# thomasneff/AdaNeRF

Hardware: AMD Instinct MI355X
Metric: FPS at 800x800 (higher is better)
Workload: dtype bf16

## Files before the change

adanerf_amd/csrc/adanerf_hip.hip:

```cpp
#include "context.hpp"

#include <algorithm>
#include <cmath>
#include <cstdio>
#include <cstring>
#include <exception>
#include <limits>
#include <string>
#include <vector>

#include "guard_record.hpp"
#include "kernels.hip.hpp"
#include "launch_f32.hpp"
#include "k_generic_f32.hip.hpp"
#include "k_generic16.hip.hpp"

using namespace adanerf;

namespace adanerf {

int fail(adanerf_ctx* c, int code, const std::string& msg) {
  if (c) c->err = msg;
  else g_create_error = msg;
  return code;
}

int hip_rc(adanerf_ctx* c, hipError_t e, const char* what) {
  return e == hipSuccess ? ADANERF_OK : fail(c, ADANERF_EDEVICE, std::string(what) + ": " + hipGetErrorString(e));
}

int dev_alloc(adanerf_ctx* c, DevBuf* b, size_t bytes) {
  if (b->bytes >= bytes && b->p) return ADANERF_OK;
  void* grown = nullptr;
  if (bytes) HIP_TRY(c, hipMalloc(&grown, bytes));
  if (b->p) HIP_TRY(c, hipFree(b->p));
  b->p = grown;
  b->bytes = bytes;
  return ADANERF_OK;
}

}

namespace {

enum { kTotalSamples = 0, kTotalRefined = 4, kTotalGuardSeen = 8, kTotalSlots = 16 };
enum { kSeenMax = 0, kSeenViolations = 1, kSeenPair = 2, kSeenAuditMismatch = 3, kSeenAudited = 4, kGuardSeenSlots = 5 };

constexpr const char* kOccupancyQuery = "hipOccupancyMaxActiveBlocksPerMultiprocessor";

int upload_net(adanerf_ctx* c, const PackedNet& pn, PackedDev* d) {
  int rc;
  if ((rc = dev_alloc(c, &d->w, pn.weights.size()))) return rc;
  if ((rc = dev_alloc(c, &d->b, pn.bias.size() * sizeof(float)))) return rc;
  HIP_TRY(c, hipMemcpy(d->w.p, pn.weights.data(), pn.weights.size(), hipMemcpyHostToDevice));
  HIP_TRY(c, hipMemcpy(d->b.p, pn.bias.data(), pn.bias.size() * sizeof(float), hipMemcpyHostToDevice));
  d->params.w = reinterpret_cast<const u32x4*>(d->w.p);
  d->params.bias = reinterpret_cast<const float*>(d->b.p);
  for (size_t i = 0; i < pn.w_off.size() && i < kMaxLayers; ++i) {
    d->params.w_off[i] = pn.w_off[i];
    d->params.b_off[i] = pn.b_off[i];
  }
  d->params.n_bias = static_cast<uint32_t>(pn.bias.size());
  d->params.out_scale[0] = std::ldexp(1.0f, pn.out_exp[0]);
  d->params.out_scale[1] = std::ldexp(1.0f, pn.out_exp[1]);
  return ADANERF_OK;
}

int ensure_shading_net(adanerf_ctx* c, int prec, bool coarse) {
  if (prec < 0 || prec > 2) return fail(c, ADANERF_EINVAL, "precision must be ADANERF_PREC_{BF16,FP16,FP32}");
  PackedDev& dev = coarse ? c->netc[prec] : c->net1[prec];
  if (dev.w.p) return ADANERF_OK;
  PackedNet pn;
  std::string err;
  const NetShape sh = coarse ? shape_of(c->ms.fp0, c->ms.fd0, c->ms.fp0, c->ms.fd0, 0, false)
                             : shape_of(c->ms.fp0, c->ms.fd0, c->ms.fp1, c->ms.fd1, c->ms.ray_samples, !c->ms.coarse_fine);
  if (!pack_shading_net(coarse ? c->net0_host : c->net1_host, sh, elem_of(prec), &pn, &err))
    return fail(c, ADANERF_EIO, (coarse ? "model0.onnx: " : "model1.onnx: ") + err);
  return upload_net(c, pn, &dev);
}

int ensure_batch_buffers(adanerf_ctx* c, int n_rays, int n_max) {
  if (n_rays <= c->cap_rays && n_max <= c->cap_nmax) return ADANERF_OK;
  n_rays = std::max(n_rays, c->cap_rays);
  n_max = std::max(n_max, c->cap_nmax);
  if (c->cap_rays > 0) HIP_TRY(c, hipStreamSynchronize(c->stream));
  const size_t R = static_cast<size_t>(n_rays), S = R * static_cast<size_t>(n_max);
  const size_t nblk = (R + 31) / 32;
  int rc;
  if ((rc = dev_alloc(c, &c->rays, R * 8 * sizeof(float)))) return rc;
  if ((rc = dev_alloc(c, &c->ray_offsets, R * sizeof(int32_t)))) return rc;
  if ((rc = dev_alloc(c, &c->ray_counts, R * sizeof(int32_t)))) return rc;
  if (c->ms.coarse_fine) {
    const size_t Sc = R * static_cast<size_t>(c->ms.n_coarse);
    if ((rc = dev_alloc(c, &c->key_coarse, Sc * sizeof(uint32_t)))) return rc;
    if ((rc = dev_alloc(c, &c->raw_coarse, Sc * 4 * sizeof(float)))) return rc;
    if ((rc = dev_alloc(c, &c->sample_z, S * sizeof(float)))) return rc;
  } else {
    if ((rc = dev_alloc(c, &c->oracle, R * kBins * sizeof(float)))) return rc;
    if ((rc = dev_alloc(c, &c->selbin, S))) return rc;
    if ((rc = dev_alloc(c, &c->selw, S * sizeof(float)))) return rc;
    if (c->sampling_mode == ADANERF_SAMPLING_GUARDED) {
      if ((rc = dev_alloc(c, &c->guard_mask, nblk * sizeof(uint32_t)))) return rc;
      if ((rc = dev_alloc(c, &c->refine_list, R * sizeof(int32_t)))) return rc;
      if ((rc = dev_alloc(c, &c->guard_probe, R * 2 * sizeof(float)))) return rc;
    }
  }
  if ((rc = dev_alloc(c, &c->block_total, nblk * sizeof(int32_t)))) return rc;
  if ((rc = dev_alloc(c, &c->block_offset, nblk * sizeof(int32_t)))) return rc;
  if (!c->total.p) {
    if ((rc = dev_alloc(c, &c->total, kTotalSlots * sizeof(int32_t)))) return rc;
    HIP_TRY(c, hipMemset(c->total.p, 0, kTotalSlots * sizeof(int32_t)));
  }
  if ((rc = dev_alloc(c, &c->sample_key, S * sizeof(uint32_t)))) return rc;
  if ((rc = dev_alloc(c, &c->sample_w, S * sizeof(float)))) return rc;
  if ((rc = dev_alloc(c, &c->raw, S * 4 * sizeof(float)))) return rc;
  if (c->ms.info.sampler_mode == ADANERF_SAMPLER_PDF && (rc = dev_alloc(c, &c->sample_z, S * sizeof(float)))) return rc;
  c->cap_rays = n_rays;
  c->cap_nmax = n_max;
  return ADANERF_OK;
}

int ensure_compact_scratch(adanerf_ctx* c, int n_rays, int n_max) {
  const size_t R = static_cast<size_t>(std::max(n_rays, 1)), S = R * static_cast<size_t>(n_max);
  const size_t nblk = (R + 31) / 32;
  int rc;
  if (c->selbin.bytes < S || c->selw.bytes < S * sizeof(float) || c->block_total.bytes < nblk * sizeof(int32_t) ||
      c->block_offset.bytes < nblk * sizeof(int32_t)) {
    HIP_TRY(c, hipStreamSynchronize(c->stream));
    if ((rc = dev_alloc(c, &c->selbin, S))) return rc;
    if ((rc = dev_alloc(c, &c->selw, S * sizeof(float)))) return rc;
    if ((rc = dev_alloc(c, &c->block_total, nblk * sizeof(int32_t)))) return rc;
    if ((rc = dev_alloc(c, &c->block_offset, nblk * sizeof(int32_t)))) return rc;
  }
  return ADANERF_OK;
}


int ensure_guard_band(adanerf_ctx* c);

bool has_split_sampling(const adanerf_ctx* c) { return (!c->generic0 || c->ms.ray_samples == 0) && c->topo0.width != kWideWidth; }

bool generic_split_sampling(const adanerf_ctx* c) {
  return c->generic0 && c->sampling_mode != ADANERF_SAMPLING_FP32 && c->ms.ray_samples == 0 && c->net0_split.w.p != nullptr;
}

RayGenParams rg_in_force(const adanerf_ctx* c) { return with_pixel_offset(c->ms.rg, c->px_dx, c->px_dy); }

bool has_budget_map(const adanerf_ctx* c) { return c->budget_n != nullptr || c->budget_thr != nullptr; }

struct RayList {
  const int32_t* ids;
  const int32_t* count;
};

int launch_sample_mlp(adanerf_ctx* c, int first_ray, int n_rays, float* d_oracle, float* d_rays, const SelectOut* sel = nullptr,
                      const RayList* list = nullptr) {
  if (n_rays <= 0) return ADANERF_OK;
  if (list && (c->generic0 || !sel || (c->sampling_mode != ADANERF_SAMPLING_SPLIT_FP16 && c->sampling_mode != ADANERF_SAMPLING_GUARDED)))
    return fail(c, ADANERF_EUNSUPPORTED, "a ray list needs the 8 x 256 sampling network on the split-precision engine with the fused selection");
  SampleArgs a{};
  if (sel) {
    a.sel = *sel;
    a.fused_select = 1;
  }
  a.g = rg_in_force(c);
  a.net = c->net0.params;
  a.net16 = c->net0_split.params;
  a.overflow_flag = reinterpret_cast<int32_t*>(c->overflow.p);
  a.first_ray = first_ray;
  a.n_rays = n_rays;
  a.oracle_out = d_oracle;
  a.rays_out = d_rays;
  dim3 grid((n_rays + 127) / 128), block(256);
  if (c->generic0) {
    if (generic_split_sampling(c)) {
      const int W0 = c->topo0.width;
      if (a.net16.n_bias > dispatch<64, 128, 256>(W0, [](auto w) { return uint32_t(gen_bias_cap<w()>()); }, 0u))
        return fail(c, ADANERF_EUNSUPPORTED, "sampling network: bias table exceeds the kernel's LDS capacity");
      return hip_rc(c, dispatch<kEnc10_4, kEnc2_2, kEncMax>(c->enc0, [&](auto e) {
        return dispatch<64, 128, 256>(W0, [&](auto w) {
          hipLaunchKernelGGL((sample_mlp16x3_gen_kernel<enc_fp(e()), enc_fd(e()), w()>), grid, block, 0, c->stream, a, c->gen0);
          return hipGetLastError();
        }, hipErrorInvalidValue);
      }, hipErrorInvalidValue), "hipGetLastError()");
    }
    if (sel) return fail(c, ADANERF_EINVAL, "fused selection is not available on the fp32 run-time-shaped sampling kernel");
    HIP_RETURN(c, launch_sample_mlp_gen(a, c->gen0, c->enc0, c->topo0.width, grid.x, c->stream));
  }
  const bool guarded = c->sampling_mode == ADANERF_SAMPLING_GUARDED && sel != nullptr && !has_budget_map(c) && !(c->sample_cap > 0.f) && !list;
  if (list) {
    a.ray_list = list->ids;
    a.n_list = list->count;
  }
  if (guarded) {
    if (int rc = c->guard_eps > 0.f ? 0 : ensure_guard_band(c)) return rc;
    a.sel.guard_mask = reinterpret_cast<uint32_t*>(c->guard_mask.p);
    a.sel.guard_eps = guard_band_of(c->ms.transform, c->guard_eps);
    a.sel.guard_pair = guard_pair_of(c->ms.transform, c->guard_eps, c->guard_eps_pair);
    a.sel.audit_period = c->guard_audit_period;
    a.sel.audit_phase = c->guard_audit_period > 0 ? static_cast<int32_t>(c->guard_frame & static_cast<uint32_t>(c->guard_audit_period - 1)) : 0;
    a.sel.guard_probe = reinterpret_cast<float*>(c->guard_probe.p);
    a.sel.guard_rows = reinterpret_cast<float*>(c->oracle.p);
    if (c->debug_guard & 1) a.sel.guard_rows = nullptr;
    a.sel.guard_seen = reinterpret_cast<uint32_t*>(c->total.p) + kTotalGuardSeen;
  }
  if (c->sampling_mode == ADANERF_SAMPLING_FP32) HIP_RETURN(c, launch_sample_mlp_f32(a, c->enc0, grid.x, c->stream));
  auto for_enc = [&](auto&& f) {
    return dispatch<kEnc10_4, kEnc2_2>(c->enc0, [&](auto e) { return f(std::integral_constant<int, enc_fp(e())>{}, std::integral_constant<int, enc_fd(e())>{}); },
                                       hipErrorInvalidValue);
  };
  if (c->sampling_mode == ADANERF_SAMPLING_FP16 || guarded) {
    if (!c->net0_f16.w.p) {
      PackedNet pn;
      std::string err;
      const NetShape sh = shape_of(c->ms.fp0, c->ms.fd0, c->ms.fp1, c->ms.fd1, c->ms.ray_samples);
      if (!pack_sampling_net(c->net0_host, sh, Elem::F16, &pn, &err)) return fail(c, ADANERF_EIO, "model0.onnx: " + err);
      if (int rc = upload_net(c, pn, &c->net0_f16)) return rc;
    }
    a.net16 = c->net0_f16.params;
    const bool two_blocks = sel != nullptr && a.fused_select && !a.oracle_out && !(c->debug_guard & 2) && (n_rays >= kSample16x2MinRays || (c->debug_guard & 4));
    if (int rc = hip_rc(c, for_enc([&](auto fp, auto fd) {
      return two_blocks ? launch_persistent(c->grids, sample_mlp16x2_kernel<fp(), fd()>, (n_rays + 255) / 256, 256, c->stream, a)
                        : launch_persistent(c->grids, sample_mlp16_kernel<fp(), fd()>, (n_rays + 255) / 256, 512, c->stream, a);
    }), kOccupancyQuery)) return rc;
    if (guarded) {
      const int n_words = (n_rays + 31) / 32;
      int32_t* n_list = reinterpret_cast<int32_t*>(c->total.p) + kTotalRefined;
      int resident = 0;
      if (int rc = hip_rc(c, for_enc([&](auto fp, auto fd) { return persistent_grid(c->grids, sample_mlp16x3_kernel<fp(), fd()>, 256, &resident); }), kOccupancyQuery)) return rc;
      const int rgrid = std::min(static_cast<int>(grid.x), resident);
      const int cap_round = (c->opt.flags & ADANERF_FLAG_GUARD_AUDIT_FILL) ? rgrid * 128 : 0;
      const int cycle = a.sel.audit_period > 0 ? static_cast<int>((c->guard_frame / static_cast<uint32_t>(a.sel.audit_period)) & 0x7fffffffu) : 0;
      hipLaunchKernelGGL(refine_list_kernel, dim3((n_words + 255) / 256), dim3(256), 0, c->stream, reinterpret_cast<const uint32_t*>(c->guard_mask.p),
                         n_words, n_rays, a.sel.audit_period, a.sel.audit_phase, cap_round, cycle, reinterpret_cast<int32_t*>(c->refine_list.p), n_list);
      SampleArgs r = a;
      r.net16 = c->net0_split.params;
      r.rays_out = nullptr;
      r.sel.guard_mask = nullptr;
      r.sel.guard_band = c->guard_eps;
      r.sel.guard_band_pair = c->ms.transform == kOracleRaw ? a.sel.guard_pair : 0.f;
      r.sel.guard_eps = 0.f;
      r.sel.guard_pair = 0.f;
      r.sel.audit_period = 0;
      r.sel.refine_list = reinterpret_cast<const int32_t*>(c->refine_list.p);
      r.ray_list = r.sel.refine_list;
      r.n_list = n_list;
      if (int rc = hip_rc(c, for_enc([&](auto fp, auto fd) { return launch_persistent(c->grids, sample_mlp16x3_kernel<fp(), fd()>, rgrid, 256, c->stream, r); }), kOccupancyQuery)) return rc;
    }
  } else {
    if (int rc = hip_rc(c, for_enc([&](auto fp, auto fd) { return launch_persistent(c->grids, sample_mlp16x3_kernel<fp(), fd()>, static_cast<int>(grid.x), 256, c->stream, a); }), kOccupancyQuery)) return rc;
  }
  HIP_RETURN(c, hipGetLastError());
}

constexpr int kInlineScanMaxBlocks = 65536;

SelectOut select_out(adanerf_ctx* c, int n_max, float thr, int32_t* d_cnt) {
  SelectOut so{};
  so.counts = d_cnt;
  so.selbin = reinterpret_cast<uint8_t*>(c->selbin.p);
  so.selw = reinterpret_cast<float*>(c->selw.p);
  so.seg_total = reinterpret_cast<int32_t*>(c->block_total.p);
  so.n_max = n_max;
  so.thr = thr;
  so.transform = c->ms.transform;
  return so;
}

int launch_expand(adanerf_ctx* c, int n_rays, int n_max, int seg_shift, int32_t* d_off, const int32_t* d_cnt, uint32_t* d_key, float* d_w,
                  int32_t* d_total) {
  const int nblk = (n_rays + (1 << seg_shift) - 1) >> seg_shift;
  const int32_t* bt = reinterpret_cast<const int32_t*>(c->block_total.p);
  int32_t* bo = reinterpret_cast<int32_t*>(c->block_offset.p);
  const dim3 egrid((n_rays + 255) / 256);
  const bool inline_scan = nblk <= kInlineScanMaxBlocks;
  if (!inline_scan) hipLaunchKernelGGL(scan_blocks_kernel, dim3(1), dim3(1024), 0, c->stream, bt, nblk, bo, d_total);
  hipLaunchKernelGGL(inline_scan ? expand_kernel<true> : expand_kernel<false>, egrid, dim3(256), 0, c->stream, d_cnt, reinterpret_cast<const uint8_t*>(c->selbin.p),
                     reinterpret_cast<const float*>(c->selw.p), bo, bt, nblk, n_rays, n_max, seg_shift, d_off, d_key, d_w, d_total);
  HIP_RETURN(c, hipGetLastError());
}

struct BudgetMaps {
  const uint8_t* n;
  const float* thr;
  int first;
};

int launch_trim(adanerf_ctx* c, const BudgetMaps& bm, int n_rays, int n_max, float thr, int seg_shift, int32_t* d_cnt) {
  if (n_rays <= 0) return ADANERF_OK;
  const bool per_thread = n_max <= kTrimThreadMaxN;
  const dim3 grid(per_thread ? (n_rays + 255) / 256 : (n_rays + (1 << seg_shift) - 1) >> seg_shift);
  hipLaunchKernelGGL(per_thread ? trim_rows_kernel : trim_rows_wave_kernel, grid, dim3(256), 0, c->stream, d_cnt, reinterpret_cast<uint8_t*>(c->selbin.p),
                     reinterpret_cast<float*>(c->selw.p), bm.n, bm.thr, bm.first, n_rays, n_max, thr, seg_shift, reinterpret_cast<int32_t*>(c->block_total.p));
  HIP_RETURN(c, hipGetLastError());
}

struct DepthLimit {
  const float* zc;
  int first;
  const int32_t* list;
  const float* rays;
  const float* ztab;
  DepthPose pose;
};

DepthPose depth_pose(const float pos[3], const float rot[9]) { return DepthPose{{pos[0], pos[1], pos[2]}, rot[2], rot[5], rot[8]}; }

int launch_depth_limit(adanerf_ctx* c, const DepthLimit& dl, int n_rays, int n_max, int seg_shift, int32_t* d_cnt) {
  if (n_rays <= 0) return ADANERF_OK;
  hipLaunchKernelGGL(depth_limit_kernel, dim3((n_rays + 255) / 256), dim3(256), 0, c->stream, d_cnt, reinterpret_cast<uint8_t*>(c->selbin.p),
                     reinterpret_cast<float*>(c->selw.p), dl.rays, dl.zc, dl.list, dl.first, dl.pose, dl.ztab, n_rays, n_max, seg_shift,
                     reinterpret_cast<int32_t*>(c->block_total.p));
  HIP_RETURN(c, hipGetLastError());
}

bool has_sample_cap(const adanerf_ctx* c) { return c->sample_cap > 0.f; }

bool cap_trims(const adanerf_ctx* c) { return has_sample_cap(c) && c->sample_cap < static_cast<float>(c->ms.info.num_samples); }

int64_t cap_total_of(const adanerf_ctx* c, int n_rays) { return static_cast<int64_t>(std::floor(static_cast<double>(c->sample_cap) * n_rays)); }

constexpr size_t kCapStateBytes = sizeof(CapState) + static_cast<size_t>(kCapLevels) * 2 * kCapBins * sizeof(uint32_t);

int ensure_cap_buffers(adanerf_ctx* c, int n_rays) {
  const size_t map_bytes = static_cast<size_t>(std::max(n_rays, 1)) * sizeof(float);
  if (c->cap_state.p && c->cap_record.p && c->cap_map.bytes >= map_bytes) return ADANERF_OK;
  HIP_TRY(c, hipStreamSynchronize(c->stream));
  int rc;
  if ((rc = dev_alloc(c, &c->cap_state, kCapStateBytes))) return rc;
  if ((rc = dev_alloc(c, &c->cap_map, map_bytes))) return rc;
  if (!c->cap_record.p) {
    if ((rc = dev_alloc(c, &c->cap_record, sizeof(CapRecord)))) return rc;
    hipLaunchKernelGGL(cap_reset_kernel, dim3(1), dim3(1), 0, c->stream, reinterpret_cast<CapRecord*>(c->cap_record.p));
    HIP_TRY(c, hipGetLastError());
  }
  return ADANERF_OK;
}

int launch_cap(adanerf_ctx* c, int n_rays, int n_max, float thr, int seg_shift, int32_t* d_cnt, int64_t cap_total) {
  if (n_rays <= 0) return ADANERF_OK;
  CapState* st = reinterpret_cast<CapState*>(c->cap_state.p);
  uint32_t* hist = reinterpret_cast<uint32_t*>(st + 1);
  CapRecord* rec = reinterpret_cast<CapRecord*>(c->cap_record.p);
  float* map = reinterpret_cast<float*>(c->cap_map.p);
  const float* selw = reinterpret_cast<const float*>(c->selw.p);
  HIP_TRY(c, hipMemsetAsync(st, 0, kCapStateBytes, c->stream));
  const bool wave = n_max > kCapThreadMaxN;
  const int cus = std::max(c->ms.info.compute_units, 1);
  const dim3 grid(wave ? std::min((n_rays + 3) / 4, 4 * cus) : std::min((n_rays + 255) / 256, 2 * cus));
  for (int level = 0; level < kCapLevels; ++level) {
    uint32_t* h = hist + static_cast<size_t>(level) * 2 * kCapBins;
    hipLaunchKernelGGL(wave ? cap_hist_kernel<true> : cap_hist_kernel<false>, grid, dim3(256), 0, c->stream, d_cnt, selw, n_rays, n_max, level, st, h);
    hipLaunchKernelGGL(cap_search_kernel, dim3(1), dim3(1024), 0, c->stream, level, static_cast<long long>(cap_total), st, h, rec);
  }
  hipLaunchKernelGGL(cap_fill_kernel, dim3((n_rays + 255) / 256), dim3(256), 0, c->stream, rec, n_rays, map);
  HIP_TRY(c, hipGetLastError());
  return launch_trim(c, BudgetMaps{nullptr, map, 0}, n_rays, n_max, thr, seg_shift, d_cnt);
}

bool use_pair_select(const adanerf_ctx* c, int n_max) { return n_max <= kPairMaxN && !(c->opt.flags & ADANERF_FLAG_WAVE_SELECT); }

int launch_compact(adanerf_ctx* c, const float* d_oracle, int n_rays, int n_max, float thr, int32_t* d_off, int32_t* d_cnt,
                   uint32_t* d_key, float* d_w, int32_t* d_total, const BudgetMaps* bm = nullptr, const DepthLimit* dl = nullptr,
                   const int64_t* cap_total = nullptr) {
  if (n_rays <= 0) return ADANERF_OK;
  if (thr == 0.0f) {
    const size_t n = static_cast<size_t>(n_rays) * kBins;
    dim3 grid(static_cast<unsigned>((n + 255) / 256)), block(256);
    hipLaunchKernelGGL(dense_expand_kernel, grid, block, 0, c->stream, d_oracle, n_rays, d_off, d_cnt, d_key, d_w, d_total);
    HIP_RETURN(c, hipGetLastError());
  }
  if (use_pair_select(c, n_max)) {
    hipLaunchKernelGGL(select_rows_kernel, dim3((n_rays + 127) / 128), dim3(256), 0, c->stream, d_oracle, n_rays, select_out(c, n_max, thr, d_cnt),
                       static_cast<const int32_t*>(nullptr));
    if (bm)
      if (int rc = launch_trim(c, *bm, n_rays, n_max, thr, kPairSegShift, d_cnt)) return rc;
    if (dl)
      if (int rc = launch_depth_limit(c, *dl, n_rays, n_max, kPairSegShift, d_cnt)) return rc;
    if (cap_total)
      if (int rc = launch_cap(c, n_rays, n_max, thr, kPairSegShift, d_cnt, *cap_total)) return rc;
    return launch_expand(c, n_rays, n_max, kPairSegShift, d_off, d_cnt, d_key, d_w, d_total);
  }
  const int nblk = (n_rays + kSelRaysPerBlock - 1) / kSelRaysPerBlock;
  hipLaunchKernelGGL(select_kernel, dim3(nblk), dim3(256), 0, c->stream, d_oracle, n_rays, n_max, thr, c->ms.transform, d_cnt,
                     reinterpret_cast<uint8_t*>(c->selbin.p), reinterpret_cast<float*>(c->selw.p),
                     reinterpret_cast<int32_t*>(c->block_total.p));
  if (bm)
    if (int rc = launch_trim(c, *bm, n_rays, n_max, thr, kSelSegShift, d_cnt)) return rc;
  if (dl)
    if (int rc = launch_depth_limit(c, *dl, n_rays, n_max, kSelSegShift, d_cnt)) return rc;
  if (cap_total)
    if (int rc = launch_cap(c, n_rays, n_max, thr, kSelSegShift, d_cnt, *cap_total)) return rc;
  return launch_expand(c, n_rays, n_max, kSelSegShift, d_off, d_cnt, d_key, d_w, d_total);
}

GuardKey guard_key(adanerf_ctx* c) {
  if (!c->model0_hash) c->model0_hash = fnv1a64_file(join_path(c->model_dir, "model0.onnx"));
  return GuardKey{c->model0_hash, c->ms.fp0, c->ms.fd0, c->ms.transform, kGuardEngineRev, c->ms.info.num_samples, c->ms.info.threshold, c->model_dir, c->opt.flags};
}

void install_guard_band(adanerf_ctx* c, float max_diff, float max_pair, int poses, int source) {
  c->guard_eps = std::max(ADANERF_GUARD_CALIB_MARGIN * max_diff, ADANERF_GUARD_EPS_MIN);
  c->guard_eps_pair = (c->ms.transform == kOracleRaw && max_pair > 0.f)
                          ? std::min(std::max(ADANERF_GUARD_CALIB_MARGIN * max_pair, ADANERF_GUARD_EPS_MIN), 2.0f * c->guard_eps)
                          : 2.0f * c->guard_eps;
  c->ms.info.guard_eps = c->guard_eps;
  c->ms.info.guard_eps_pair = c->guard_eps_pair;
  c->ms.info.guard_calib_source = source;
  c->ms.info.guard_calib_poses = poses;
}

int calibrate_guard(adanerf_ctx* c, int n_poses, uint32_t seed, bool install, float* max_diff, float* max_pair) {
  if (c->ms.coarse_fine || c->generic0) return fail(c, ADANERF_EUNSUPPORTED, "guard calibration needs an 8 x 256 sampling network");
  if (n_poses < 1 || n_poses > 4096) return fail(c, ADANERF_EINVAL, "n_poses must be in 1..4096");
  constexpr int CW = 64, CH = 64, CR = CW * CH;
  const RayGenParams saved = c->ms.rg;
  const int saved_mode = c->sampling_mode;
  const float saved_dx = c->px_dx, saved_dy = c->px_dy;
  c->px_dx = c->px_dy = 0.f;
  RayGenParams g = saved;
  const double x_dist = -saved.start_x + saved.x_pp / 2, y_dist = -saved.start_y + saved.y_pp / 2;
  g.w = CW;
  g.h = CH;
  g.x_pp = x_dist / (CW / 2.0);
  g.y_pp = y_dist / (CH / 2.0);
  g.start_x = -(x_dist - g.x_pp / 2);
  g.start_y = -(y_dist - g.y_pp / 2);
  g.strip_rows = CH;
  g.world = 1;
  g.rank = 0;
  DevBuf a_buf, b_buf, acc;
  int rc = ADANERF_OK;
  auto done = [&](int code) {
    (void)hipStreamSynchronize(c->stream);
    c->ms.rg = saved;
    c->sampling_mode = saved_mode;
    c->px_dx = saved_dx;
    c->px_dy = saved_dy;
    return code;
  };
  if ((rc = dev_alloc(c, &a_buf, static_cast<size_t>(CR) * kBins * sizeof(float)))) return done(rc);
  if ((rc = dev_alloc(c, &b_buf, static_cast<size_t>(CR) * kBins * sizeof(float)))) return done(rc);
  if ((rc = dev_alloc(c, &acc, 64))) return done(rc);
  if (hipMemsetAsync(acc.p, 0, 64, c->stream) != hipSuccess) return done(fail(c, ADANERF_EDEVICE, "hipMemsetAsync failed"));
  const bool want_pairs = c->ms.transform == kOracleRaw && c->ms.info.threshold > 0.f && c->ms.info.num_samples <= kPairMaxN;
  float d = 0.f, dp = 0.f;
  bool nonfinite = false;
  for (int sweep = 0; sweep < (want_pairs ? 2 : 1) && !nonfinite; ++sweep) {
    const float two_eps = sweep == 0 ? 0.f : 2.0f * std::max(ADANERF_GUARD_CALIB_MARGIN * d, ADANERF_GUARD_EPS_MIN);
    uint64_t st = 0x9E3779B97F4A7C15ull ^ (static_cast<uint64_t>(seed) << 17);
    auto rnd = [&]() {
      st ^= st >> 12;
      st ^= st << 25;
      st ^= st >> 27;
      return static_cast<double>((st * 0x2545F4914F6CDD1Dull) >> 11) * (1.0 / 9007199254740992.0);
    };
    for (int k = 0; k < n_poses; ++k) {
      for (int i = 0; i < 3; ++i) g.pos[i] = g.center[i] + static_cast<float>((rnd() - 0.5) * 0.9 * c->ms.info.view_cell_size[i]);
      const double yaw = 2.0 * M_PI * rnd(), pitch = (rnd() - 0.5) * (c->ms.info.use_ndc ? 0.2 : 1.4);
      const double cy = std::cos(yaw), sy = std::sin(yaw), cp = std::cos(pitch), sp = std::sin(pitch);
      double fwd[3], right[3], up[3];
      if (c->ms.info.use_ndc) {
        fwd[0] = sp * cy; fwd[1] = sp * sy; fwd[2] = -cp;
        right[0] = 1; right[1] = 0; right[2] = 0;
      } else {
        fwd[0] = cp * cy; fwd[1] = cp * sy; fwd[2] = sp;
        right[0] = sy; right[1] = -cy; right[2] = 0;
      }
      const double rf = right[0] * fwd[0] + right[1] * fwd[1] + right[2] * fwd[2];
      double n = 0;
      for (int i = 0; i < 3; ++i) { right[i] -= rf * fwd[i]; n += right[i] * right[i]; }
      n = std::sqrt(n);
      for (int i = 0; i < 3; ++i) right[i] /= n;
      up[0] = right[1] * fwd[2] - right[2] * fwd[1];
      up[1] = right[2] * fwd[0] - right[0] * fwd[2];
      up[2] = right[0] * fwd[1] - right[1] * fwd[0];
      for (int i = 0; i < 3; ++i) {
        g.rot[3 * i + 0] = static_cast<float>(right[i]);
        g.rot[3 * i + 1] = static_cast<float>(up[i]);
        g.rot[3 * i + 2] = static_cast<float>(-fwd[i]);
      }
      c->ms.rg = g;
      c->sampling_mode = ADANERF_SAMPLING_SPLIT_FP16;
      if ((rc = launch_sample_mlp(c, 0, CR, reinterpret_cast<float*>(a_buf.p), nullptr))) return done(rc);
      c->sampling_mode = ADANERF_SAMPLING_FP16;
      if ((rc = launch_sample_mlp(c, 0, CR, reinterpret_cast<float*>(b_buf.p), nullptr))) return done(rc);
      hipLaunchKernelGGL(guard_stats_kernel, dim3((CR + 3) / 4), dim3(256), 0, c->stream, reinterpret_cast<const float*>(b_buf.p),
                         reinterpret_cast<const float*>(a_buf.p), CR, c->ms.info.num_samples, c->ms.info.threshold, two_eps, reinterpret_cast<uint32_t*>(acc.p));
    }
    uint32_t res[3] = {0, 0, 0};
    if (hipMemcpyAsync(res, acc.p, sizeof(res), hipMemcpyDeviceToHost, c->stream) != hipSuccess || hipStreamSynchronize(c->stream) != hipSuccess)
      return done(fail(c, ADANERF_EDEVICE, "guard calibration: read-back failed"));
    std::memcpy(&d, &res[0], sizeof(d));
    std::memcpy(&dp, &res[2], sizeof(dp));
    nonfinite = res[1] != 0;
  }
  if (max_diff) *max_diff = nonfinite ? INFINITY : d;
  if (max_pair) *max_pair = (nonfinite || !want_pairs) ? 0.f : dp;
  if (install) {
    if (nonfinite) {
      c->guard_eps = ADANERF_GUARD_EPS_DEFAULT;
      c->guard_eps_pair = 2.0f * c->guard_eps;
      c->ms.info.guard_eps = c->guard_eps;
      c->ms.info.guard_eps_pair = c->guard_eps_pair;
      c->ms.info.guard_calib_source = ADANERF_GUARD_FROM_CALIBRATION;
      c->ms.info.guard_calib_poses = n_poses;
    } else {
      install_guard_band(c, d, want_pairs ? dp : 0.f, n_poses, ADANERF_GUARD_FROM_CALIBRATION);
      const GuardKey key = guard_key(c);
      GuardRecord old;
      if (!(read_guard_record(key, &old) && old.poses > n_poses)) write_guard_record(key, GuardRecord{n_poses, seed, d, want_pairs ? dp : 0.f});
    }
  }
  return done(ADANERF_OK);
}

int ensure_guard_band(adanerf_ctx* c) {
  GuardRecord r;
  if (read_guard_record(guard_key(c), &r) && r.poses >= ADANERF_GUARD_CALIB_POSES) {
    install_guard_band(c, r.max_diff, r.max_pair, r.poses, ADANERF_GUARD_FROM_RECORD);
    return ADANERF_OK;
  }
  float d = 0.f, dp = 0.f;
  return calibrate_guard(c, ADANERF_GUARD_CALIB_POSES, 1u, true, &d, &dp);
}

int reset_guard_band(adanerf_ctx* c) {
  if (c->sampling_mode == ADANERF_SAMPLING_GUARDED)
    HIP_TRY(c, hipMemsetAsync(reinterpret_cast<int32_t*>(c->total.p) + kTotalRefined, 0, sizeof(int32_t), c->stream));
  const adanerf_options& opt = c->opt;
  c->guard_eps = opt.guard_eps > 0.f ? opt.guard_eps : 0.f;
  c->guard_eps_pair = (c->guard_eps > 0.f && opt.guard_eps_pair > 0.f) ? std::min(opt.guard_eps_pair, 2.0f * c->guard_eps) : 2.0f * c->guard_eps;
  c->ms.info.guard_eps = c->guard_eps;
  c->ms.info.guard_eps_pair = c->guard_eps_pair;
  c->ms.info.guard_calib_source = c->guard_eps > 0.f ? ADANERF_GUARD_FROM_OPTIONS : ADANERF_GUARD_FROM_NONE;
  c->ms.info.guard_calib_poses = 0;
  c->guard_frame = 0;
  c->guard_ev_stale = c->guard_ev_pending;
  return ADANERF_OK;
}

int apply_selection(adanerf_ctx* c) {
  if (int rc = ensure_batch_buffers(c, c->ms.info.batch_rays, c->ms.info.num_samples)) return rc;
  if (int rc = reset_guard_band(c)) return rc;
  c->ms.sp.ztab = reinterpret_cast<const float*>(c->ztab.p) + (c->ms.info.dense ? kBins : 0);
  return ADANERF_OK;
}

int apply_frame_size(adanerf_ctx* c, int was_rays) {
  const size_t B = static_cast<size_t>(c->ms.info.batch_rays);
  if (int rc = ensure_batch_buffers(c, c->ms.info.batch_rays, c->ms.info.num_samples)) return rc;
  if (c->disp_scratch.p && c->disp_scratch.bytes < B * 2 * sizeof(float)) {
    HIP_TRY(c, hipStreamSynchronize(c->stream));
    if (int rc = dev_alloc(c, &c->disp_scratch, B * 2 * sizeof(float))) return rc;
  }
  if (c->ms.info.rays_local != was_rays) {
    c->aux_depth = c->aux_acc = c->aux_disp = nullptr;
    c->budget_n = nullptr;
    c->budget_thr = nullptr;
    c->depth_limit = nullptr;
  }
  c->guard_frame = 0;
  return ADANERF_OK;
}

int launch_shade_mlp(adanerf_ctx* c, const float* d_rays, const uint32_t* d_key, const int32_t* d_total, int max_samples, int prec,
                     float* d_raw, const float* d_z = nullptr, bool coarse = false) {
  if (max_samples <= 0) return ADANERF_OK;
  const bool generic = coarse ? c->genericc : c->generic1;
  const NetTopology& topo = coarse ? c->topoc : c->topo1;
  const GenericTopo& gen = coarse ? c->genc : c->gen1;
  int rc = ensure_shading_net(c, prec, coarse);
  if (rc) return rc;
  ShadeArgs a{};
  a.sp = coarse ? c->spc : c->ms.sp;
  a.net = coarse ? c->netc[prec].params : c->net1[prec].params;
  a.rays = d_rays;
  a.sample_key = d_key;
  a.sample_z = d_z;
  a.total = d_total;
  a.max_samples = max_samples;
  a.raw_out = d_raw;
  a.pos_limit = prec == ADANERF_PREC_BF16 ? static_cast<float>(kPosIdentityBound) : std::numeric_limits<float>::max();
  const int enc = coarse ? enc_layout(c->ms.fp0, c->ms.fd0, false) : c->enc1;
  auto for_elem = [&](auto&& f) { return prec == ADANERF_PREC_BF16 ? f(Bf16{}) : f(Fp16{}); };
  if (generic && prec != ADANERF_PREC_FP32) {
    if (a.net.n_bias > dispatch<64, 128, 256, 512>(topo.width, [](auto w) { return uint32_t(gen_bias_cap<w()>()); }, 0u))
      return fail(c, ADANERF_EUNSUPPORTED, "shading network: bias table exceeds the kernel's LDS capacity");
    if ((rc = hip_rc(c, for_elem([&](auto et) {
      return dispatch<kEnc10_4, kEncMax>(enc, [&](auto e) {
        return dispatch<64, 128, 256, 512>(topo.width, [&](auto w) {
          using ET = decltype(et);
          constexpr int FP = enc_fp(e()), FD = enc_fd(e()), W = w(), NB = gen_blocks<W, FP>();
          const int tiles = (max_samples + 128 * NB - 1) / (128 * NB);
          return launch_persistent(c->grids, shade_mlp16_gen_staged_kernel<ET, FP, FD, W, NB, gen_occupancy<W, FP>()>, tiles, 256, c->stream, a, gen);
        }, hipErrorInvalidValue);
      }, hipErrorInvalidValue);
    }), kOccupancyQuery))) return rc;
  } else if (generic) {
    const int per_wg = topo.width == kWideWidth ? 64 : 128;
    HIP_TRY(c, launch_shade_mlp_gen(c->grids, a, gen, enc, topo.width, (max_samples + per_wg - 1) / per_wg, c->stream));
  } else if (prec == ADANERF_PREC_FP32) {
    HIP_TRY(c, launch_shade_mlp_f32(c->grids, a, (max_samples + 127) / 128, c->stream));
  } else {
    const int tiles = (max_samples + 255) / 256;
    if ((rc = hip_rc(c, for_elem([&](auto et) {
      using ET = decltype(et);
      hipLaunchKernelGGL((shade_mlp16x2_kernel<ET, 10, 4>), dim3(std::min(tiles, c->ms.info.compute_units)), dim3(256), 0, c->stream, a);
      return hipSuccess;
    }), kOccupancyQuery))) return rc;
  }
  HIP_RETURN(c, hipGetLastError());
}

int launch_sample_pdf(adanerf_ctx* c, const float* d_oracle, int n_rays, int n, int32_t* d_off, int32_t* d_cnt, uint32_t* d_key, float* d_w,
                      float* d_z, int32_t* d_total) {
  if (n_rays <= 0) return ADANERF_OK;
  const int grid = std::min((n_rays + 3) / 4, c->ms.info.compute_units * 8);
  hipLaunchKernelGGL(pdf_sample_kernel, dim3(grid), dim3(256), 0, c->stream, d_oracle, n_rays, n, c->ms.transform, c->ms.dm, d_off, d_cnt, d_key, d_w, d_z, d_total);
  HIP_RETURN(c, hipGetLastError());
}

int launch_camera_rays(adanerf_ctx* c, int first_ray, int n_rays, float* d_rays) {
  if (n_rays <= 0) return ADANERF_OK;
  hipLaunchKernelGGL(camera_rays_kernel, dim3((n_rays + 255) / 256), dim3(256), 0, c->stream, rg_in_force(c), first_ray, n_rays, d_rays);
  HIP_RETURN(c, hipGetLastError());
}

int launch_sample_uniform(adanerf_ctx* c, int n_rays, int n, int32_t* d_off, int32_t* d_cnt, uint32_t* d_key, int32_t* d_total) {
  if (n_rays <= 0) return ADANERF_OK;
  const int64_t s = static_cast<int64_t>(n_rays) * n;
  hipLaunchKernelGGL(uniform_sample_kernel, dim3(static_cast<unsigned>((s + 255) / 256)), dim3(256), 0, c->stream, n_rays, n, d_off, d_cnt, d_key, d_total);
  HIP_RETURN(c, hipGetLastError());
}

int launch_sample_fine(adanerf_ctx* c, const float* d_raw_coarse, const float* d_rays, int n_rays, int32_t* d_off, int32_t* d_cnt,
                       uint32_t* d_key, float* d_z, int32_t* d_total) {
  if (n_rays <= 0) return ADANERF_OK;
  hipLaunchKernelGGL(fine_sample_kernel, dim3((n_rays + kFineRaysPerBlock - 1) / kFineRaysPerBlock), dim3(kFineRaysPerBlock), 0, c->stream,
                     reinterpret_cast<const float4*>(d_raw_coarse), reinterpret_cast<const float*>(c->ztab_coarse.p), d_rays, n_rays, c->ms.n_coarse,
                     c->ms.info.num_samples - c->ms.n_coarse, d_off, d_cnt, d_key, d_z, d_total);
  HIP_RETURN(c, hipGetLastError());
}

int launch_composite_classic(adanerf_ctx* c, const float* d_raw, const float* d_z, const float* d_rays, int n_rays, int n, float* d_rgb,
                             void* d_rgba8, float* d_depth = nullptr, float* d_acc = nullptr) {
  if (n_rays <= 0) return ADANERF_OK;
  const bool wave = n > 32;
  hipLaunchKernelGGL(wave ? composite_classic_wave_kernel : composite_classic_kernel, dim3((n_rays + (wave ? 3 : 255)) / (wave ? 4 : 256)), dim3(256), 0, c->stream,
                     reinterpret_cast<const float4*>(d_raw), d_z, d_rays, n_rays, n, d_rgb, reinterpret_cast<uchar4*>(d_rgba8), d_depth, d_acc);
  HIP_RETURN(c, hipGetLastError());
}

int launch_composite(adanerf_ctx* c, const float* d_raw, const float* d_w, const int32_t* d_off, const int32_t* d_cnt, int n_rays,
                     float* d_rgb, void* d_rgba8, const uint32_t* d_key = nullptr, float* d_depth = nullptr, float* d_acc = nullptr) {
  if (n_rays <= 0) return ADANERF_OK;
  AuxOut aux{};
  if ((d_key || c->ms.info.dense) && (d_depth || d_acc)) {
    aux.depth = d_depth;
    aux.acc = d_acc;
    aux.sample_key = d_key;
    aux.ztab = c->ms.sp.ztab;
  }
  if (c->ms.info.num_samples > 32)
    hipLaunchKernelGGL(composite_wave_kernel, dim3((n_rays + 3) / 4), dim3(256), 0, c->stream, reinterpret_cast<const float4*>(d_raw), d_w,
                       d_off, d_cnt, n_rays, c->ms.mult_mode, d_rgb, reinterpret_cast<uchar4*>(d_rgba8), aux);
  else {
    const int N = c->ms.info.num_samples;
    auto run = [&](auto rb_tag) {
      constexpr int RB = decltype(rb_tag)::value;
      const int cap = RB * N;
      hipLaunchKernelGGL(composite_kernel<RB>, dim3((n_rays + RB - 1) / RB), dim3(RB), static_cast<size_t>(cap) * 20, c->stream,
                         reinterpret_cast<const float4*>(d_raw), d_w, d_off, d_cnt, n_rays, c->ms.mult_mode, cap, d_rgb,
                         reinterpret_cast<uchar4*>(d_rgba8), aux);
    };
    if (N <= 9) run(std::integral_constant<int, 256>{});
    else if (N <= 19) run(std::integral_constant<int, 128>{});
    else run(std::integral_constant<int, 64>{});
  }
  HIP_RETURN(c, hipGetLastError());
}

}


extern "C" {

const char* adanerf_last_error(const adanerf_ctx* ctx) { return ctx ? ctx->err.c_str() : g_create_error.c_str(); }

static int create_on(adanerf_ctx* c, const char* model_dir, const adanerf_options* opt, adanerf_ctx** out);

int adanerf_create(const char* model_dir, const adanerf_options* opt, adanerf_ctx** out) {
  if (!out) return fail(nullptr, ADANERF_EINVAL, "out == NULL");
  *out = nullptr;
  if (!model_dir || !opt) return fail(nullptr, ADANERF_EINVAL, "model_dir/opt == NULL");
  adanerf_ctx* c = nullptr;
  try {
    c = new adanerf_ctx();
    return create_on(c, model_dir, opt, out);
  } catch (const std::exception& e) {
    *out = nullptr;
    adanerf_destroy(c);
    return fail(nullptr, ADANERF_EIO, std::string("adanerf_create: ") + e.what());
  }
}

static int create_on(adanerf_ctx* c, const char* model_dir, const adanerf_options* opt, adanerf_ctx** out) {
  auto bail = [&](int code, const std::string& msg) {
    g_create_error = msg;
    adanerf_destroy(c);
    return code;
  };
  std::string err;
  ModelSetup& ms = c->ms;
  int rc = setup_model(model_dir, opt, &ms, &err);
  if (rc) return bail(rc, err);
  c->opt = *opt;

  TensorMap& n0 = c->net0_host;
  if (!read_onnx_initializers(join_path(model_dir, "model0.onnx"), &n0, &err)) return bail(ADANERF_EIO, err);
  if (!read_onnx_initializers(join_path(model_dir, "model1.onnx"), &c->net1_host, &err)) return bail(ADANERF_EIO, err);
  const NetShape sh = shape_of(c->ms.fp0, c->ms.fd0, c->ms.fp1, c->ms.fd1, c->ms.ray_samples, !c->ms.coarse_fine);
  c->enc0 = enc_layout(c->ms.fp0, c->ms.fd0, !c->ms.coarse_fine);
  c->enc1 = enc_layout(c->ms.fp1, c->ms.fd1, false);
  PackedNet p0, p0s, p1;
  if (c->ms.coarse_fine) {
    const NetShape shc = shape_of(c->ms.fp0, c->ms.fd0, c->ms.fp0, c->ms.fd0, 0, false);
    if (!pack_shading_net(n0, shc, Elem::F32, &p0, &err)) return bail(ADANERF_EIO, "model0.onnx: " + err);
    c->topoc = p0.topo;
    c->genericc = !p0.topo.is_default(true) || c->enc0 == kEncMax;
    if (opt->precision != ADANERF_PREC_FP32 && !pack_shading_net(n0, shc, elem_of(opt->precision), &p0, &err))
      return bail(ADANERF_EIO, "model0.onnx: " + err);
  } else {
    if (!pack_sampling_net(n0, sh, Elem::F32, &p0, &err)) return bail(ADANERF_EIO, "model0.onnx: " + err);
    if (p0.topo.bins != ms.bins)
      return bail(ADANERF_EIO, "model0.onnx has " + std::to_string(p0.topo.bins) + " outputs, config.ini says multiDepthFeatures = " + std::to_string(ms.bins));
    c->topo0 = p0.topo;
    c->generic0 = !p0.topo.is_default(false) || c->enc0 == kEncMax;
    if (has_split_sampling(c) && !pack_sampling_net(n0, sh, Elem::F16_SPLIT, &p0s, &err)) return bail(ADANERF_EIO, "model0.onnx: " + err);
  }
  c->sampling_mode = opt->sampling_mode;
  c->model_dir = model_dir;
  if (const char* dbg = std::getenv("ADANERF_DEBUG_GUARD")) c->debug_guard = std::atoi(dbg);
  c->guard_audit_period = opt->guard_audit_period == 0 ? ADANERF_GUARD_AUDIT_PERIOD : std::max(opt->guard_audit_period, 0);
  c->ms.info.guard_audit_period = c->sampling_mode == ADANERF_SAMPLING_GUARDED ? c->guard_audit_period : 0;
  if (c->sampling_mode == ADANERF_SAMPLING_GUARDED) c->model0_hash = fnv1a64_file(join_path(model_dir, "model0.onnx"));
  {
    PackedNet probe;
    if (!pack_shading_net(c->net1_host, sh, Elem::F32, &probe, &err)) return bail(ADANERF_EIO, "model1.onnx: " + err);
    c->topo1 = probe.topo;
    c->generic1 = !probe.topo.is_default(true) || c->enc1 == kEncMax;
    if (opt->precision == ADANERF_PREC_FP32) p1 = std::move(probe);
    else if (!pack_shading_net(c->net1_host, sh, elem_of(opt->precision), &p1, &err)) return bail(ADANERF_EIO, "model1.onnx: " + err);
  }
  auto width_ok = [](int w) { return w == 64 || w == 128 || w == 256 || w == kWideWidth; };
  if (c->genericc && !width_ok(c->topoc.width)) return bail(ADANERF_EUNSUPPORTED, "model0.onnx: layer width " + std::to_string(c->topoc.width) + " (64, 128, 256 or 512 supported)");
  if (c->generic0 && !width_ok(c->topo0.width)) return bail(ADANERF_EUNSUPPORTED, "model0.onnx: layer width " + std::to_string(c->topo0.width) + " (64, 128, 256 or 512 supported)");
  if (c->generic1 && !width_ok(c->topo1.width)) return bail(ADANERF_EUNSUPPORTED, "model1.onnx: layer width " + std::to_string(c->topo1.width) + " (64, 128, 256 or 512 supported)");

  int n_dev = 0;
  if (hipGetDeviceCount(&n_dev) != hipSuccess || n_dev <= 0)
    return bail(ADANERF_EDEVICE, "no HIP device available: libadanerf_hip has no CPU fallback");
  if (hipSetDevice(opt->device_id) != hipSuccess) return bail(ADANERF_EDEVICE, "hipSetDevice failed");
  hipDeviceProp_t prop;
  if (hipGetDeviceProperties(&prop, opt->device_id) != hipSuccess) return bail(ADANERF_EDEVICE, "hipGetDeviceProperties failed");
  if (std::string(prop.gcnArchName).find("gfx950") == std::string::npos)
    return bail(ADANERF_EDEVICE, std::string("device is ") + prop.gcnArchName + "; this library is built for gfx950 (MI355X) only");
  c->ms.info.compute_units = c->grids.compute_units = prop.multiProcessorCount;
  c->device = opt->device_id;
  if (hipStreamCreateWithFlags(&c->own_stream, hipStreamNonBlocking) != hipSuccess) return bail(ADANERF_EDEVICE, "hipStreamCreate failed");
  c->stream = c->own_stream;

  rc = dev_alloc(c, &c->ztab, 2 * kBins * sizeof(float));
  if (rc) return bail(rc, c->err);
  float ztabs[2 * kBins];
  depth_table(ms, false, ztabs);
  depth_table(ms, true, ztabs + kBins);
  if (hipMemcpy(c->ztab.p, ztabs, sizeof(ztabs), hipMemcpyHostToDevice) != hipSuccess)
    return bail(ADANERF_EDEVICE, "ztab upload failed");
  if (c->ms.coarse_fine) {
    if ((rc = upload_net(c, p0, &c->netc[opt->precision]))) return bail(rc, c->err);
    if ((rc = dev_alloc(c, &c->ztab_coarse, kMaxCoarse * sizeof(float)))) return bail(rc, c->err);
    if (hipMemcpy(c->ztab_coarse.p, ms.ztab_coarse.data(), ms.ztab_coarse.size() * sizeof(float), hipMemcpyHostToDevice) != hipSuccess)
      return bail(ADANERF_EDEVICE, "coarse depth table upload failed");
    c->spc = c->ms.sp;
    c->spc.normalize = ms.normalize0;
    c->ms.sp.unit_dir = 0;
    c->spc.ztab = reinterpret_cast<const float*>(c->ztab_coarse.p);
    c->genc = GenericTopo{c->topoc.depth, c->topoc.cat_mask, 0, 0, nullptr, 0.f};
  } else {
    if ((rc = upload_net(c, p0, &c->net0))) return bail(rc, c->err);
    if (has_split_sampling(c) && (rc = upload_net(c, p0s, &c->net0_split))) return bail(rc, c->err);
  }
  if (c->ms.ray_samples > 0) {
    if ((rc = dev_alloc(c, &c->rsi_z, ms.rsi_z.size() * sizeof(float)))) return bail(rc, c->err);
    if (hipMemcpy(c->rsi_z.p, ms.rsi_z.data(), ms.rsi_z.size() * sizeof(float), hipMemcpyHostToDevice) != hipSuccess)
      return bail(ADANERF_EDEVICE, "raySampleInput depth table upload failed");
  }
  c->gen0 = GenericTopo{c->topo0.depth, 0, c->ms.ray_samples, p0.rsi_w_off, reinterpret_cast<const float*>(c->rsi_z.p), c->ms.cfg.depthRange[1]};
  c->gen1 = GenericTopo{c->topo1.depth, c->topo1.cat_mask, 0, 0, nullptr, 0.f};
  if ((rc = dev_alloc(c, &c->overflow, 64))) return bail(rc, c->err);
  if (hipMemset(c->overflow.p, 0, 64) != hipSuccess) return bail(ADANERF_EDEVICE, "hipMemset failed");
  if ((rc = upload_net(c, p1, &c->net1[opt->precision]))) return bail(rc, c->err);
  if ((rc = apply_selection(c))) return bail(rc, c->err);
  *out = c;
  return ADANERF_OK;
}

int adanerf_destroy(adanerf_ctx* c) {
  if (!c) return ADANERF_OK;
  (void)hipSetDevice(c->device);
  if (c->peer_event) (void)hipEventDestroy(c->peer_event);
  if (c->stream) (void)hipStreamSynchronize(c->stream);
  for (hipEvent_t e : c->events) (void)hipEventDestroy(e);
  for (int32_t* p : c->pinned_totals) (void)hipHostFree(p);
  if (c->guard_host) (void)hipHostFree(c->guard_host);
  if (c->guard_ev) (void)hipEventDestroy(c->guard_ev);
  const hipStream_t own = c->own_stream;
  delete c;
  if (own) (void)hipStreamDestroy(own);
  return ADANERF_OK;
}

int adanerf_get_info(const adanerf_ctx* c, adanerf_info* info) {
  if (!c || !info) return ADANERF_EINVAL;
  *info = c->ms.info;
  return ADANERF_OK;
}

int adanerf_set_camera(adanerf_ctx* c, const float pos[3], const float rot[9]) {
  if (!c) return ADANERF_EINVAL;
  if (!pos || !rot) return fail(c, ADANERF_EINVAL, "pos/rot == NULL");
  if (c->ms.pos_bound.active) {
    double d2 = 0.0;
    for (int i = 0; i < 3; ++i) d2 += (pos[i] - c->ms.pos_bound.center[i]) * (pos[i] - c->ms.pos_bound.center[i]);
    const double bound = c->ms.pos_bound.at(std::sqrt(d2));
    if (!(bound <= kPosIdentityBound)) {
      char msg[256];
      std::snprintf(msg, sizeof(msg), "camera %.3g away from the view-cell centre: sample positions can reach %.3g, beyond the %.0f the bf16 shading path's "
                    "layer scaling assumes -- create the context with precision fp16 or fp32 for such poses", std::sqrt(d2), bound, kPosIdentityBound);
      return fail(c, ADANERF_EUNSUPPORTED, msg);
    }
  }
  std::memcpy(c->ms.rg.pos, pos, 3 * sizeof(float));
  std::memcpy(c->ms.rg.rot, rot, 9 * sizeof(float));
  return ADANERF_OK;
}

int adanerf_set_selection(adanerf_ctx* c, int32_t num_samples, float threshold) {
  BIND(c);
  if (std::isnan(threshold)) return fail(c, ADANERF_EINVAL, "threshold is not a number (a negative value keeps the one in force)");
  if (threshold >= 0.f && c->ms.info.sampler_mode != ADANERF_SAMPLER_ADAPTIVE)
    return fail(c, ADANERF_EUNSUPPORTED, "this model's sampler takes no threshold (adanerf_create ignores options.threshold for it): pass a negative one");
  if (threshold == 0.f && has_budget_map(c))
    return fail(c, ADANERF_EUNSUPPORTED, "threshold 0 (dense) keeps every bin: remove the budget map first (adanerf_set_budget_map with two NULLs)");
  if (threshold == 0.f && c->depth_limit)
    return fail(c, ADANERF_EUNSUPPORTED, "threshold 0 (dense) keeps every bin with implicit keys: remove the depth limit first (adanerf_set_depth_limit with NULL)");
  if (threshold == 0.f && has_sample_cap(c))
    return fail(c, ADANERF_EUNSUPPORTED, "threshold 0 (dense) keeps every bin: remove the sample cap first (adanerf_set_sample_cap with 0)");
  ModelSetup& ms = c->ms;
  const adanerf_info was = ms.info;
  const ModelSetup::PosBound was_bound = ms.pos_bound;
  const int was_n = ms.sel_n;
  const float was_thr = ms.sel_thr;
  std::vector<float> was_ztab = ms.ztab;
  std::string err;
  if (int rc = select_samples(&ms, num_samples, threshold, &err)) return fail(c, rc, err);
  if (ms.info.num_samples == was.num_samples && ms.info.threshold == was.threshold) return ADANERF_OK;
  if (int rc = apply_selection(c)) {
    ms.info = was;
    ms.pos_bound = was_bound;
    ms.sel_n = was_n;
    ms.sel_thr = was_thr;
    ms.ztab = std::move(was_ztab);
    return rc;
  }
  return ADANERF_OK;
}

int adanerf_set_frame_size(adanerf_ctx* c, int32_t width, int32_t height) {
  BIND(c);
  ModelSetup& ms = c->ms;
  const int w = width > 0 ? width : ms.info.width, h = height > 0 ? height : ms.info.height;
  if (w == ms.info.width && h == ms.info.height) return ADANERF_OK;
  const adanerf_info was = ms.info;
  const RayGenParams was_rg = ms.rg;
  std::string err;
  if (int rc = frame_geometry(&ms, &c->opt, w, h, &err)) return fail(c, rc, err);
  if (int rc = apply_frame_size(c, was.rays_local)) {
    ms.info = was;
    ms.rg = was_rg;
    return rc;
  }
  c->opt.width = w;
  c->opt.height = h;
  return ADANERF_OK;
}

int adanerf_set_pixel_offset(adanerf_ctx* c, float dx, float dy) {
  if (!c) return ADANERF_EINVAL;
  if (!(std::fabs(dx) <= 1.f) || !(std::fabs(dy) <= 1.f))
    return fail(c, ADANERF_EINVAL, "adanerf_set_pixel_offset: dx and dy must be finite and within -1..1 (pixels)");
  c->px_dx = dx;
  c->px_dy = dy;
  return ADANERF_OK;
}

int adanerf_get_pixel_offset(const adanerf_ctx* c, float out[2]) {
  if (!c || !out) return ADANERF_EINVAL;
  out[0] = c->px_dx;
  out[1] = c->px_dy;
  return ADANERF_OK;
}

int adanerf_sync(adanerf_ctx* c) {
  BIND(c);
  HIP_RETURN(c, hipStreamSynchronize(c->stream));
}

int adanerf_ray_features(adanerf_ctx* c, int32_t first_ray, int32_t n_rays, float* d_feat, float* d_rays) {
  BIND(c);
  if (c->ms.coarse_fine) return fail(c, ADANERF_EUNSUPPORTED, "coarse/fine models have no sampling network");
  if (first_ray < 0 || n_rays < 0 || first_ray + n_rays > c->ms.info.rays_local) return fail(c, ADANERF_EINVAL, "ray range outside this context's rays");
  if (n_rays == 0) return ADANERF_OK;
  dim3 grid((n_rays + 255) / 256), block(256);
  const float* rz = reinterpret_cast<const float*>(c->rsi_z.p);
  const float d1 = c->ms.cfg.depthRange[1];
  hipLaunchKernelGGL(ray_features_kernel, grid, block, 0, c->stream, rg_in_force(c), first_ray, n_rays, d_feat, d_rays, c->ms.ray_samples, rz, d1, c->ms.fp0, c->ms.fd0);
  HIP_RETURN(c, hipGetLastError());
}

int adanerf_sample_mlp(adanerf_ctx* c, int32_t first_ray, int32_t n_rays, float* d_oracle, float* d_rays) {
  BIND(c);
  if (c->ms.coarse_fine) return fail(c, ADANERF_EUNSUPPORTED, "coarse/fine models have no sampling network (adanerf_sample_uniform / adanerf_shade_mlp_coarse)");
  if (first_ray < 0 || n_rays < 0 || first_ray + n_rays > c->ms.info.rays_local) return fail(c, ADANERF_EINVAL, "ray range outside this context's rays");
  return launch_sample_mlp(c, first_ray, n_rays, d_oracle, d_rays);
}

int adanerf_compact(adanerf_ctx* c, const float* d_oracle, int32_t n_rays, int32_t n_max, float thr, int32_t* d_off, int32_t* d_cnt,
                    uint32_t* d_key, float* d_w, int32_t* d_total) {
  BIND(c);
  if (!d_oracle || !d_off || !d_cnt || !d_key || !d_w || !d_total) return fail(c, ADANERF_EINVAL, "NULL buffer");
  if (n_rays < 0 || n_max < 1 || n_max > kBins || thr < 0.f) return fail(c, ADANERF_EINVAL, "n_rays/n_max/thr out of range");
  if (thr == 0.f && n_max != kBins) return fail(c, ADANERF_EINVAL, "dense mode (thr == 0) requires n_max == 128");
  if (static_cast<int64_t>(n_rays) >= (1ll << 25)) return fail(c, ADANERF_EINVAL, "n_rays must be < 2^25 per batch");
  if (static_cast<int64_t>(n_rays) * n_max > 0x7fffffffll) return fail(c, ADANERF_EINVAL, "n_rays * n_max exceeds 2^31 - 1");
  if (int rc = ensure_compact_scratch(c, n_rays, n_max)) return rc;
  return launch_compact(c, d_oracle, n_rays, n_max, thr, d_off, d_cnt, d_key, d_w, d_total);
}

int adanerf_compact_guarded(adanerf_ctx* c, const float* d_approx, const float* d_exact, int32_t n_rays, int32_t n_max, float thr, float eps,
                            float eps_pair, int32_t audit_period, int32_t audit_phase, int32_t audit_fill_cap, int32_t audit_cycle, int32_t* d_off,
                            int32_t* d_cnt, uint32_t* d_key, float* d_w, int32_t* d_total, int32_t* d_refined, uint32_t* d_monitor) {
  BIND(c);
  if (!d_approx || !d_exact || !d_off || !d_cnt || !d_key || !d_w || !d_total || !d_refined) return fail(c, ADANERF_EINVAL, "NULL buffer");
  if (n_rays < 0 || n_max < 1 || n_max > kPairMaxN || !(thr > 0.f) || !(eps > 0.f)) return fail(c, ADANERF_EINVAL, "n_rays/n_max/thr/eps out of range");
  if (audit_period > 32 || (audit_period > 0 && (audit_period & (audit_period - 1)) != 0)) return fail(c, ADANERF_EINVAL, "audit_period must be a power of two <= 32");
  if (static_cast<int64_t>(n_rays) >= (1ll << 25)) return fail(c, ADANERF_EINVAL, "n_rays must be < 2^25 per batch");
  if (n_rays == 0) return ADANERF_OK;
  int rc = ensure_compact_scratch(c, n_rays, n_max);
  if (rc) return rc;
  const int n_words = (n_rays + 31) / 32;
  if (c->guard_mask.bytes < n_words * sizeof(uint32_t) || c->refine_list.bytes < static_cast<size_t>(n_rays) * sizeof(int32_t) ||
      c->guard_probe.bytes < static_cast<size_t>(n_rays) * 2 * sizeof(float)) {
    HIP_TRY(c, hipStreamSynchronize(c->stream));
    if ((rc = dev_alloc(c, &c->guard_mask, n_words * sizeof(uint32_t)))) return rc;
    if ((rc = dev_alloc(c, &c->refine_list, static_cast<size_t>(n_rays) * sizeof(int32_t)))) return rc;
    if ((rc = dev_alloc(c, &c->guard_probe, static_cast<size_t>(n_rays) * 2 * sizeof(float)))) return rc;
  }
  const int period = audit_period > 0 ? audit_period : 0, phase = period ? (audit_phase & (period - 1)) : 0;
  SelectOut so = select_out(c, n_max, thr, d_cnt);
  so.guard_mask = reinterpret_cast<uint32_t*>(c->guard_mask.p);
  so.guard_eps = guard_band_of(c->ms.transform, eps);
  so.guard_pair = guard_pair_of(c->ms.transform, eps, eps_pair);
  so.audit_period = period;
  so.audit_phase = phase;
  so.guard_probe = reinterpret_cast<float*>(c->guard_probe.p);
  const dim3 grid((n_rays + 127) / 128), block(256);
  hipLaunchKernelGGL(select_rows_kernel, grid, block, 0, c->stream, d_approx, n_rays, so, static_cast<const int32_t*>(nullptr));
  hipLaunchKernelGGL(refine_list_kernel, dim3((n_words + 255) / 256), dim3(256), 0, c->stream, reinterpret_cast<const uint32_t*>(c->guard_mask.p), n_words,
                     n_rays, period, phase, audit_fill_cap > 0 ? audit_fill_cap : 0, audit_cycle, reinterpret_cast<int32_t*>(c->refine_list.p), d_refined);
  so.guard_mask = nullptr;
  so.guard_band = eps;
  so.guard_band_pair = c->ms.transform == kOracleRaw ? so.guard_pair : 0.f;
  so.guard_eps = 0.f;
  so.guard_pair = 0.f;
  so.audit_period = 0;
  so.refine_list = reinterpret_cast<const int32_t*>(c->refine_list.p);
  so.guard_rows = d_monitor ? const_cast<float*>(d_approx) : nullptr;
  so.guard_seen = d_monitor;
  hipLaunchKernelGGL(select_rows_kernel, grid, block, 0, c->stream, d_exact, n_rays, so, static_cast<const int32_t*>(d_refined));
  return launch_expand(c, n_rays, n_max, kPairSegShift, d_off, d_cnt, d_key, d_w, d_total);
}

int adanerf_calibrate_guard(adanerf_ctx* c, int32_t n_poses, uint32_t seed, int32_t set, float* max_diff, float* max_pair_diff) {
  BIND(c);
  return calibrate_guard(c, n_poses, seed, set != 0, max_diff, max_pair_diff);
}

int adanerf_guard_calibration_file(const adanerf_ctx* c, char* buf, size_t buf_bytes) {
  if (!c) return ADANERF_EINVAL;
  const std::string p = guard_record_path(guard_key(const_cast<adanerf_ctx*>(c)));
  if (buf && buf_bytes > 0) {
    const size_t n = std::min(p.size(), buf_bytes - 1);
    std::memcpy(buf, p.data(), n);
    buf[n] = 0;
  }
  return static_cast<int>(p.size() + 1);
}

int adanerf_abi_version(void) { return ADANERF_ABI_VERSION; }

int adanerf_struct_sizes(int32_t sizes_out[3]) {
  if (!sizes_out) return ADANERF_EINVAL;
  sizes_out[0] = static_cast<int32_t>(sizeof(adanerf_options));
  sizes_out[1] = static_cast<int32_t>(sizeof(adanerf_info));
  sizes_out[2] = static_cast<int32_t>(sizeof(adanerf_stats));
  return ADANERF_OK;
}

int adanerf_shade_features(adanerf_ctx* c, const float* d_rays, const uint32_t* d_key, int32_t n_samples, float* d_feat) {
  BIND(c);
  if (!d_rays || !d_key || !d_feat || n_samples < 0) return fail(c, ADANERF_EINVAL, "bad argument");
  if (n_samples == 0) return ADANERF_OK;
  ShadeArgs a{};
  a.sp = c->ms.sp;
  a.rays = d_rays;
  a.sample_key = d_key;
  a.max_samples = n_samples;
  hipLaunchKernelGGL(shade_features_kernel, dim3((n_samples + 255) / 256), dim3(256), 0, c->stream, a, d_feat, c->ms.fp1, c->ms.fd1);
  HIP_RETURN(c, hipGetLastError());
}

int adanerf_shade_mlp(adanerf_ctx* c, const float* d_rays, const uint32_t* d_key, const int32_t* d_total, int32_t max_samples,
                      int32_t precision, float* d_raw) {
  return adanerf_shade_mlp_z(c, d_rays, d_key, nullptr, d_total, max_samples, precision, d_raw);
}

int adanerf_shade_mlp_z(adanerf_ctx* c, const float* d_rays, const uint32_t* d_key, const float* d_z, const int32_t* d_total,
                        int32_t max_samples, int32_t precision, float* d_raw) {
  BIND(c);
  if (!d_rays || !d_key || !d_raw || max_samples < 0) return fail(c, ADANERF_EINVAL, "bad argument");
  return launch_shade_mlp(c, d_rays, d_key, d_total, max_samples, precision < 0 ? c->ms.info.precision : precision, d_raw, d_z);
}

int adanerf_sample_uniform(adanerf_ctx* c, int32_t first_ray, int32_t n_rays, float* d_rays, int32_t* d_off, int32_t* d_cnt, uint32_t* d_key,
                           int32_t* d_total) {
  BIND(c);
  if (!c->ms.coarse_fine) return fail(c, ADANERF_EUNSUPPORTED, "adanerf_sample_uniform: not a coarse/fine model");
  if (!d_rays || !d_off || !d_cnt || !d_key || !d_total) return fail(c, ADANERF_EINVAL, "NULL buffer");
  if (first_ray < 0 || n_rays < 0 || first_ray + n_rays > c->ms.info.rays_local) return fail(c, ADANERF_EINVAL, "ray range outside this context's rays");
  int rc = launch_camera_rays(c, first_ray, n_rays, d_rays);
  return rc ? rc : launch_sample_uniform(c, n_rays, c->ms.n_coarse, d_off, d_cnt, d_key, d_total);
}

int adanerf_shade_mlp_coarse(adanerf_ctx* c, const float* d_rays, const uint32_t* d_key, const int32_t* d_total, int32_t max_samples,
                             int32_t precision, float* d_raw) {
  BIND(c);
  if (!c->ms.coarse_fine) return fail(c, ADANERF_EUNSUPPORTED, "adanerf_shade_mlp_coarse: not a coarse/fine model");
  if (!d_rays || !d_key || !d_raw || max_samples < 0) return fail(c, ADANERF_EINVAL, "bad argument");
  return launch_shade_mlp(c, d_rays, d_key, d_total, max_samples, precision < 0 ? c->ms.info.precision : precision, d_raw, nullptr, true);
}

int adanerf_sample_from_coarse(adanerf_ctx* c, const float* d_raw_coarse, const float* d_rays, int32_t n_rays, int32_t* d_off, int32_t* d_cnt,
                               uint32_t* d_key, float* d_z, int32_t* d_total) {
  BIND(c);
  if (!c->ms.coarse_fine) return fail(c, ADANERF_EUNSUPPORTED, "adanerf_sample_from_coarse: not a coarse/fine model");
  if (!d_raw_coarse || !d_rays || !d_off || !d_cnt || !d_key || !d_z || !d_total) return fail(c, ADANERF_EINVAL, "NULL buffer");
  if (n_rays < 0 || static_cast<int64_t>(n_rays) * c->ms.info.num_samples > 0x7fffffffll || n_rays >= (1 << 25))
    return fail(c, ADANERF_EINVAL, "n_rays out of range");
  return launch_sample_fine(c, d_raw_coarse, d_rays, n_rays, d_off, d_cnt, d_key, d_z, d_total);
}

int adanerf_sample_pdf(adanerf_ctx* c, const float* d_oracle, int32_t n_rays, int32_t n, int32_t* d_off, int32_t* d_cnt, uint32_t* d_key,
                       float* d_w, float* d_z, int32_t* d_total) {
  BIND(c);
  if (!d_oracle || !d_off || !d_cnt || !d_key || !d_w || !d_z || !d_total) return fail(c, ADANERF_EINVAL, "NULL buffer");
  if (n_rays < 0 || n < 1 || n > 4096) return fail(c, ADANERF_EINVAL, "n_rays/n out of range");
  if (static_cast<int64_t>(n_rays) * n > 0x7fffffffll || n_rays >= (1 << 25)) return fail(c, ADANERF_EINVAL, "n_rays * n too large");
  return launch_sample_pdf(c, d_oracle, n_rays, n, d_off, d_cnt, d_key, d_w, d_z, d_total);
}

int adanerf_composite_classic(adanerf_ctx* c, const float* d_raw, const float* d_z, const float* d_rays, int32_t n_rays, int32_t n,
                              float* d_rgb, void* d_rgba8) {
  BIND(c);
  if (!d_raw || !d_z || !d_rays || n_rays < 0 || n < 1) return fail(c, ADANERF_EINVAL, "bad argument");
  return launch_composite_classic(c, d_raw, d_z, d_rays, n_rays, n, d_rgb, d_rgba8);
}

int adanerf_composite(adanerf_ctx* c, const float* d_raw, const float* d_w, const int32_t* d_off, const int32_t* d_cnt, int32_t n_rays,
                      float* d_rgb, void* d_rgba8) {
  BIND(c);
  if (!d_raw || !d_w || !d_off || !d_cnt || n_rays < 0) return fail(c, ADANERF_EINVAL, "bad argument");
  return launch_composite(c, d_raw, d_w, d_off, d_cnt, n_rays, d_rgb, d_rgba8);
}

int adanerf_composite_aux(adanerf_ctx* c, const float* d_raw, const float* d_w, const int32_t* d_off, const int32_t* d_cnt, const uint32_t* d_key,
                          int32_t n_rays, float* d_rgb, void* d_rgba8, float* d_depth, float* d_acc) {
  BIND(c);
  if (!d_raw || !d_w || !d_off || !d_cnt || n_rays < 0) return fail(c, ADANERF_EINVAL, "bad argument");
  if (!d_key && !c->ms.info.dense && (d_depth || d_acc))
    return fail(c, ADANERF_EINVAL, "adanerf_composite_aux: a depth or acc map needs d_sample_key unless the context is dense (threshold 0)");
  return launch_composite(c, d_raw, d_w, d_off, d_cnt, n_rays, d_rgb, d_rgba8, d_key, d_depth, d_acc);
}

int adanerf_composite_classic_aux(adanerf_ctx* c, const float* d_raw, const float* d_z, const float* d_rays, int32_t n_rays, int32_t n,
                                  float* d_rgb, void* d_rgba8, float* d_depth, float* d_acc) {
  BIND(c);
  if (!d_raw || !d_z || !d_rays || n_rays < 0 || n < 1) return fail(c, ADANERF_EINVAL, "bad argument");
  return launch_composite_classic(c, d_raw, d_z, d_rays, n_rays, n, d_rgb, d_rgba8, d_depth, d_acc);
}

int adanerf_disp_map(adanerf_ctx* c, const float* d_depth, const float* d_acc, int32_t n, float* d_disp) {
  BIND(c);
  if (!d_depth || !d_acc || !d_disp || n < 0) return fail(c, ADANERF_EINVAL, "adanerf_disp_map: NULL buffer or n < 0");
  if (n == 0) return ADANERF_OK;
  hipLaunchKernelGGL(disp_map_kernel, dim3((n + 255) / 256), dim3(256), 0, c->stream, d_depth, d_acc, n, d_disp);
  HIP_RETURN(c, hipGetLastError());
}

namespace {

constexpr size_t kMaxProfiledBatches = 1 << 16;

void reset_record(adanerf_ctx* c) {
  c->events_used = 0;
  c->prof_frames = 0;
  c->folded = adanerf_stats{};
}

int sum_stats(adanerf_ctx* c, adanerf_stats* stats) {
  std::memset(stats, 0, sizeof(*stats));
  const size_t nb = c->events_used / 5;
  for (size_t b = 0; b < nb; ++b) {
    hipEvent_t* ev = &c->events[b * 5];
    float t;
    HIP_TRY(c, hipEventElapsedTime(&t, ev[0], ev[1]));
    stats->ms_sample_mlp += t;
    HIP_TRY(c, hipEventElapsedTime(&t, ev[1], ev[2]));
    stats->ms_compact += t;
    HIP_TRY(c, hipEventElapsedTime(&t, ev[2], ev[3]));
    stats->ms_shade_mlp += t;
    HIP_TRY(c, hipEventElapsedTime(&t, ev[3], ev[4]));
    stats->ms_composite += t;
    HIP_TRY(c, hipEventElapsedTime(&t, ev[0], ev[4]));
    stats->ms_total += t;
    const int32_t* tot = c->pinned_totals[b];
    stats->total_samples += tot[kTotalSamples];
    if (c->sampling_mode == ADANERF_SAMPLING_GUARDED) {
      stats->rays_refined += tot[kTotalRefined];
      const int32_t* gs = tot + kTotalGuardSeen;
      float seen, pair;
      std::memcpy(&seen, &gs[kSeenMax], sizeof(seen));
      std::memcpy(&pair, &gs[kSeenPair], sizeof(pair));
      stats->guard_max_seen = std::max(stats->guard_max_seen, seen);
      stats->guard_pair_seen = std::max(stats->guard_pair_seen, pair);
      stats->guard_violations = std::max(stats->guard_violations, gs[kSeenViolations]);
      stats->guard_audit_mismatch = std::max(stats->guard_audit_mismatch, gs[kSeenAuditMismatch]);
      stats->guard_audited = std::max(stats->guard_audited, gs[kSeenAudited]);
    }
  }
  int32_t ovf = 0;
  HIP_TRY(c, hipMemcpy(&ovf, c->overflow.p, sizeof(int32_t), hipMemcpyDeviceToHost));
  stats->sampling_overflow = ovf;
  stats->batches = static_cast<int32_t>(nb);
  stats->shade_launches = static_cast<int32_t>(nb);
  stats->sample_launches = static_cast<int32_t>(nb);
  const adanerf_stats& f = c->folded;
  stats->total_samples += f.total_samples;
  stats->rays_refined += f.rays_refined;
  stats->guard_max_seen = std::max(stats->guard_max_seen, f.guard_max_seen);
  stats->guard_violations = std::max(stats->guard_violations, f.guard_violations);
  stats->guard_pair_seen = std::max(stats->guard_pair_seen, f.guard_pair_seen);
  stats->guard_audit_mismatch = std::max(stats->guard_audit_mismatch, f.guard_audit_mismatch);
  stats->guard_audited = std::max(stats->guard_audited, f.guard_audited);
  stats->guard_widened = c->guard_widened;
  stats->ms_total += f.ms_total;
  stats->ms_sample_mlp += f.ms_sample_mlp;
  stats->ms_compact += f.ms_compact;
  stats->ms_shade_mlp += f.ms_shade_mlp;
  stats->ms_composite += f.ms_composite;
  stats->batches += f.batches;
  stats->shade_launches += f.shade_launches;
  stats->sample_launches += f.sample_launches;
  return ADANERF_OK;
}

}

int adanerf_copy_result_sampling_network(adanerf_ctx* c, const float* d_oracle, int32_t n_rays, void* d_rgba8) {
  BIND(c);
  if (!d_oracle || !d_rgba8) return fail(c, ADANERF_EINVAL, "NULL buffer");
  if (n_rays < 0) return fail(c, ADANERF_EINVAL, "n_rays out of range");
  if (n_rays == 0) return ADANERF_OK;
  hipLaunchKernelGGL(oracle_view_kernel, dim3((n_rays + 3) / 4), dim3(256), 0, c->stream, d_oracle, n_rays, static_cast<uchar4*>(d_rgba8));
  HIP_RETURN(c, hipGetLastError());
}

int adanerf_render_oracle(adanerf_ctx* c, void* d_rgba8) {
  BIND(c);
  if (!d_rgba8) return fail(c, ADANERF_EINVAL, "NULL buffer");
  if (c->ms.coarse_fine) return fail(c, ADANERF_EUNSUPPORTED, "coarse/fine models have no sampling network to view");
  const int R = c->ms.info.rays_local, B = c->ms.info.batch_rays;
  int rc = ensure_batch_buffers(c, std::min(B, std::max(R, 1)), c->ms.info.num_samples);
  if (rc) return rc;
  float* rays = reinterpret_cast<float*>(c->rays.p);
  float* oracle = reinterpret_cast<float*>(c->oracle.p);
  for (int first = 0; first < R; first += B) {
    const int n = std::min(B, R - first);
    if ((rc = launch_sample_mlp(c, first, n, oracle, rays))) return rc;
    if ((rc = adanerf_copy_result_sampling_network(c, oracle, n, static_cast<char*>(d_rgba8) + static_cast<size_t>(first) * 4))) return rc;
  }
  return ADANERF_OK;
}

namespace {

void poll_guard(adanerf_ctx* c) {
  if (!c->guard_ev_pending) return;
  const hipError_t q = hipEventQuery(c->guard_ev);
  (void)hipGetLastError();
  if (q != hipSuccess) return;
  c->guard_ev_pending = false;
  float seen, pair;
  std::memcpy(&seen, &c->guard_host[kSeenMax], sizeof(seen));
  std::memcpy(&pair, &c->guard_host[kSeenPair], sizeof(pair));
  const int viol = c->guard_host[kSeenViolations], mism = c->guard_host[kSeenAuditMismatch];
  if (c->guard_ev_stale) {
    c->guard_ev_stale = false;
    c->guard_viol_seen = std::max(c->guard_viol_seen, viol);
    c->guard_mism_seen = std::max(c->guard_mism_seen, mism);
    return;
  }
  bool widened = false;
  if (viol > c->guard_viol_seen) {
    c->guard_viol_seen = viol;
    if (seen > c->guard_eps) {
      c->guard_eps = ADANERF_GUARD_CALIB_MARGIN * seen;
      c->guard_eps_pair = 2.0f * c->guard_eps;
      widened = true;
    } else if (pair > c->guard_eps_pair) {
      c->guard_eps_pair = ADANERF_GUARD_CALIB_MARGIN * pair;
      widened = true;
    }
  }
  if (mism > c->guard_mism_seen) {
    c->guard_mism_seen = mism;
    if (!widened) {
      c->guard_eps *= 2.0f;
      c->guard_eps_pair = 2.0f * c->guard_eps;
      widened = true;
    }
  }
  if (widened) {
    c->guard_eps_pair = std::min(std::max(c->guard_eps_pair, ADANERF_GUARD_EPS_MIN), 2.0f * c->guard_eps);
    c->ms.info.guard_eps = c->guard_eps;
    c->ms.info.guard_eps_pair = c->guard_eps_pair;
    c->ms.info.guard_calib_source = ADANERF_GUARD_FROM_MONITOR;
    ++c->guard_widened;
  }
}


int begin_record(adanerf_ctx* c, adanerf_stats* stats, int n_batches, bool* record_out) {
  int rc;
  if (stats && c->profiling && c->events_used) {
    HIP_TRY(c, hipStreamSynchronize(c->stream));
    reset_record(c);
  }
  const bool record = (stats || c->profiling) && static_cast<size_t>(n_batches) <= kMaxProfiledBatches;
  if (record && c->events_used && c->events_used / 5 + n_batches > kMaxProfiledBatches) {
    HIP_TRY(c, hipStreamSynchronize(c->stream));
    adanerf_stats part;
    if ((rc = sum_stats(c, &part))) return rc;
    c->folded = part;
    c->events_used = 0;
  }
  if (record) {
    const size_t need = c->events_used + static_cast<size_t>(n_batches) * 5;
    while (c->events.size() < need) {
      hipEvent_t e;
      HIP_TRY(c, hipEventCreate(&e));
      c->events.push_back(e);
    }
    while (c->pinned_totals.size() < need / 5) {
      int32_t* p = nullptr;
      HIP_TRY(c, hipHostMalloc(reinterpret_cast<void**>(&p), kTotalSlots * sizeof(int32_t), hipHostMallocDefault));
      std::memset(p, 0, kTotalSlots * sizeof(int32_t));
      c->pinned_totals.push_back(p);
    }
  }
  *record_out = record;
  return ADANERF_OK;
}

struct BatchOut {
  float* rgb;
  void* rgba8;
  float* depth;
  float* acc;
  float* disp;
};

int render_batch(adanerf_ctx* c, int first, int n, const RayList* list, const BatchOut& out, bool record) {
  const int B = c->ms.info.batch_rays, N = c->ms.info.num_samples;
  const float thr = c->ms.info.threshold;
  const bool budget = has_budget_map(c);
  int rc;
  float* rays = reinterpret_cast<float*>(c->rays.p);
  float* oracle = reinterpret_cast<float*>(c->oracle.p);
  int32_t* off = reinterpret_cast<int32_t*>(c->ray_offsets.p);
  const bool cfm = c->ms.coarse_fine;
  int32_t* cnt = reinterpret_cast<int32_t*>(c->ray_counts.p);
  uint32_t* key = reinterpret_cast<uint32_t*>(c->sample_key.p);
  float* sw = reinterpret_cast<float*>(c->sample_w.p);
  float* raw = reinterpret_cast<float*>(c->raw.p);
  int32_t* total = reinterpret_cast<int32_t*>(c->total.p);
  hipEvent_t* ev = record ? &c->events[c->events_used] : nullptr;
  if (ev) HIP_TRY(c, hipEventRecord(ev[0], c->stream));
  const bool pdf = c->ms.info.sampler_mode == ADANERF_SAMPLER_PDF || cfm;
  if (cfm) {
    uint32_t* keyc = reinterpret_cast<uint32_t*>(c->key_coarse.p);
    float* rawc = reinterpret_cast<float*>(c->raw_coarse.p);
    if ((rc = launch_camera_rays(c, first, n, rays))) return rc;
    if ((rc = launch_sample_uniform(c, n, c->ms.n_coarse, off, cnt, keyc, total))) return rc;
    if ((rc = launch_shade_mlp(c, rays, keyc, total, n * c->ms.n_coarse, c->ms.info.precision, rawc, nullptr, true))) return rc;
    if (ev) HIP_TRY(c, hipEventRecord(ev[1], c->stream));
    if ((rc = launch_sample_fine(c, rawc, rays, n, off, cnt, key, reinterpret_cast<float*>(c->sample_z.p), total))) return rc;
  }
  const bool fused = !pdf && thr > 0.f && use_pair_select(c, N) && c->sampling_mode != ADANERF_SAMPLING_FP32 && (!c->generic0 || generic_split_sampling(c)) &&
                     !(c->opt.flags & ADANERF_FLAG_KEEP_ORACLE);
  const SelectOut so = select_out(c, N, thr, cnt);
  const BudgetMaps bm{c->budget_n, c->budget_thr, first};
  const bool limited = c->depth_limit != nullptr;
  const bool capped = cap_trims(c) && !pdf && thr > 0.f;
  const int64_t cap_total = capped ? cap_total_of(c, n) : 0;
  const DepthLimit dl{c->depth_limit, first, list ? list->ids : nullptr, rays, c->ms.sp.ztab, depth_pose(c->ms.rg.pos, c->ms.rg.rot)};
  if (!cfm && (rc = launch_sample_mlp(c, first, n, fused ? nullptr : oracle, rays, fused ? &so : nullptr, list))) return rc;
  if (ev && !cfm) HIP_TRY(c, hipEventRecord(ev[1], c->stream));
  float* sz = reinterpret_cast<float*>(c->sample_z.p);
  if (cfm) rc = ADANERF_OK;
  else if (pdf) rc = launch_sample_pdf(c, oracle, n, N, off, cnt, key, sw, sz, total);
  else if (fused) {
    rc = budget ? launch_trim(c, bm, n, N, thr, kPairSegShift, cnt) : ADANERF_OK;
    if (!rc && limited) rc = launch_depth_limit(c, dl, n, N, kPairSegShift, cnt);
    if (!rc && capped) rc = launch_cap(c, n, N, thr, kPairSegShift, cnt, cap_total);
    if (!rc) rc = launch_expand(c, n, N, kPairSegShift, off, cnt, key, sw, total);
  }
  else if (thr == 0.f) {
    hipLaunchKernelGGL(dense_offsets_kernel, dim3((n + 255) / 256), dim3(256), 0, c->stream, n, off, cnt, total);
    HIP_TRY(c, hipGetLastError());
  } else rc = launch_compact(c, oracle, n, N, thr, off, cnt, key, sw, total, budget ? &bm : nullptr, limited ? &dl : nullptr, capped ? &cap_total : nullptr);
  if (rc) return rc;
  const bool dense_implicit = !cfm && !pdf && !fused && thr == 0.f;
  const uint32_t* key_s = dense_implicit ? nullptr : key;
  const float* sw_s = dense_implicit ? oracle : sw;
  if (ev) HIP_TRY(c, hipEventRecord(ev[2], c->stream));
  const int64_t max_s = static_cast<int64_t>(n) * N;
  if ((rc = launch_shade_mlp(c, rays, key_s, total, static_cast<int>(max_s), c->ms.info.precision, raw, pdf ? sz : nullptr))) return rc;
  if (ev) HIP_TRY(c, hipEventRecord(ev[3], c->stream));
  float* depth_b = out.depth;
  float* acc_b = out.acc;
  if (out.disp && (!depth_b || !acc_b)) {
    if ((rc = dev_alloc(c, &c->disp_scratch, static_cast<size_t>(B) * 2 * sizeof(float)))) return rc;
    if (!depth_b) depth_b = reinterpret_cast<float*>(c->disp_scratch.p);
    if (!acc_b) acc_b = reinterpret_cast<float*>(c->disp_scratch.p) + B;
  }
  if (pdf) rc = launch_composite_classic(c, raw, sz, rays, n, N, out.rgb, out.rgba8, depth_b, acc_b);
  else rc = launch_composite(c, raw, sw_s, off, cnt, n, out.rgb, out.rgba8, key_s, depth_b, acc_b);
  if (rc) return rc;
  if (out.disp && n > 0) {
    hipLaunchKernelGGL(disp_map_kernel, dim3((n + 255) / 256), dim3(256), 0, c->stream, depth_b, acc_b, n, out.disp);
    HIP_TRY(c, hipGetLastError());
  }
  if (ev) {
    HIP_TRY(c, hipEventRecord(ev[4], c->stream));
    HIP_TRY(c, hipMemcpyAsync(c->pinned_totals[c->events_used / 5], total, kTotalSlots * sizeof(int32_t), hipMemcpyDeviceToHost, c->stream));
    c->events_used += 5;
  }
  return ADANERF_OK;
}

int end_record(adanerf_ctx* c, adanerf_stats* stats, int n_batches, bool record, int rays) {
  if (record) c->prof_frames++;
  if (stats) {
    HIP_TRY(c, hipStreamSynchronize(c->stream));
    poll_guard(c);
    if (int rc = sum_stats(c, stats)) return rc;
    stats->rays = rays;
    if (n_batches > 0 && record) {
      const size_t e0 = c->events_used - static_cast<size_t>(n_batches) * 5;
      HIP_TRY(c, hipEventElapsedTime(&stats->ms_total, c->events[e0], c->events[c->events_used - 1]));
    }
    reset_record(c);
  }
  return ADANERF_OK;
}

}

int adanerf_render(adanerf_ctx* c, void* d_rgba8, float* d_rgb, adanerf_stats* stats) {
  BIND(c);
  poll_guard(c);
  const int R = c->ms.info.rays_local, B = c->ms.info.batch_rays, N = c->ms.info.num_samples;
  const int n_batches = R > 0 ? (R + B - 1) / B : 0;
  const bool budget = has_budget_map(c) || has_sample_cap(c);
  int rc = ensure_batch_buffers(c, std::min(B, std::max(R, 1)), N);
  if (rc) return rc;
  if (has_sample_cap(c)) c->cap_record_live = cap_trims(c);
  if (cap_trims(c)) {
    if ((rc = ensure_cap_buffers(c, std::min(B, std::max(R, 1))))) return rc;
    hipLaunchKernelGGL(cap_reset_kernel, dim3(1), dim3(1), 0, c->stream, reinterpret_cast<CapRecord*>(c->cap_record.p));
    HIP_TRY(c, hipGetLastError());
  }
  bool record = false;
  if ((rc = begin_record(c, stats, n_batches, &record))) return rc;
  int32_t* total = reinterpret_cast<int32_t*>(c->total.p);
  for (int b = 0; b < n_batches; ++b) {
    const int first = b * B, n = std::min(B, R - first);
    const BatchOut out{d_rgb ? d_rgb + static_cast<size_t>(first) * 3 : nullptr, d_rgba8 ? static_cast<char*>(d_rgba8) + static_cast<size_t>(first) * 4 : nullptr,
                       c->aux_depth ? c->aux_depth + first : nullptr, c->aux_acc ? c->aux_acc + first : nullptr, c->aux_disp ? c->aux_disp + first : nullptr};
    if ((rc = render_batch(c, first, n, nullptr, out, record))) return rc;
  }
  if (c->sampling_mode == ADANERF_SAMPLING_GUARDED && c->guard_mask.p && n_batches > 0 && !budget) ++c->guard_frame;
  if (c->sampling_mode == ADANERF_SAMPLING_GUARDED && c->guard_mask.p && n_batches > 0 && !budget && !c->guard_ev_pending) {
    if (!c->guard_host) {
      HIP_TRY(c, hipHostMalloc(reinterpret_cast<void**>(&c->guard_host), 8 * sizeof(int32_t)));
      std::memset(c->guard_host, 0, 8 * sizeof(int32_t));
      HIP_TRY(c, hipEventCreateWithFlags(&c->guard_ev, hipEventDisableTiming));
    }
    HIP_TRY(c, hipMemcpyAsync(c->guard_host, total + kTotalGuardSeen, kGuardSeenSlots * sizeof(int32_t), hipMemcpyDeviceToHost, c->stream));
    HIP_TRY(c, hipEventRecord(c->guard_ev, c->stream));
    c->guard_ev_pending = true;
  }
  return end_record(c, stats, n_batches, record, R);
}

namespace {

int ensure_mask_buffers(adanerf_ctx* c, int R, int n) {
  const size_t words = (static_cast<size_t>(R) + 31) / 32;
  if (c->mask_bits.bytes < words * sizeof(uint32_t) || c->ray_list.bytes < static_cast<size_t>(R) * sizeof(int32_t) || !c->ray_list_count.p || n > c->stage_cap) {
    HIP_TRY(c, hipStreamSynchronize(c->stream));
    n = std::max(n, c->stage_cap);
    const size_t S = static_cast<size_t>(n);
    int rc;
    if ((rc = dev_alloc(c, &c->mask_bits, std::max(words, size_t(4)) * sizeof(uint32_t)))) return rc;
    if ((rc = dev_alloc(c, &c->ray_list, static_cast<size_t>(std::max(R, 1)) * sizeof(int32_t)))) return rc;
    if ((rc = dev_alloc(c, &c->ray_list_count, 64))) return rc;
    if ((rc = dev_alloc(c, &c->stage_rgba8, std::max(S, size_t(1)) * 4))) return rc;
    if ((rc = dev_alloc(c, &c->stage_rgb, std::max(S, size_t(1)) * 3 * sizeof(float)))) return rc;
    if ((rc = dev_alloc(c, &c->stage_aux, std::max(S, size_t(1)) * 3 * sizeof(float)))) return rc;
    c->stage_cap = n;
  }
  return ADANERF_OK;
}

}

int adanerf_render_masked(adanerf_ctx* c, const uint8_t* d_mask, uint32_t values, void* d_rgba8, float* d_rgb, adanerf_stats* stats, int32_t* n_rendered) {
  if (!c) return ADANERF_EINVAL;
  if (!d_mask) return fail(c, ADANERF_EINVAL, "adanerf_render_masked: NULL mask");
  if (!d_rgba8 && !d_rgb) return fail(c, ADANERF_EINVAL, "adanerf_render_masked: both colour outputs NULL");
  if (values == 0) return fail(c, ADANERF_EINVAL, "adanerf_render_masked: values == 0 selects no mask byte");
  const int R = c->ms.info.rays_local, B = c->ms.info.batch_rays, N = c->ms.info.num_samples;
  const auto refuse = [&](const char* why) { return fail(c, ADANERF_EUNSUPPORTED, std::string("adanerf_render_masked: ") + why); };
  if (c->ms.coarse_fine) return refuse("the coarse / fine sampler has no ray list");
  if (c->ms.info.sampler_mode == ADANERF_SAMPLER_PDF) return refuse("the PDF sampler has no ray list");
  if (c->generic0) return refuse("run-time-shaped sampling networks have no ray list (the 8 x 256 network only)");
  if (c->sampling_mode != ADANERF_SAMPLING_SPLIT_FP16 && c->sampling_mode != ADANERF_SAMPLING_GUARDED)
    return refuse("sampling modes fp16 and fp32 have no ray list (split_fp16 or guarded only)");
  if (!(c->ms.info.threshold > 0.f)) return refuse("a dense context (threshold 0) has no fused selection");
  if (!use_pair_select(c, N) || (c->opt.flags & ADANERF_FLAG_KEEP_ORACLE))
    return refuse("the ray list needs the fused selection (N <= 16, neither ADANERF_FLAG_KEEP_ORACLE nor ADANERF_FLAG_WAVE_SELECT)");
  if (has_budget_map(c)) return refuse("a budget map is installed: its maps are indexed by frame position (remove it first)");
  if (has_sample_cap(c)) return refuse("a sample cap is installed: its threshold depends on which rays share a batch (adanerf_set_sample_cap(ctx, 0) removes it)");
  if (c->ms.rg.world != 1) return refuse("whole frames only (shard_world must be 1)");
  BIND(c);
  if (n_rendered) *n_rendered = 0;
  if (R <= 0) return ADANERF_OK;
  int rc = ensure_mask_buffers(c, R, 0);
  if (rc) return rc;
  const int n_words = (R + 31) / 32, n_halves = 2 * n_words;
  int32_t* ids = reinterpret_cast<int32_t*>(c->ray_list.p);
  int32_t* count = reinterpret_cast<int32_t*>(c->ray_list_count.p);
  hipLaunchKernelGGL(mask_bits_kernel, dim3((n_halves + 255) / 256), dim3(256), 0, c->stream, d_mask, R, values,
                     (reinterpret_cast<uintptr_t>(d_mask) & 15) == 0 ? 1 : 0, n_halves, reinterpret_cast<uint16_t*>(c->mask_bits.p));
  HIP_TRY(c, hipGetLastError());
  hipLaunchKernelGGL(refine_list_kernel, dim3((n_words + 255) / 256), dim3(256), 0, c->stream, reinterpret_cast<const uint32_t*>(c->mask_bits.p), n_words, R, 0, 0, 0,
                     0, ids, count);
  HIP_TRY(c, hipGetLastError());
  int32_t M = 0;
  HIP_TRY(c, hipMemcpyAsync(&M, count, sizeof(int32_t), hipMemcpyDeviceToHost, c->stream));
  HIP_TRY(c, hipStreamSynchronize(c->stream));
  if (M < 0 || M > R) return fail(c, ADANERF_EDEVICE, "adanerf_render_masked: the list count is outside 0..rays_local");
  if (n_rendered) *n_rendered = M;
  const int chunk = std::min(M, B), n_batches = M > 0 ? (M + B - 1) / B : 0;
  if (M > 0) {
    if ((rc = ensure_batch_buffers(c, chunk, N))) return rc;
    if ((rc = ensure_mask_buffers(c, R, chunk))) return rc;
    if (c->sampling_mode == ADANERF_SAMPLING_GUARDED)
      HIP_TRY(c, hipMemsetAsync(reinterpret_cast<int32_t*>(c->total.p) + kTotalRefined, 0, sizeof(int32_t), c->stream));
  }
  bool record = false;
  if ((rc = begin_record(c, stats, n_batches, &record))) return rc;
  const bool want_depth = c->aux_depth || c->aux_disp, want_acc = c->aux_acc || c->aux_disp;
  float* aux = reinterpret_cast<float*>(c->stage_aux.p);
  for (int b = 0; b < n_batches; ++b) {
    const int at = b * B, n = std::min(B, M - at);
    const RayList list{ids + at, count};
    const BatchOut out{d_rgb ? reinterpret_cast<float*>(c->stage_rgb.p) : nullptr, d_rgba8 ? c->stage_rgba8.p : nullptr, want_depth ? aux : nullptr,
                       want_acc ? aux + c->stage_cap : nullptr, c->aux_disp ? aux + 2 * static_cast<size_t>(c->stage_cap) : nullptr};
    if ((rc = render_batch(c, 0, n, &list, out, record))) return rc;
    MaskScatter s{};
    s.list = list.ids;
    s.rgba8 = static_cast<const uint32_t*>(out.rgba8);
    s.rgb = out.rgb;
    s.depth = out.depth;
    s.acc = out.acc;
    s.disp = out.disp;
    s.o_rgba8 = static_cast<uint32_t*>(d_rgba8);
    s.o_rgb = d_rgb;
    s.o_depth = c->aux_depth;
    s.o_acc = c->aux_acc;
    s.o_disp = c->aux_disp;
    hipLaunchKernelGGL(mask_scatter_kernel, dim3((n + 255) / 256), dim3(256), 0, c->stream, s, n);
    HIP_TRY(c, hipGetLastError());
  }
  return end_record(c, stats, n_batches, record, M);
}

int adanerf_set_aux_outputs(adanerf_ctx* c, float* d_depth_map, float* d_acc_map) {
  BIND(c);
  c->aux_depth = d_depth_map;
  c->aux_acc = d_acc_map;
  return ADANERF_OK;
}

int adanerf_set_disp_output(adanerf_ctx* c, float* d_disp_map) {
  BIND(c);
  c->aux_disp = d_disp_map;
  return ADANERF_OK;
}

int adanerf_set_budget_map(adanerf_ctx* c, const uint8_t* d_n_map, const float* d_thr_map) {
  BIND(c);
  if (d_n_map || d_thr_map) {
    if (c->ms.coarse_fine || c->ms.info.sampler_mode != ADANERF_SAMPLER_ADAPTIVE)
      return fail(c, ADANERF_EUNSUPPORTED, "per-ray budgets trim the adaptive selection: this model's sampler has none");
    if (c->ms.info.dense) return fail(c, ADANERF_EUNSUPPORTED, "threshold 0 (dense) keeps every bin: there is no selection to trim");
  }
  if (c->sampling_mode == ADANERF_SAMPLING_GUARDED && (d_n_map || d_thr_map) && !has_budget_map(c) && c->total.p)
    HIP_TRY(c, hipMemsetAsync(reinterpret_cast<int32_t*>(c->total.p) + kTotalRefined, 0, sizeof(int32_t), c->stream));
  c->budget_n = d_n_map;
  c->budget_thr = d_thr_map;
  return ADANERF_OK;
}

int adanerf_foveate(adanerf_ctx* c, float gaze_x, float gaze_y, int32_t n_rings, const int32_t* radius_px, const int32_t* n, const float* thr,
                    uint8_t* d_n_map, float* d_thr_map) {
  if (!c) return ADANERF_EINVAL;
  if (!std::isfinite(gaze_x) || !std::isfinite(gaze_y)) return fail(c, ADANERF_EINVAL, "adanerf_foveate: the gaze must be finite");
  if (n_rings < 0 || n_rings > kFoveaMaxRings) return fail(c, ADANERF_EINVAL, "adanerf_foveate: n_rings must be in 0.." + std::to_string(kFoveaMaxRings));
  if ((n_rings > 0 && !radius_px) || !n || !thr) return fail(c, ADANERF_EINVAL, "adanerf_foveate: NULL array");
  FoveaParams f{};
  for (int k = 0; k < n_rings; ++k) {
    if (radius_px[k] < 0 || (k > 0 && radius_px[k] <= radius_px[k - 1]))
      return fail(c, ADANERF_EINVAL, "adanerf_foveate: radii must be >= 0 and strictly ascending");
    const uint64_t d = 2ull * static_cast<uint64_t>(radius_px[k]);
    f.r2x4[k] = d * d;
  }
  for (int k = 0; k <= n_rings; ++k) {
    if (n[k] < 0 || n[k] > 255) return fail(c, ADANERF_EINVAL, "adanerf_foveate: every n must be in 0..255");
    if (std::isnan(thr[k])) return fail(c, ADANERF_EINVAL, "adanerf_foveate: a threshold is not a number");
    f.n[k] = static_cast<uint8_t>(n[k]);
    f.thr[k] = thr[k];
  }
  for (int k = n_rings; k < kFoveaMaxRings; ++k) {
    f.r2x4[k] = ~0ull;
    f.n[k + 1] = f.n[n_rings];
    f.thr[k + 1] = f.thr[n_rings];
  }
  auto half_px = [](float g) { return static_cast<int64_t>(std::lrintf(std::min(std::max(2.0f * g, -2147483648.0f), 2147483648.0f))); };
  f.gx2 = half_px(gaze_x);
  f.gy2 = half_px(gaze_y);
  BIND(c);
  const int R = c->ms.info.rays_local;
  if (R <= 0 || (!d_n_map && !d_thr_map)) return ADANERF_OK;
  hipLaunchKernelGGL(foveate_kernel, dim3((R + 255) / 256), dim3(256), 0, c->stream, c->ms.rg, f, R, d_n_map, d_thr_map);
  HIP_RETURN(c, hipGetLastError());
}

int adanerf_compact_budget(adanerf_ctx* c, const float* d_oracle, int32_t n_rays, int32_t n_max, float thr, const uint8_t* d_n_map,
                           const float* d_thr_map, int32_t* d_off, int32_t* d_cnt, uint32_t* d_key, float* d_w, int32_t* d_total) {
  BIND(c);
  if (!d_oracle || !d_off || !d_cnt || !d_key || !d_w || !d_total) return fail(c, ADANERF_EINVAL, "NULL buffer");
  if (n_rays < 0 || n_max < 1 || n_max > kBins || !(thr > 0.f)) return fail(c, ADANERF_EINVAL, "n_rays/n_max/thr out of range (thr must be > 0: the dense mode selects nothing)");
  if (static_cast<int64_t>(n_rays) >= (1ll << 25)) return fail(c, ADANERF_EINVAL, "n_rays must be < 2^25 per batch");
  if (static_cast<int64_t>(n_rays) * n_max > 0x7fffffffll) return fail(c, ADANERF_EINVAL, "n_rays * n_max exceeds 2^31 - 1");
  if (int rc = ensure_compact_scratch(c, n_rays, n_max)) return rc;
  const BudgetMaps bm{d_n_map, d_thr_map, 0};
  return launch_compact(c, d_oracle, n_rays, n_max, thr, d_off, d_cnt, d_key, d_w, d_total, &bm);
}

int adanerf_set_depth_limit(adanerf_ctx* c, const float* d_limit_zc) {
  if (!c) return ADANERF_EINVAL;
  if (d_limit_zc) {
    if (c->ms.coarse_fine || c->ms.info.sampler_mode != ADANERF_SAMPLER_ADAPTIVE)
      return fail(c, ADANERF_EUNSUPPORTED, "adanerf_set_depth_limit: a depth limit trims the adaptive selection: this model's sampler has none");
    if (c->ms.info.use_ndc) return fail(c, ADANERF_EUNSUPPORTED, "adanerf_set_depth_limit: the samples of a useNDC model live in NDC space, not along the camera's viewing axis");
    if (c->ms.info.dense) return fail(c, ADANERF_EUNSUPPORTED, "adanerf_set_depth_limit: threshold 0 (dense) keeps every bin with implicit keys: there is no selection to trim");
    if (reinterpret_cast<uintptr_t>(d_limit_zc) & 3) return fail(c, ADANERF_EINVAL, "adanerf_set_depth_limit: the map must be 4-byte aligned");
  }
  c->depth_limit = d_limit_zc;
  return ADANERF_OK;
}

int adanerf_compact_depth_limit(adanerf_ctx* c, const float* d_oracle, int32_t n_rays, int32_t n_max, float thr, const float* d_rays,
                                const float* d_limit_zc, const float pos[3], const float rot[9], int32_t* d_off, int32_t* d_cnt, uint32_t* d_key,
                                float* d_w, int32_t* d_total) {
  BIND(c);
  if (!d_oracle || !d_rays || !d_limit_zc || !pos || !rot || !d_off || !d_cnt || !d_key || !d_w || !d_total) return fail(c, ADANERF_EINVAL, "NULL buffer");
  if (n_rays < 0 || n_max < 1 || n_max > kBins || !(thr > 0.f)) return fail(c, ADANERF_EINVAL, "n_rays/n_max/thr out of range (thr must be > 0: the dense mode selects nothing)");
  if (static_cast<int64_t>(n_rays) >= (1ll << 25)) return fail(c, ADANERF_EINVAL, "n_rays must be < 2^25 per batch");
  if (static_cast<int64_t>(n_rays) * n_max > 0x7fffffffll) return fail(c, ADANERF_EINVAL, "n_rays * n_max exceeds 2^31 - 1");
  if ((reinterpret_cast<uintptr_t>(d_rays) & 15) || (reinterpret_cast<uintptr_t>(d_limit_zc) & 3))
    return fail(c, ADANERF_EINVAL, "d_rays must be 16-byte aligned, d_limit_zc 4-byte aligned");
  if (!c->ms.sp.ztab) return fail(c, ADANERF_EUNSUPPORTED, "adanerf_compact_depth_limit: this context has no depth table");
  if (int rc = ensure_compact_scratch(c, n_rays, n_max)) return rc;
  const DepthLimit dl{d_limit_zc, 0, nullptr, d_rays, c->ms.sp.ztab, depth_pose(pos, rot)};
  return launch_compact(c, d_oracle, n_rays, n_max, thr, d_off, d_cnt, d_key, d_w, d_total, nullptr, &dl);
}

int adanerf_set_sample_cap(adanerf_ctx* c, float mean_samples_per_ray) {
  BIND(c);
  const float cap = mean_samples_per_ray;
  if (cap != 0.f && !(std::isfinite(cap) && cap >= 1.f))
    return fail(c, ADANERF_EINVAL, "adanerf_set_sample_cap: the cap must be 0 (off) or a finite mean of at least 1 sample per ray");
  if (cap != 0.f) {
    if (c->ms.coarse_fine || c->ms.info.sampler_mode != ADANERF_SAMPLER_ADAPTIVE)
      return fail(c, ADANERF_EUNSUPPORTED, "adanerf_set_sample_cap: a cap trims the adaptive selection: this model's sampler has none");
    if (c->ms.info.dense) return fail(c, ADANERF_EUNSUPPORTED, "adanerf_set_sample_cap: threshold 0 (dense) keeps every bin: there is no selection to trim");
  }
  if (c->sampling_mode == ADANERF_SAMPLING_GUARDED && cap != 0.f && !has_sample_cap(c) && c->total.p)
    HIP_TRY(c, hipMemsetAsync(reinterpret_cast<int32_t*>(c->total.p) + kTotalRefined, 0, sizeof(int32_t), c->stream));
  c->sample_cap = cap == 0.f ? 0.f : cap;
  return ADANERF_OK;
}

int adanerf_sample_cap_report(adanerf_ctx* c, adanerf_cap_report* out) {
  BIND(c);
  if (!out) return fail(c, ADANERF_EINVAL, "adanerf_sample_cap_report: out == NULL");
  CapRecord r{};
  r.thr_max = -INFINITY;
  if (c->cap_record.p && c->cap_record_live) {
    HIP_TRY(c, hipMemcpyAsync(&r, c->cap_record.p, sizeof(r), hipMemcpyDeviceToHost, c->stream));
    HIP_TRY(c, hipStreamSynchronize(c->stream));
  }
  out->threshold_max = r.thr_max;
  out->batches_trimmed = r.batches_trimmed;
  out->samples_selected = r.selected;
  out->samples_kept = r.kept;
  return ADANERF_OK;
}

int adanerf_compact_cap(adanerf_ctx* c, const float* d_oracle, int32_t n_rays, int32_t n_max, float thr, const uint8_t* d_n_map, const float* d_thr_map,
                        const float* d_rays, const float* d_limit_zc, const float pos[3], const float rot[9], int64_t cap_total, int32_t* d_off,
                        int32_t* d_cnt, uint32_t* d_key, float* d_w, int32_t* d_total, float* d_tstar) {
  BIND(c);
  if (!d_oracle || !d_off || !d_cnt || !d_key || !d_w || !d_total || !d_tstar) return fail(c, ADANERF_EINVAL, "NULL buffer");
  if (n_rays < 0 || n_max < 1 || n_max > kBins || !(thr > 0.f)) return fail(c, ADANERF_EINVAL, "n_rays/n_max/thr out of range (thr must be > 0: the dense mode selects nothing)");
  if (static_cast<int64_t>(n_rays) >= (1ll << 25)) return fail(c, ADANERF_EINVAL, "n_rays must be < 2^25 per batch");
  if (static_cast<int64_t>(n_rays) * n_max > 0x7fffffffll) return fail(c, ADANERF_EINVAL, "n_rays * n_max exceeds 2^31 - 1");
  if (cap_total < n_rays) return fail(c, ADANERF_EINVAL, "adanerf_compact_cap: cap_total must be at least n_rays (every non-empty row keeps one entry)");
  if (d_limit_zc) {
    if (!d_rays || !pos || !rot) return fail(c, ADANERF_EINVAL, "adanerf_compact_cap: a depth limit needs d_rays, pos and rot");
    if ((reinterpret_cast<uintptr_t>(d_rays) & 15) || (reinterpret_cast<uintptr_t>(d_limit_zc) & 3))
      return fail(c, ADANERF_EINVAL, "d_rays must be 16-byte aligned, d_limit_zc 4-byte aligned");
    if (!c->ms.sp.ztab) return fail(c, ADANERF_EUNSUPPORTED, "adanerf_compact_cap: this context has no depth table");
  }
  if (int rc = ensure_compact_scratch(c, n_rays, n_max)) return rc;
  if (int rc = ensure_cap_buffers(c, n_rays)) return rc;
  c->cap_record_live = true;
  const BudgetMaps bm{d_n_map, d_thr_map, 0};
  const DepthLimit dl = d_limit_zc ? DepthLimit{d_limit_zc, 0, nullptr, d_rays, c->ms.sp.ztab, depth_pose(pos, rot)} : DepthLimit{};
  hipLaunchKernelGGL(cap_reset_kernel, dim3(1), dim3(1), 0, c->stream, reinterpret_cast<CapRecord*>(c->cap_record.p));
  HIP_TRY(c, hipGetLastError());
  if (int rc = launch_compact(c, d_oracle, n_rays, n_max, thr, d_off, d_cnt, d_key, d_w, d_total, (d_n_map || d_thr_map) ? &bm : nullptr,
                              d_limit_zc ? &dl : nullptr, &cap_total))
    return rc;
  HIP_RETURN(c, hipMemcpyAsync(d_tstar, c->cap_record.p, sizeof(float), hipMemcpyDeviceToDevice, c->stream));
}

int adanerf_set_stream(adanerf_ctx* c, void* hip_stream) {
  BIND(c);
  HIP_TRY(c, hipStreamSynchronize(c->stream));
  c->stream = hip_stream ? reinterpret_cast<hipStream_t>(hip_stream) : c->own_stream;
  return ADANERF_OK;
}

int adanerf_set_profiling(adanerf_ctx* c, int32_t enabled) {
  BIND(c);
  HIP_TRY(c, hipStreamSynchronize(c->stream));
  c->profiling = enabled != 0;
  reset_record(c);
  return ADANERF_OK;
}

int adanerf_collect_stats(adanerf_ctx* c, adanerf_stats* stats, int32_t* frames) {
  if (!c || !stats) return ADANERF_EINVAL;
  BIND(c);
  HIP_TRY(c, hipStreamSynchronize(c->stream));
  if (int rc = sum_stats(c, stats)) return rc;
  stats->rays = c->ms.info.rays_local;
  if (frames) *frames = c->prof_frames;
  reset_record(c);
  return ADANERF_OK;
}

int adanerf_assemble_strips(adanerf_ctx* c, const void* d_gathered, void* d_image) {
  BIND(c);
  if (!d_gathered || !d_image) return fail(c, ADANERF_EINVAL, "NULL buffer");
  const int n = c->ms.info.width * c->ms.info.height;
  hipLaunchKernelGGL(assemble_strips_kernel, dim3((n + 255) / 256), dim3(256), 0, c->stream, reinterpret_cast<const uchar4*>(d_gathered),
                     reinterpret_cast<uchar4*>(d_image), c->ms.info.width, c->ms.info.height, c->ms.rg.strip_rows, c->ms.rg.world, c->ms.info.rays_local_max);
  HIP_RETURN(c, hipGetLastError());
}

int adanerf_gather_to(adanerf_ctx* dst, void* d_dst, adanerf_ctx* src, const void* d_src, size_t bytes) {
  if (!dst || !src) return ADANERF_EINVAL;
  if (!d_dst || !d_src) return fail(dst, ADANERF_EINVAL, "NULL buffer");
  if (bytes == 0) return ADANERF_OK;
  adanerf_ctx* c = src;
  BIND(src);
  if (src->device != dst->device) {
    if (dst->device < 64 && !((src->peer_tried >> dst->device) & 1)) {
      src->peer_tried |= 1ull << dst->device;
      int can = 0;
      if (hipDeviceCanAccessPeer(&can, src->device, dst->device) == hipSuccess && can)
        (void)hipDeviceEnablePeerAccess(dst->device, 0);
      (void)hipGetLastError();
    }
    HIP_TRY(c, hipMemcpyPeerAsync(d_dst, dst->device, d_src, src->device, bytes, src->stream));
  } else {
    HIP_TRY(c, hipMemcpyAsync(d_dst, d_src, bytes, hipMemcpyDeviceToDevice, src->stream));
  }
  if (src == dst || src->stream == dst->stream) return ADANERF_OK;
  if (!src->peer_event) HIP_TRY(c, hipEventCreateWithFlags(&src->peer_event, hipEventDisableTiming));
  HIP_TRY(c, hipEventRecord(src->peer_event, src->stream));
  c = dst;
  BIND(dst);
  HIP_RETURN(c, hipStreamWaitEvent(dst->stream, src->peer_event, 0));
}

int adanerf_probe_mfma(adanerf_ctx* c, int32_t operands, int32_t f16, float target_ms, float* tflops, float* clock_mhz) {
  BIND(c);
  if (operands < 0 || operands > 3 || !(target_ms > 0.f) || target_ms > 5000.f || !tflops || !clock_mhz)
    return fail(c, ADANERF_EINVAL, "operands must be 0..3, target_ms in (0, 5000], outputs non-NULL");
  HIP_TRY(c, hipStreamSynchronize(c->stream));
  double tf = 0, mhz = 0;
  HIP_TRY(c, probe_mfma_rate(operands, f16 != 0, target_ms, c->ms.info.compute_units, c->stream, &tf, &mhz));
  *tflops = static_cast<float>(tf);
  *clock_mhz = static_cast<float>(mhz);
  return ADANERF_OK;
}

int adanerf_malloc(adanerf_ctx* c, size_t bytes, void** d_out) {
  if (!c || !d_out) return ADANERF_EINVAL;
  BIND(c);
  HIP_RETURN(c, hipMalloc(d_out, bytes ? bytes : 1));
}
int adanerf_free(adanerf_ctx* c, void* d_ptr) {
  BIND(c);
  HIP_TRY(c, hipStreamSynchronize(c->stream));
  HIP_RETURN(c, hipFree(d_ptr));
}
int adanerf_memcpy_h2d(adanerf_ctx* c, void* d_dst, const void* src, size_t bytes) {
  BIND(c);
  HIP_TRY(c, hipMemcpyAsync(d_dst, src, bytes, hipMemcpyHostToDevice, c->stream));
  HIP_RETURN(c, hipStreamSynchronize(c->stream));
}
int adanerf_memcpy_d2h(adanerf_ctx* c, void* dst, const void* d_src, size_t bytes) {
  BIND(c);
  HIP_TRY(c, hipMemcpyAsync(dst, d_src, bytes, hipMemcpyDeviceToHost, c->stream));
  HIP_RETURN(c, hipStreamSynchronize(c->stream));
}

int adanerf_get_buffer(adanerf_ctx* c, int32_t which, void** d_out, size_t* bytes_out) {
  if (!c || !d_out) return ADANERF_EINVAL;
  DevBuf* b = nullptr;
  switch (which) {
    case ADANERF_BUF_RAYS: b = &c->rays; break;
    case ADANERF_BUF_ORACLE: b = &c->oracle; break;
    case ADANERF_BUF_RAY_OFFSETS: b = &c->ray_offsets; break;
    case ADANERF_BUF_RAY_COUNTS: b = &c->ray_counts; break;
    case ADANERF_BUF_SAMPLE_KEY: b = &c->sample_key; break;
    case ADANERF_BUF_SAMPLE_W: b = &c->sample_w; break;
    case ADANERF_BUF_RAW: b = &c->raw; break;
    case ADANERF_BUF_TOTAL: b = &c->total; break;
    case ADANERF_BUF_SAMPLE_Z: b = &c->sample_z; break;
    case ADANERF_BUF_RAW_COARSE: b = &c->raw_coarse; break;
    case ADANERF_BUF_RAY_LIST: b = &c->ray_list; break;
    case ADANERF_BUF_RAY_LIST_COUNT: b = &c->ray_list_count; break;
    default: return fail(c, ADANERF_EINVAL, "unknown buffer id");
  }
  *d_out = b->p;
  if (bytes_out) *bytes_out = b->bytes;
  return ADANERF_OK;
}

}
```

adanerf_amd/csrc/context.hpp:

```cpp
#pragma once
#include "../../include/adanerf_hip.h"

#include <hip/hip_runtime.h>

#include <string>
#include <utility>
#include <vector>

#include "k_common.hip.hpp"
#include "launch.hpp"
#include "model_setup.hpp"

namespace adanerf {

struct DevBuf {
  void* p = nullptr;
  size_t bytes = 0;
  DevBuf() = default;
  DevBuf(DevBuf&& o) noexcept { *this = std::move(o); }
  DevBuf& operator=(DevBuf&& o) noexcept { return std::swap(p, o.p), std::swap(bytes, o.bytes), *this; }
  ~DevBuf() {
    if (p) (void)hipFree(p);
  }
};

struct PackedDev {
  DevBuf w, b;
  NetParams params{};
};

int fail(adanerf_ctx* c, int code, const std::string& msg);
int hip_rc(adanerf_ctx* c, hipError_t e, const char* what);
int dev_alloc(adanerf_ctx* c, DevBuf* b, size_t bytes);

struct StageScratch {
  DevBuf flip_tab, flip_partial, flip_mean;
  double flip_ppd = 0.0;
  FlipParams flip_params{};
  bool flip_lds_raised = false;
  DevBuf zbuf;
  DevBuf gather_surface;
  DevBuf count;
  DevBuf upsample_zp;
};

}

struct adanerf_ctx {
  adanerf_options opt{};
  adanerf::ModelSetup ms;
  std::string err;
  hipStream_t stream = nullptr;
  hipStream_t own_stream = nullptr;
  adanerf::GridCache grids;
  std::vector<hipEvent_t> events;
  size_t events_used = 0;
  bool profiling = false;
  int prof_frames = 0;
  std::vector<int32_t*> pinned_totals;
  int32_t* guard_host = nullptr;
  hipEvent_t guard_ev = nullptr;
  bool guard_ev_pending = false;
  int guard_viol_seen = 0;
  int guard_mism_seen = 0;
  bool guard_ev_stale = false;
  int guard_widened = 0;
  uint32_t guard_frame = 0;
  int debug_guard = 0;
  std::string model_dir;
  uint64_t model0_hash = 0;
  adanerf_stats folded{};

  adanerf::NetTopology topo0, topo1;
  bool generic0 = false, generic1 = false;
  int enc0 = adanerf::kEnc10_4, enc1 = adanerf::kEnc10_4;
  adanerf::GenericTopo gen0{}, gen1{};
  adanerf::DevBuf rsi_z;

  adanerf::PackedDev net0;
  adanerf::PackedDev net0_split;
  adanerf::PackedDev net0_f16;
  adanerf::TensorMap net0_host;
  int sampling_mode = 0;
  adanerf::DevBuf overflow;
  adanerf::PackedDev net1[3];
  adanerf::TensorMap net1_host;
  adanerf::DevBuf ztab;
  adanerf::PackedDev netc[3];
  adanerf::NetTopology topoc;
  bool genericc = false;
  adanerf::GenericTopo genc{};
  adanerf::ShadeParams spc{};
  adanerf::DevBuf ztab_coarse, raw_coarse, key_coarse;

  int cap_rays = 0, cap_nmax = 0;
  adanerf::DevBuf rays, oracle, ray_offsets, ray_counts, selbin, selw, block_total, block_offset, total;
  adanerf::DevBuf sample_key, sample_w, raw, sample_z;
  adanerf::DevBuf guard_mask, refine_list, guard_probe;
  float guard_eps = 0.f;
  float guard_eps_pair = 0.f;
  int guard_audit_period = 0;
  int device = 0;
  float* aux_depth = nullptr;
  float* aux_acc = nullptr;
  float* aux_disp = nullptr;
  const uint8_t* budget_n = nullptr;
  const float* budget_thr = nullptr;
  const float* depth_limit = nullptr;
  float sample_cap = 0.f;
  adanerf::DevBuf cap_state;
  adanerf::DevBuf cap_record;
  bool cap_record_live = false;
  adanerf::DevBuf cap_map;
  adanerf::DevBuf disp_scratch;
  adanerf::StageScratch stages;
  adanerf::DevBuf mask_bits, ray_list, ray_list_count, stage_rgba8, stage_rgb, stage_aux;
  int stage_cap = 0;
  float px_dx = 0.f, px_dy = 0.f;
  hipEvent_t peer_event = nullptr;
  uint64_t peer_tried = 0;
};

#define HIP_TRY(ctx, call) do { if (int rc_ = adanerf::hip_rc(ctx, (call), #call)) return rc_; } while (0)
#define HIP_RETURN(ctx, call) return adanerf::hip_rc(ctx, (call), #call)
#define BIND(ctx) do { if (!(ctx)) return ADANERF_EINVAL; HIP_TRY(ctx, hipSetDevice((ctx)->device)); } while (0)
```

adanerf_amd/csrc/k_compact.hip.hpp:

```cpp
#pragma once
#include "k_common.hip.hpp"
#include "tuning.hpp"
#include "k_select_pair.hip.hpp"

namespace adanerf {


using tune::kSelRaysPerBlock;
static_assert(kSelRaysPerBlock == 32 || kSelRaysPerBlock == 64, "segment must fit one wave");
constexpr int kSelSegShift = kSelRaysPerBlock == 64 ? 6 : 5;
constexpr float kFltMax = __FLT_MAX__;

__device__ __forceinline__ void select_ray(float v0, float v1, int lane, int n_max, float thr, uint64_t* s0, uint64_t* s1) {
  const uint64_t b0 = __ballot(v0 >= thr), b1 = __ballot(v1 >= thr);
  const int c = __popcll(b0) + __popcll(b1);
  uint64_t sel0, sel1;
  if (c <= n_max && c > 0) {
    sel0 = b0;
    sel1 = b1;
  } else {
    const float m = wave_max_f32(fmaxf(v0, v1));
    const uint64_t e0 = __ballot(v0 == m), e1 = __ballot(v1 == m);
    if (c == 0) {
      sel0 = e0 & (~e0 + 1);
      sel1 = e0 ? 0 : (e1 & (~e1 + 1));
      if ((sel0 | sel1) == 0) sel0 = 1;
    } else {
      float lo = thr, hi = m;
      uint64_t g0 = e0, g1 = e1;
      int ch = __popcll(e0) + __popcll(e1);
      uint64_t t0 = b0, t1 = b1;
      if (m == INFINITY && ch < n_max) {
        const uint64_t f0 = __ballot(v0 >= kFltMax), f1 = __ballot(v1 >= kFltMax);
        const int cf = __popcll(f0) + __popcll(f1);
        if (cf <= n_max) {
          hi = kFltMax;
          g0 = f0;
          g1 = f1;
          ch = cf;
        } else {
          lo = kFltMax;
          t0 = f0;
          t1 = f1;
        }
      }
      while (ch < n_max) {
        const float mid = lo + (hi - lo) * 0.5f;
        if (!(mid > lo) || !(mid < hi)) break;
        const uint64_t m0 = __ballot(v0 >= mid), m1 = __ballot(v1 >= mid);
        const int cm = __popcll(m0) + __popcll(m1);
        if (cm > n_max) {
          lo = mid;
          t0 = m0;
          t1 = m1;
        } else {
          hi = mid;
          g0 = m0;
          g1 = m1;
          ch = cm;
        }
      }
      if (ch >= n_max) {
        if (ch == n_max) {
          sel0 = g0;
          sel1 = g1;
        } else {
          g0 = 0;
          g1 = 0;
          ch = 0;
          t0 = e0;
          t1 = e1;
          goto tie;
        }
      } else {
      tie:
        const uint64_t q0 = t0 & ~g0, q1 = t1 & ~g1;
        const int need = n_max - ch;
        const int r0 = mbcnt64(q0), r1 = __popcll(q0) + mbcnt64(q1);
        const uint64_t k0 = __ballot(((q0 >> lane) & 1) && r0 < need), k1 = __ballot(((q1 >> lane) & 1) && r1 < need);
        sel0 = g0 | k0;
        sel1 = g1 | k1;
      }
    }
  }
  *s0 = sel0;
  *s1 = sel1;
}

__device__ __forceinline__ float wave_sum_all_f32(float v) { return wave_sum_dpp_f32(v); }

__device__ __forceinline__ void oracle_transform_wave(int transform, float* v0, float* v1) {
  if (transform == kOracleSigmoid) {
    *v0 = 1.0f / (1.0f + expf(-*v0));
    *v1 = 1.0f / (1.0f + expf(-*v1));
  } else if (transform == kOracleSoftmax) {
    const float m = wave_max_f32(fmaxf(*v0, *v1));
    const float e0 = expf(*v0 - m), e1 = expf(*v1 - m);
    const float s = wave_sum_all_f32(e0 + e1);
    *v0 = e0 / s;
    *v1 = e1 / s;
  }
}

__global__ __launch_bounds__(256) void select_kernel(const float* __restrict__ oracle, int n_rays, int n_max, float thr, int transform,
                                                     int32_t* __restrict__ counts, uint8_t* __restrict__ selbin,
                                                     float* __restrict__ selw, int32_t* __restrict__ block_total) {
  __shared__ int wave_tot[4];
  constexpr int RPW = kSelRaysPerBlock / 4;
  const int lane = lane_id();
  const int wave = static_cast<int>(threadIdx.x) >> 6;
  const int base = blockIdx.x * kSelRaysPerBlock + wave * RPW;
  int total = 0;
  float n0[4], n1[4];
  auto fetch = [&](int i) {
#pragma unroll
    for (int u = 0; u < 4; ++u) {
      const int r = base + i + u;
      const float* row = oracle + static_cast<size_t>(r < n_rays ? r : 0) * kBins;
      n0[u] = row[lane];
      n1[u] = row[64 + lane];
    }
  };
  fetch(0);
#pragma unroll
  for (int i = 0; i < RPW; i += 4) {
    float v0[4], v1[4];
#pragma unroll
    for (int u = 0; u < 4; ++u) {
      v0[u] = n0[u];
      v1[u] = n1[u];
    }
    if (i + 4 < RPW) fetch(i + 4);
#pragma unroll
    for (int u = 0; u < 4; ++u) {
      const int r = base + i + u;
      if (r >= n_rays) break;
      uint64_t s0, s1;
      oracle_transform_wave(transform, &v0[u], &v1[u]);
      select_ray(v0[u], v1[u], lane, n_max, thr, &s0, &s1);
      const int c0 = __popcll(s0);
      const int cnt = c0 + __popcll(s1);
      const size_t o = static_cast<size_t>(r) * n_max;
      if ((s0 >> lane) & 1) {
        const int rank = mbcnt64(s0);
        selbin[o + rank] = static_cast<uint8_t>(lane);
        selw[o + rank] = v0[u];
      }
      if ((s1 >> lane) & 1) {
        const int rank = c0 + mbcnt64(s1);
        selbin[o + rank] = static_cast<uint8_t>(64 + lane);
        selw[o + rank] = v1[u];
      }
      if (lane == 0) counts[r] = cnt;
      total += cnt;
    }
  }
  if (lane == 0) wave_tot[wave] = total;
  __syncthreads();
  if (threadIdx.x == 0) block_total[blockIdx.x] = wave_tot[0] + wave_tot[1] + wave_tot[2] + wave_tot[3];
}

__global__ __launch_bounds__(256) void select_rows_kernel(const float* __restrict__ oracle, int n_rays, SelectOut so,
                                                          const int32_t* __restrict__ n_list = nullptr) {
  __shared__ __attribute__((aligned(16))) char lds[4 * kPairLdsBytesPerWave];
  const int lane = lane_id();
  const int wave = static_cast<int>(threadIdx.x) >> 6;
  const int j = lane & 31, h = lane >> 5;
  const int first = (blockIdx.x * 4 + wave) * 32;
  if (n_list) n_rays = min(n_rays, *n_list);
  if (first >= n_rays) return;
  const int local = first + j;
  const bool valid = local < n_rays;
  const int lidx = valid ? local : n_rays - 1;
  const int entry = n_list ? so.refine_list[lidx] : 0;
  const float* row = oracle + static_cast<size_t>(n_list ? (entry & kRefineRayMask) : lidx) * kBins;
  float x[64];
#pragma unroll
  for (int m = 0; m < 4; ++m)
#pragma unroll
    for (int g = 0; g < 4; ++g) {
      const float4 v = *reinterpret_cast<const float4*>(row + 32 * m + 8 * g + 4 * h);
      x[16 * m + 4 * g + 0] = v.x;
      x[16 * m + 4 * g + 1] = v.y;
      x[16 * m + 4 * g + 2] = v.z;
      x[16 * m + 4 * g + 3] = v.w;
    }
  const uint32_t stage = static_cast<uint32_t>(reinterpret_cast<uintptr_t>(lds)) + wave * kPairLdsBytesPerWave + lane * 16;
  bool bad = false;
  if (so.guard_mask) {
    float z = 0.f;
#pragma unroll
    for (int i = 0; i < 64; ++i) z = __builtin_fmaf(x[i], 0.f, z);
    bad = (z != z) | (pair_xchg(static_cast<uint32_t>(z != z)) != 0u);
  }
  GuardAcc gacc;
  pair_epilogue(x, lane, local, valid, stage, so, bad, entry, &gacc);
  if (n_list) guard_flush(so, gacc, lane);
}

__global__ __launch_bounds__(256) void max_abs_diff_kernel(const float* __restrict__ a, const float* __restrict__ b, size_t n, uint32_t* __restrict__ out) {
  float m = 0.f;
  bool bad = false;
  for (size_t i = static_cast<size_t>(blockIdx.x) * blockDim.x + threadIdx.x; i < n; i += static_cast<size_t>(gridDim.x) * blockDim.x) {
    const float d = fabsf(a[i] - b[i]);
    if (d == d && d < INFINITY) m = fmaxf(m, d);
    else bad = true;
  }
  m = wave_max_nonneg(m);
  const uint64_t anybad = __ballot(bad);
  if ((threadIdx.x & 63) == 0) {
    if (m > 0.f) atomicMax(&out[0], __builtin_bit_cast(uint32_t, m));
    if (anybad) atomicAdd(&out[1], 1u);
  }
}

__global__ __launch_bounds__(256) void guard_stats_kernel(const float* __restrict__ y, const float* __restrict__ x, int n_rays, int n_max, float thr,
                                                          float two_eps, uint32_t* __restrict__ out) {
  const int lane = lane_id();
  const int r = blockIdx.x * 4 + (static_cast<int>(threadIdx.x) >> 6);
  if (r >= n_rays) return;
  const float* yr = y + static_cast<size_t>(r) * kBins;
  const float* xr = x + static_cast<size_t>(r) * kBins;
  const float y0 = yr[lane], y1 = yr[64 + lane];
  const float d0 = y0 - xr[lane], d1 = y1 - xr[64 + lane];
  const bool f0 = fabsf(d0) < INFINITY, f1 = fabsf(d1) < INFINITY;
  const float ma = wave_max_f32(fmaxf(f0 ? fabsf(d0) : 0.f, f1 ? fabsf(d1) : 0.f));
  const uint64_t bad = __ballot(!f0 || !f1);
  float mp = 0.f;
  if (two_eps > 0.f && !bad) {
    float a0 = y0, a1 = y1, c0 = 0.f, tn = 0.f;
    for (int k = 0; k < n_max; ++k) {
      const float m = wave_max_f32(fmaxf(a0, a1));
      if (k == 0) c0 = m;
      tn = m;
      const uint64_t e0 = __ballot(a0 == m), e1 = __ballot(a1 == m);
      if (e0) {
        if (lane == __builtin_ctzll(e0)) a0 = -INFINITY;
      } else if (lane == __builtin_ctzll(e1)) a1 = -INFINITY;
    }
    const bool none = c0 < thr;
    const float t = none ? c0 : fmaxf(tn, thr);
    const float cut = none ? c0 - two_eps : fmaxf(tn - two_eps, thr - 0.5f * two_eps);
    const float dk = wave_max_f32(fmaxf(y0 >= t ? d0 : -INFINITY, y1 >= t ? d1 : -INFINITY));
    const float dn = -wave_max_f32(fmaxf((y0 >= cut && y0 < t) ? -d0 : -INFINITY, (y1 >= cut && y1 < t) ? -d1 : -INFINITY));
    const float pr = dk - dn;
    mp = (pr > 0.f && pr < INFINITY) ? pr : 0.f;
  }
  if (lane == 0) {
    if (ma > 0.f) atomicMax(&out[0], __builtin_bit_cast(uint32_t, ma));
    if (bad) atomicAdd(&out[1], 1u);
    if (mp > 0.f) atomicMax(&out[2], __builtin_bit_cast(uint32_t, mp));
  }
}

__global__ __launch_bounds__(1024) void scan_blocks_kernel(const int32_t* __restrict__ block_total, int n_blocks,
                                                           int32_t* __restrict__ block_offset, int32_t* __restrict__ total) {
  __shared__ int part[1024];
  const int t = threadIdx.x;
  const int per = (n_blocks + 1023) / 1024;
  const int lo = t * per;
  int s = 0;
  for (int i = 0; i < per; ++i) {
    const int k = lo + i;
    if (k < n_blocks) s += block_total[k];
  }
  part[t] = s;
  __syncthreads();
  for (int off = 1; off < 1024; off <<= 1) {
    int v = (t >= off) ? part[t - off] : 0;
    __syncthreads();
    part[t] += v;
    __syncthreads();
  }
  int run = part[t] - s;
  for (int i = 0; i < per; ++i) {
    const int k = lo + i;
    if (k < n_blocks) {
      block_offset[k] = run;
      run += block_total[k];
    }
  }
  if (t == 1023) *total = part[1023];
}

template <bool INLINE_SCAN>
__global__ __launch_bounds__(256) void expand_kernel(const int32_t* __restrict__ counts, const uint8_t* __restrict__ selbin,
                                                     const float* __restrict__ selw, const int32_t* __restrict__ block_offset,
                                                     const int32_t* __restrict__ block_total, int n_blocks, int n_rays, int n_max,
                                                     int seg_shift, int32_t* __restrict__ ray_offsets, uint32_t* __restrict__ sample_key,
                                                     float* __restrict__ sample_w, int32_t* __restrict__ total) {
  const int segs = 256 >> seg_shift;
  const int t = static_cast<int>(threadIdx.x);
  const int r = blockIdx.x * 256 + t;
  const int c = (r < n_rays) ? counts[r] : 0;
  const int x = seg_shift == 5 ? wave_incl_sum_dpp_i32<32>(c) : wave_incl_sum_dpp_i32<64>(c);
  const int seg = r >> seg_shift;
  int seg_base;
  if (INLINE_SCAN) {
    __shared__ int part[4];
    const int b0 = blockIdx.x * segs;
    int s = 0;
    for (int i = t; i < b0; i += 256) s += block_total[i];
    s = wave_sum_dpp_i32(s);
    if ((t & 63) == 0) part[t >> 6] = s;
    __syncthreads();
    seg_base = part[0] + part[1] + part[2] + part[3];
    for (int i = b0; i < seg && i < n_blocks; ++i) seg_base += block_total[i];
    if (blockIdx.x == gridDim.x - 1 && t == 0) {
      int tot = part[0] + part[1] + part[2] + part[3];
      for (int i = b0; i < n_blocks; ++i) tot += block_total[i];
      *total = tot;
    }
  } else {
    seg_base = (seg < n_blocks) ? block_offset[seg] : 0;
  }
  if (r >= n_rays) return;
  const int o = seg_base + x - c;
  ray_offsets[r] = o;
  const size_t src = static_cast<size_t>(r) * n_max;
  for (int k = 0; k < c; ++k) {
    sample_key[o + k] = (static_cast<uint32_t>(r) << 7) | selbin[src + k];
    sample_w[o + k] = selw[src + k];
  }
}

struct RefinePlan {
  int tot_und, tot_aud, budget, offset;
};
__device__ __forceinline__ int refine_accepted_before(const RefinePlan& p, int pa) {
  if (p.budget >= p.tot_aud) return pa;
  const int wrap = p.offset + p.budget - p.tot_aud;
  if (wrap <= 0) return min(max(pa - p.offset, 0), p.budget);
  return min(pa, wrap) + max(pa - p.offset, 0);
}
__device__ __forceinline__ bool refine_accepts(const RefinePlan& p, int pa) {
  if (p.budget >= p.tot_aud) return true;
  int d = pa - p.offset;
  if (d < 0) d += p.tot_aud;
  return d < p.budget;
}
__global__ __launch_bounds__(256) void refine_list_kernel(const uint32_t* __restrict__ mask, int n_words, int n_rays, int period, int phase,
                                                          int cap_round, int cycle, int32_t* __restrict__ list, int32_t* __restrict__ count) {
  __shared__ int red[4][4], wtot[2][4];
  const int t = static_cast<int>(threadIdx.x);
  const int b0 = blockIdx.x * 256;
  auto word = [&](int i, uint32_t m, uint32_t* und, uint32_t* aud) {
    const int left = n_rays - i * 32;
    const uint32_t in_range = left >= 32 ? 0xFFFFFFFFu : (left > 0 ? low_bits32(left) : 0u);
    const uint32_t u = m & in_range;
    *und = u;
    *aud = audit_bits(period, phase, i) & ~u & in_range;
  };
  int s[4] = {0, 0, 0, 0};
  auto tally = [&](int i, uint32_t m) {
    uint32_t u, a;
    word(i, m, &u, &a);
    const int cu = __popc(u), ca = __popc(a);
    if (i < b0) {
      s[0] += cu;
      s[1] += ca;
    }
    s[2] += cu;
    s[3] += ca;
  };
  const int n_quads = n_words >> 2;
  const uint4* __restrict__ mask4 = reinterpret_cast<const uint4*>(mask);
#pragma unroll 2
  for (int q = t; q < n_quads; q += 256) {
    const uint4 v = mask4[q];
    tally(4 * q, v.x);
    tally(4 * q + 1, v.y);
    tally(4 * q + 2, v.z);
    tally(4 * q + 3, v.w);
  }
  for (int i = 4 * n_quads + t; i < n_words; i += 256) tally(i, mask[i]);
#pragma unroll
  for (int k = 0; k < 4; ++k) s[k] = wave_sum_dpp_i32(s[k]);
  const int wi = b0 + t;
  uint32_t und = 0u, aud = 0u;
  if (wi < n_words) word(wi, mask[wi], &und, &aud);
  const int cu = __popc(und), ca = __popc(aud);
  const int xu = wave_incl_sum_dpp_i32<64>(cu), xa = wave_incl_sum_dpp_i32<64>(ca);
  if ((t & 63) == 63) {
    wtot[0][t >> 6] = xu;
    wtot[1][t >> 6] = xa;
  }
  if ((t & 63) == 0) {
#pragma unroll
    for (int k = 0; k < 4; ++k) red[k][t >> 6] = s[k];
  }
  __syncthreads();
  int tot[4];
#pragma unroll
  for (int k = 0; k < 4; ++k) tot[k] = red[k][0] + red[k][1] + red[k][2] + red[k][3];
  RefinePlan p;
  p.tot_und = tot[2];
  p.tot_aud = tot[3];
  p.budget = p.tot_aud;
  p.offset = 0;
  if (cap_round > 0) {
    const int rounds = max(1, (p.tot_und + cap_round - 1) / cap_round);
    int room = max(0, rounds * cap_round - p.tot_und);
    if (room < (p.tot_aud + 3) / 4) room += cap_round;
    p.budget = min(p.tot_aud, room);
    if (p.budget > 0 && p.budget < p.tot_aud) p.offset = static_cast<int>((static_cast<long long>(cycle) * p.budget) % p.tot_aud);
  }
  int pu = tot[0] + xu - cu, pa = tot[1] + xa - ca;
  for (int w = 0; w < (t >> 6); ++w) {
    pu += wtot[0][w];
    pa += wtot[1][w];
  }
  for (uint32_t r = und | aud; r; r &= r - 1u) {
    const int bit = __builtin_ctz(r);
    const int ray = wi * 32 + bit;
    if ((und >> bit) & 1u) {
      list[pu + refine_accepted_before(p, pa)] = ray;
      ++pu;
    } else {
      if (refine_accepts(p, pa)) list[pu + refine_accepted_before(p, pa)] = ray | kRefineAuditBit;
      ++pa;
    }
  }
  if (blockIdx.x == 0 && t == 0) *count = p.tot_und + p.budget;
}

__global__ __launch_bounds__(256) void oracle_view_kernel(const float* __restrict__ oracle, int n_rays, uchar4* __restrict__ rgba8) {
  const int lane = lane_id();
  const int r = blockIdx.x * 4 + (static_cast<int>(threadIdx.x) >> 6);
  if (r >= n_rays) return;
  const float* row = oracle + static_cast<size_t>(r) * kBins;
  float v0 = row[lane], v1 = row[64 + lane];
  int bin[3];
#pragma unroll
  for (int k = 0; k < 3; ++k) {
    const float m = wave_max_f32(fmaxf(v0, v1));
    const uint64_t e0 = __ballot(v0 == m), e1 = __ballot(v1 == m);
    int b = k;
    if (e0) b = __builtin_ctzll(e0);
    else if (e1) b = 64 + __builtin_ctzll(e1);
    bin[k] = b;
    if (b == lane) v0 = -INFINITY;
    if (b == 64 + lane) v1 = -INFINITY;
  }
  if (lane == 0) {
    uchar4 px;
    px.x = static_cast<unsigned char>((0.5f + static_cast<float>(bin[0])) / 128.0f * 255.0f);
    px.y = static_cast<unsigned char>((0.5f + static_cast<float>(bin[1])) / 128.0f * 255.0f);
    px.z = static_cast<unsigned char>((0.5f + static_cast<float>(bin[2])) / 128.0f * 255.0f);
    px.w = 255;
    rgba8[r] = px;
  }
}

__global__ __launch_bounds__(256) void dense_offsets_kernel(int n_rays, int32_t* __restrict__ ray_offsets, int32_t* __restrict__ counts,
                                                            int32_t* __restrict__ total) {
  const int r = blockIdx.x * blockDim.x + threadIdx.x;
  if (r == 0) *total = n_rays * kBins;
  if (r >= n_rays) return;
  ray_offsets[r] = r * kBins;
  counts[r] = kBins;
}

__global__ __launch_bounds__(256) void dense_expand_kernel(const float* __restrict__ oracle, int n_rays, int32_t* __restrict__ ray_offsets,
                                                           int32_t* __restrict__ counts, uint32_t* __restrict__ sample_key,
                                                           float* __restrict__ sample_w, int32_t* __restrict__ total) {
  const size_t i = static_cast<size_t>(blockIdx.x) * blockDim.x + threadIdx.x;
  const size_t n = static_cast<size_t>(n_rays) * kBins;
  if (i == 0) *total = static_cast<int32_t>(n);
  if (i >= n) return;
  sample_key[i] = static_cast<uint32_t>(i);
  sample_w[i] = oracle[i];
  if ((i & (kBins - 1)) == 0) {
    const int r = static_cast<int>(i >> 7);
    ray_offsets[r] = static_cast<int32_t>(i);
    counts[r] = kBins;
  }
}

}
```

adanerf_amd/csrc/k_mlp16.hip.hpp:

```cpp
#pragma once
#include "k_common.hip.hpp"
#include "k_mlp_f32.hip.hpp"
#include "tuning.hpp"
#include <utility>

namespace adanerf {


struct ShadeArgs {
  ShadeParams sp;
  NetParams net;
  const float* rays;
  const uint32_t* sample_key;
  const float* sample_z;
  const int32_t* total;
  int32_t max_samples;
  float* raw_out;
  float pos_limit;
};

__device__ __forceinline__ uint64_t position_outside(const ShadeArgs& a, const float x[3]) {
  const float m = __builtin_elementwise_maximum(__builtin_elementwise_maximum(fabsf(x[0]), fabsf(x[1])), fabsf(x[2]));
  uint64_t mask = __builtin_amdgcn_ballot_w64(!(m <= a.pos_limit));
  asm volatile("" : "+s"(mask));
  return mask;
}
__device__ __forceinline__ bool outside_lane(uint64_t mask) { return __builtin_amdgcn_inverse_ballot_w64(mask); }

__device__ __forceinline__ void store_raw(const ShadeArgs& a, int s, float r, float g, float b, float alpha, bool outside) {
  const float ks = a.net.out_scale[1], q = __builtin_nanf("");
  *reinterpret_cast<float4*>(a.raw_out + static_cast<size_t>(s) * 4) =
      make_float4(outside ? q : r * ks, outside ? q : g * ks, outside ? q : b * ks, outside ? q : alpha * a.net.out_scale[0]);
}
__device__ __forceinline__ void store_raw_f32(const ShadeArgs& a, int s, float r, float g, float b, float alpha, bool outside) {
  const float q = __builtin_nanf("");
  *reinterpret_cast<float4*>(a.raw_out + static_cast<size_t>(s) * 4) = make_float4(outside ? q : r, outside ? q : g, outside ? q : b, outside ? q : alpha);
}

struct Bf16 {
  static constexpr bool kClampRelu = true;
  typedef bf16x8 vec8;
  static __device__ __forceinline__ uint32_t pack(float lo, float hi) {
    f32x2 v = {lo, hi};
    return __builtin_bit_cast(uint32_t, __builtin_convertvector(v, bf16x2));
  }
  static __device__ __forceinline__ f32x16 mfma(u32x4 a, u32x4 b, f32x16 c) {
    return __builtin_amdgcn_mfma_f32_32x32x16_bf16(__builtin_bit_cast(bf16x8, a), __builtin_bit_cast(bf16x8, b), c, 0, 0, 0);
  }
};
struct Fp16 {
  static constexpr bool kClampRelu = false;
  typedef f16x8 vec8;
  static __device__ __forceinline__ uint32_t pack(float lo, float hi) {
    f32x2 v = {lo, hi};
    return __builtin_bit_cast(uint32_t, __builtin_convertvector(v, f16x2));
  }
  static __device__ __forceinline__ f32x16 mfma(u32x4 a, u32x4 b, f32x16 c) {
    return __builtin_amdgcn_mfma_f32_32x32x16_f16(__builtin_bit_cast(f16x8, a), __builtin_bit_cast(f16x8, b), c, 0, 0, 0);
  }
};

using tune::kRegFrags;
constexpr int kShadeFrags16 = 32 + 4 * 128 + 160 + 2 * 128 + 144 + 72 + 8;
constexpr int kShadeBiasFloats = 8 * 256 + 288 + 128 + 32;

template <int CF, int RS, int LPW, int NR = kRegFrags>
struct WStream {
  static constexpr int kRegs = NR;
  static constexpr int kChunk = CF;
  static constexpr int kChunkBytes = CF * 1024;
#if defined(__HIP_DEVICE_COMPILE__)
  __amdgpu_buffer_rsrc_t rsrc;
#endif
  const char* gbase;
  uint32_t gbytes;
  uint32_t goff;
  uint32_t lane_off;
  uint32_t wave_off;
  uint32_t slot_cur;
  uint32_t rd_cur;
  uint32_t rd_next;
  uint32_t lds_base;
  uint32_t grp;
  uint32_t issuer;
  uint32_t dma_lds;
  uint32_t dma_goff;
  bool stag;
  u32x4 R[NR];
};

__device__ __forceinline__ u32x4 lds_read128(uint32_t byte_addr) {
  typedef const __attribute__((address_space(3))) u32x4* lds_u32x4_ptr;
  return *((lds_u32x4_ptr)(uintptr_t)byte_addr);
}

template <int CF, int RS, int LPW, int NR>
__device__ __forceinline__ void ws_piece(WStream<CF, RS, LPW, NR>& st, int i) {
  static_assert(LPW >= 1 && LPW <= 8, "a piece is addressed by the 12-bit immediate offset of buffer_load ... lds (pieces 4 .. 7: a second base)");
#if defined(__HIP_DEVICE_COMPILE__)
  typedef __attribute__((address_space(3))) void* lds_ptr;
  const uint32_t far = i >= 4 ? 4096u : 0u;
  lds_ptr dst = (lds_ptr) static_cast<uintptr_t>(st.dma_lds + far);
  const int voff = static_cast<int>(st.lane_off), soff = static_cast<int>(st.dma_goff + far);
  if (tune::kAblateDmaBytes) {
    if ((i & 3) == 0) __builtin_amdgcn_raw_ptr_buffer_load_lds(st.rsrc, dst, 4, voff, soff, 0, 0);
    else if ((i & 3) == 1) __builtin_amdgcn_raw_ptr_buffer_load_lds(st.rsrc, dst, 4, voff, soff, 1024, 0);
    else if ((i & 3) == 2) __builtin_amdgcn_raw_ptr_buffer_load_lds(st.rsrc, dst, 4, voff, soff, 2048, 0);
    else __builtin_amdgcn_raw_ptr_buffer_load_lds(st.rsrc, dst, 4, voff, soff, 3072, 0);
    return;
  }
  if ((i & 3) == 0) __builtin_amdgcn_raw_ptr_buffer_load_lds(st.rsrc, dst, 16, voff, soff, 0, 0);
  else if ((i & 3) == 1) __builtin_amdgcn_raw_ptr_buffer_load_lds(st.rsrc, dst, 16, voff, soff, 1024, 0);
  else if ((i & 3) == 2) __builtin_amdgcn_raw_ptr_buffer_load_lds(st.rsrc, dst, 16, voff, soff, 2048, 0);
  else __builtin_amdgcn_raw_ptr_buffer_load_lds(st.rsrc, dst, 16, voff, soff, 3072, 0);
#endif
}

template <int CF, int RS, int LPW, int NR>
__device__ __forceinline__ void ws_chunk_begin(WStream<CF, RS, LPW, NR>& st, uint32_t slot) {
  st.dma_lds = st.lds_base + slot * (CF * 1024) + st.wave_off;
  st.dma_goff = st.goff + st.wave_off;
  st.goff += CF * 1024;
  if (st.goff >= st.gbytes) st.goff = 0;
}

template <int CF, int RS, int LPW, int NR>
__device__ __forceinline__ void ws_issue(WStream<CF, RS, LPW, NR>& st, uint32_t slot) {
  ws_chunk_begin(st, slot);
#pragma unroll
  for (int i = 0; i < LPW; ++i) ws_piece(st, i);
}

__device__ __forceinline__ void ws_skip_pad() {
  asm volatile("s_nop %0" ::"n"(tune::kSkipPad) : "memory");
}

template <int ABL, int CF, int RS, int LPW, int NR>
__device__ __forceinline__ void ws_sync(WStream<CF, RS, LPW, NR>& st, bool pad, int piece) {
  static_assert(RS >= 3 && (RS - 2) * LPW < 64, "vmcnt is a 6-bit counter");
  if (ABL & 1) return;
  if (!(ABL & 32)) asm volatile("s_waitcnt vmcnt(%0)\n\ts_barrier" ::"n"((RS - 3) * LPW) : "memory");
  const uint32_t slot = (st.grp == 0) ? st.slot_cur : (st.slot_cur == 0 ? RS - 1 : st.slot_cur - 1);
  if (!(ABL & 16)) {
    if (st.issuer) {
      ws_chunk_begin(st, slot);
      ws_piece(st, piece);
    } else if (pad) ws_skip_pad();
  }
}

template <int CF, int RS, int LPW, int NR>
__device__ __forceinline__ void ws_advance(WStream<CF, RS, LPW, NR>& st) {
  st.slot_cur = (st.slot_cur + 1 == RS) ? 0 : st.slot_cur + 1;
  const uint32_t nxt = (st.slot_cur + 1 == RS) ? 0 : st.slot_cur + 1;
  st.rd_cur = st.rd_next;
  st.rd_next = st.lds_base + nxt * (CF * 1024) + st.lane_off;
}


template <int ABL, int CF, int RS, int LPW, int NR>
__device__ __forceinline__ void ws_position(WStream<CF, RS, LPW, NR>& st, int f, bool tile_start) {
  constexpr int STEP = RS == 3 ? CF / LPW / 2 : CF / LPW;
  static_assert(CF % LPW == 0 && STEP >= 1 && (RS == 3 || (CF / 2) % STEP == 0), "piece positions: both groups' synchronisation points are piece positions");
  const bool pad = tile_start;
  const bool piece_pos = f % STEP == 0 && f / STEP < LPW && !(ABL & (1 | 16));
  if (f == 0) {
    if (ABL & 1) return;
    if (st.grp == 0) ws_sync<ABL>(st, pad, 0);
    else {
      if (pad) ws_skip_pad();
      if (piece_pos && st.issuer) ws_piece(st, 0);
    }
    ws_advance(st);
  } else if (f == CF / 2 && st.stag) {
    if (st.grp != 0) ws_sync<ABL>(st, pad, (CF / 2) / STEP);
    else {
      if (pad) ws_skip_pad();
      if (piece_pos && st.issuer) ws_piece(st, (CF / 2) / STEP);
    }
  } else if (piece_pos) {
    if (st.issuer) ws_piece(st, f / STEP);
  }
}

template <int ABL, int CF, int RS, int LPW, int NR>
__device__ __forceinline__ void ws_refill(WStream<CF, RS, LPW, NR>& st, int p) {
  if (ABL & 2) {
    asm volatile("" : "+v"(st.R[p % NR]));
    return;
  }
  const int q = p + NR;
  st.R[p % NR] = (q < CF) ? lds_read128(st.rd_cur + q * 1024) : lds_read128(st.rd_next + (q - CF) * 1024);
}

template <int CF, int RS, int LPW, int NR>
__device__ __forceinline__ void ws_start(WStream<CF, RS, LPW, NR>& st, const void* gbase, uint32_t gbytes, char* lds, int wave, int lane,
                                         int grp = -1, bool issuer = true) {
  st.stag = grp >= 0;
  st.grp = grp > 0 ? 1u : 0u;
  st.issuer = issuer;
  st.gbase = reinterpret_cast<const char*>(gbase);
  st.gbytes = gbytes;
#if defined(__HIP_DEVICE_COMPILE__)
  st.rsrc = __builtin_amdgcn_make_buffer_rsrc(const_cast<void*>(gbase), 0, static_cast<int>(gbytes), 0x00020000);
#endif
  st.goff = 0;
  st.lane_off = lane * 16;
  st.wave_off = wave * LPW * 1024;
  st.lds_base = static_cast<uint32_t>(reinterpret_cast<uintptr_t>(lds));
  if (issuer) {
#pragma unroll
    for (int k = 0; k < RS - 1; ++k) ws_issue(st, k);
  }
  asm volatile("s_waitcnt vmcnt(%0)\n\ts_barrier" ::"n"((RS - 2) * LPW) : "memory");
  st.slot_cur = RS - 1;
  st.rd_cur = st.lds_base + st.lane_off;
  st.rd_next = st.lds_base + st.lane_off;
#pragma unroll
  for (int i = 0; i < NR; ++i) st.R[i] = lds_read128(st.rd_next + i * 1024);
}

__device__ __forceinline__ float relu_keep_nan(float x) { return __builtin_elementwise_maximum(x, 0.0f); }

template <class ET, int F>
__device__ __forceinline__ void pe_pack(const float x[3], int h, uint32_t* out) {
  float t[pe_slots(F)];
  pe_eval<F, false>(x, h, t);
#pragma unroll
  for (int q = 0; q < pe_slots(F) / 2; ++q) out[q] = ET::pack(t[2 * q], t[2 * q + 1]);
}

struct BiasRegs {
  f32x4 b0, b1, b2, b3;
};
__device__ __forceinline__ void lds_bias_issue(uint32_t byte_addr, BiasRegs& r, uint32_t& rd0, uint32_t& rd1) {
  asm volatile("ds_read_b128 %0, %6\n\tds_read_b128 %1, %6 offset:16\n\tds_read_b128 %2, %6 offset:32\n\tds_read_b128 %3, %6 offset:48"
               : "=&v"(r.b0), "=&v"(r.b1), "=&v"(r.b2), "=&v"(r.b3), "+v"(rd0), "+v"(rd1)
               : "v"(byte_addr));
}
template <int YOUNGER = 0>
__device__ __forceinline__ void lds_bias_take(BiasRegs& r, f32x16* acc) {
  asm volatile("s_waitcnt lgkmcnt(%4)" : "+v"(r.b0), "+v"(r.b1), "+v"(r.b2), "+v"(r.b3) : "n"(YOUNGER > 15 ? 15 : YOUNGER));
  f32x16 a;
#pragma unroll
  for (int e = 0; e < 4; ++e) {
    a[e] = r.b0[e];
    a[4 + e] = r.b1[e];
    a[8 + e] = r.b2[e];
    a[12 + e] = r.b3[e];
  }
  *acc = a;
}

__device__ __forceinline__ void lds_bias16(uint32_t byte_addr, f32x16* acc) {
  f32x4 b0, b1, b2, b3;
  asm volatile("ds_read_b128 %0, %4\n\tds_read_b128 %1, %4 offset:16\n\tds_read_b128 %2, %4 offset:32\n\tds_read_b128 %3, %4 offset:48"
               : "=&v"(b0), "=&v"(b1), "=&v"(b2), "=&v"(b3)
               : "v"(byte_addr));
  asm volatile("s_waitcnt lgkmcnt(0)" : "+v"(b0), "+v"(b1), "+v"(b2), "+v"(b3));
  f32x16 a;
#pragma unroll
  for (int e = 0; e < 4; ++e) {
    a[e] = b0[e];
    a[4 + e] = b1[e];
    a[8 + e] = b2[e];
    a[12 + e] = b3[e];
  }
  *acc = a;
}

template <class ET, bool RELU>
__device__ __forceinline__ int mfma_guard(const f32x16& acc) {
  if constexpr (RELU && ET::kClampRelu) return __builtin_amdgcn_readfirstlane(__builtin_bit_cast(int, acc[15]));
  else return 0;
}

template <class ET, bool RELU>
__device__ __forceinline__ void epilogue_quad_16(const f32x16& acc, int m, int g, uint32_t* out, int guard = 0) {
  if constexpr (RELU && ET::kClampRelu) {
    uint32_t q0, q1;
    asm("v_cvt_pk_bf16_f32 %0, %1, %2 clamp\n\t; after the accumulator's guard %3" : "=v"(q0) : "v"(acc[4 * g + 0]), "v"(acc[4 * g + 1]), "s"(guard));
    asm("v_cvt_pk_bf16_f32 %0, %1, %2 clamp\n\t; after the accumulator's guard %3" : "=v"(q1) : "v"(acc[4 * g + 2]), "v"(acc[4 * g + 3]), "s"(guard));
    out[8 * m + 2 * g + 0] = q0;
    out[8 * m + 2 * g + 1] = q1;
    return;
  }
  uint32_t p0 = ET::pack(acc[4 * g + 0], acc[4 * g + 1]), p1 = ET::pack(acc[4 * g + 2], acc[4 * g + 3]);
  if (RELU) {
    if constexpr (std::is_same_v<ET, Fp16>) {
      const f16x2 z = {static_cast<_Float16>(0.f), static_cast<_Float16>(0.f)};
      p0 = __builtin_bit_cast(uint32_t, __builtin_elementwise_maximum(__builtin_bit_cast(f16x2, p0), z));
      p1 = __builtin_bit_cast(uint32_t, __builtin_elementwise_maximum(__builtin_bit_cast(f16x2, p1), z));
    } else {
      const s16x2 z = {0, 0};
      p0 = __builtin_bit_cast(uint32_t, __builtin_elementwise_max(__builtin_bit_cast(s16x2, p0), z));
      p1 = __builtin_bit_cast(uint32_t, __builtin_elementwise_max(__builtin_bit_cast(s16x2, p1), z));
    }
  }
  out[8 * m + 2 * g + 0] = p0;
  out[8 * m + 2 * g + 1] = p1;
}

constexpr int kKeepAllF32 = -2;


template <class ET, class WS, int S1, int S2, int MT, bool RELU, int FPOS, int KEEP_F32_TILE = -1>
__device__ __forceinline__ void layer_16(WS& st, uint32_t bias_addr, int lane, const uint32_t* in1, const uint32_t* in2,
                                         uint32_t* out, f32x16* keep = nullptr) {
  constexpr int CF = WS::kChunk;
  constexpr int KS = S1 + S2;
#pragma unroll
  for (int m = 0; m < MT; ++m) {
    f32x16 acc;
    if (tune::kAblateShade & 4) {
#pragma unroll
      for (int r = 0; r < 16; ++r) acc[r] = 0.f;
    } else {
      lds_bias16(bias_addr + m * 128, &acc);
    }
#pragma unroll
    for (int s = 0; s < KS; ++s) {
      const int f = (FPOS + m * KS + s) % CF;
      ws_position<tune::kAblateShade>(st, f, s == 0);
      const uint32_t* src = (s < S1) ? (in1 + 4 * s) : (in2 + 4 * (s - S1));
      u32x4 b = {src[0], src[1], src[2], src[3]};
      acc = ET::mfma(st.R[f % WS::kRegs], b, acc);
      ws_refill<tune::kAblateShade>(st, f);
    }
    if (KEEP_F32_TILE == kKeepAllF32) {
      keep[m] = acc;
    } else if (KEEP_F32_TILE == m) {
      *keep = acc;
    } else if (tune::kAblateShade & 8) {
      asm volatile("" ::"v"(acc));
#pragma unroll
      for (int g = 0; g < 8; ++g) asm volatile("" : "=v"(out[8 * m + g]));
    } else {
      const int gd = mfma_guard<ET, RELU>(acc);
#pragma unroll
      for (int g = 0; g < 4; ++g) epilogue_quad_16<ET, RELU>(acc, m, g, out, gd);
    }
  }
}

__device__ __forceinline__ uint64_t load_sample(const ShadeArgs& a, int s, int total, float x[3], float dpe[3]) {
  const int si = (s < total) ? s : (total > 0 ? total - 1 : 0);
  const uint32_t key = a.sample_key ? a.sample_key[si] : static_cast<uint32_t>(si);
  const uint32_t ray = key >> 7;
  const int bin = static_cast<int>(key & 127u);
  const float4* rr = reinterpret_cast<const float4*>(a.rays + static_cast<size_t>(ray) * 8);
  const float4 o4 = rr[0], d4 = rr[1];
  const float o[3] = {o4.x, o4.y, o4.z}, d[3] = {d4.x, d4.y, d4.z};
  sample_position(a.sp, o, d, a.sample_z ? a.sample_z[si] : a.sp.ztab[bin], x);
  if (a.sp.unit_dir) unit3(d, dpe);
  else {
    dpe[0] = d[0];
    dpe[1] = d[1];
    dpe[2] = d[2];
  }
  return position_outside(a, x);
}

template <int NQ>
__device__ __forceinline__ void lds_stash_write(uint32_t byte_addr, const uint32_t* v) {
#pragma unroll
  for (int g = 0; g < NQ; ++g) {
    const u32x4 t = {v[4 * g], v[4 * g + 1], v[4 * g + 2], v[4 * g + 3]};
    asm volatile("ds_write_b128 %0, %1" ::"v"(byte_addr + g * 1024), "v"(t) : "memory");
  }
}
template <int NQ>
__device__ __forceinline__ void lds_stash_read(uint32_t byte_addr, uint32_t* v) {
  u32x4 t[NQ];
#pragma unroll
  for (int g = 0; g < NQ; ++g) asm volatile("ds_read_b128 %0, %1" : "=&v"(t[g]) : "v"(byte_addr + g * 1024));
  if (NQ == 4) asm volatile("s_waitcnt lgkmcnt(0)" : "+v"(t[0]), "+v"(t[1]), "+v"(t[2]), "+v"(t[NQ > 3 ? 3 : 0]));
  else asm volatile("s_waitcnt lgkmcnt(0)" : "+v"(t[0]), "+v"(t[NQ > 1 ? 1 : 0]));
#pragma unroll
  for (int g = 0; g < NQ; ++g) {
    v[4 * g] = t[g][0];
    v[4 * g + 1] = t[g][1];
    v[4 * g + 2] = t[g][2];
    v[4 * g + 3] = t[g][3];
  }
}

struct PendingTile2 {
  f32x16 a, b;
};
template <class ET, class WS, int S1, int S2, int MT, bool RELU, int FPOS, int KEEP_F32_TILE = -1, int PEND_M = -1, bool PEND_RELU = true,
          bool CARRY_OUT = false>
__device__ __forceinline__ void layer_16x2(WS& st, uint32_t bias_addr, const uint32_t* in1A, const uint32_t* in2A, const uint32_t* in1B,
                                           const uint32_t* in2B, uint32_t* outA, uint32_t* outB, PendingTile2& pend, uint32_t* pendA = nullptr,
                                           uint32_t* pendB = nullptr, f32x16* keepA = nullptr, f32x16* keepB = nullptr) {
  constexpr int CF = WS::kChunk;
  constexpr int KS = S1 + S2;
  constexpr int ABL = tune::kAblateShade;
  constexpr int PER = (KS >= 8) ? 1 : (8 + KS - 1) / KS;
  constexpr bool kKeepAll = KEEP_F32_TILE == kKeepAllF32;
  auto kept = [](int m) { return kKeepAll || KEEP_F32_TILE == m; };
  constexpr bool kCarry = !(ABL & 8);
  constexpr bool kHasPend = kCarry && PEND_M >= 0;
  constexpr int PERP = 1;
  static_assert(!kHasPend || KS >= 16, "a carried tile is consumed by the last two k-steps of a 16-k-step input segment, 6 k-steps behind its last conversion");
  static_assert(!CARRY_OUT || (KEEP_F32_TILE != MT - 1 && KEEP_F32_TILE != kKeepAllF32), "the kept tile is not converted");
  constexpr bool kCounted = !(ABL & (2 | 4));
  constexpr int kYounger = kCounted ? KS : 0;
  BiasRegs br;
  f32x16 pA, pB;
  int gA = 0, gB = 0;
  if (kHasPend) {
    pA = pend.a;
    pB = pend.b;
  }
  if (!(ABL & 4)) lds_bias_issue(bias_addr, br, st.rd_cur, st.rd_next);
#pragma unroll
  for (int m = 0; m < MT; ++m) {
    f32x16 bias, accA, accB;
    __builtin_amdgcn_sched_barrier(0);
    if (ABL & 4) {
#pragma unroll
      for (int r = 0; r < 16; ++r) bias[r] = 0.f;
    } else {
      if (m == 0) lds_bias_take<0>(br, &bias);
      else lds_bias_take<kYounger>(br, &bias);
      if (m + 1 < MT) lds_bias_issue(bias_addr + (m + 1) * 128, br, st.rd_cur, st.rd_next);
    }
#pragma unroll
    for (int s = 0; s < KS; ++s) {
      const int f = (FPOS + m * KS + s) % CF;
      ws_position<ABL>(st, f, false);
      const uint32_t* sa = (s < S1) ? (in1A + 4 * s) : (in2A + 4 * (s - S1));
      const uint32_t* sb = (s < S1) ? (in1B + 4 * s) : (in2B + 4 * (s - S1));
      const u32x4 ba = {sa[0], sa[1], sa[2], sa[3]}, bb = {sb[0], sb[1], sb[2], sb[3]};
      accA = ET::mfma(st.R[f % WS::kRegs], ba, s == 0 ? bias : accA);
      accB = ET::mfma(st.R[f % WS::kRegs], bb, s == 0 ? bias : accB);
      ws_refill<ABL>(st, f);
      constexpr int E0 = KS >= 8 + tune::kShadeGuardStep ? tune::kShadeGuardStep : 0;
      if (m > 0 && !kept(m - 1) && !(ABL & 8) && s >= E0) {
        if (s == E0) {
          gA = mfma_guard<ET, RELU>(pA);
          gB = mfma_guard<ET, RELU>(pB);
        }
#pragma unroll
        for (int k = 0; k < PER; ++k) {
          const int q = (s - E0) * PER + k;
          if (q < 4) epilogue_quad_16<ET, RELU>(pA, m - 1, q, outA, gA);
          else if (q < 8) epilogue_quad_16<ET, RELU>(pB, m - 1, q - 4, outB, gB);
        }
      }
      if (m == 0 && kHasPend && s >= E0) {
        if (s == E0) {
          gA = mfma_guard<ET, PEND_RELU>(pA);
          gB = mfma_guard<ET, PEND_RELU>(pB);
        }
#pragma unroll
        for (int k = 0; k < PERP; ++k) {
          const int q = (s - E0) * PERP + k;
          if (q < 4) epilogue_quad_16<ET, PEND_RELU>(pA, PEND_M < 0 ? 0 : PEND_M, q, pendA, gA);
          else if (q < 8) epilogue_quad_16<ET, PEND_RELU>(pB, PEND_M < 0 ? 0 : PEND_M, q - 4, pendB, gB);
        }
      }
      __builtin_amdgcn_sched_group_barrier(0x008, 1, 0);
      __builtin_amdgcn_sched_group_barrier(0x002, 2, 0);
      __builtin_amdgcn_sched_group_barrier(0x008, 1, 0);
      __builtin_amdgcn_sched_group_barrier(0x100, 1, 0);
      __builtin_amdgcn_sched_group_barrier(0x002, 2, 0);
      __builtin_amdgcn_sched_barrier(0);
    }
    if (kept(m)) {
      keepA[kKeepAll ? m : 0] = accA;
      keepB[kKeepAll ? m : 0] = accB;
    }
    if ((ABL & 8) && !kept(m)) {
      asm volatile("" ::"v"(accA), "v"(accB));
#pragma unroll
      for (int g = 0; g < 8; ++g) asm volatile("" : "=v"(outA[8 * m + g]), "=v"(outB[8 * m + g]));
    } else if (m + 1 < MT) {
      pA = accA;
      pB = accB;
    } else if (!kept(m)) {
      if (CARRY_OUT && kCarry) {
        pend.a = accA;
        pend.b = accB;
      } else {
        gA = mfma_guard<ET, RELU>(accA);
        gB = mfma_guard<ET, RELU>(accB);
#pragma unroll
        for (int g = 0; g < 4; ++g) epilogue_quad_16<ET, RELU>(accA, m, g, outA, gA);
#pragma unroll
        for (int g = 0; g < 4; ++g) epilogue_quad_16<ET, RELU>(accB, m, g, outB, gB);
      }
    }
  }
}

template <class ET, int FP, int FD>
__global__ __launch_bounds__(256) void shade_mlp16x2_kernel(ShadeArgs a) {
  static_assert(FP == 10 && FD == 4, "fragment positions below assume the 10-4 shading encoding");
  constexpr int QP = pe_slots(FP), QD = pe_slots(FD);
  constexpr int WAVES = 4, TILE = WAVES * 64, CF = tune::kChunkFrags2, RS = tune::kRingSlots2, LPW = CF / WAVES;
  constexpr int kRingBytes = CF * RS * 1024;
  static_assert(CF % WAVES == 0 && CF % tune::kRegFrags2 == 0 && kShadeFrags16 % CF == 0 && CF % 8 == 0 && CF <= 32, "chunk geometry");
  typedef WStream<CF, RS, LPW, tune::kRegFrags2> WS;
  constexpr int kStashPerBlock = (QP / 8 + QD / 8) * 1024;
  __shared__ __attribute__((aligned(16))) char lds[kRingBytes + kShadeBiasFloats * 4 + WAVES * 2 * kStashPerBlock];
  const int lane = lane_id();
  const int wave = __builtin_amdgcn_readfirstlane(static_cast<int>(threadIdx.x) >> 6);
  const int j = lane & 31, h = lane >> 5;
  const uint32_t stash = static_cast<uint32_t>(reinterpret_cast<uintptr_t>(lds)) + kRingBytes + kShadeBiasFloats * 4 +
                         wave * 2 * kStashPerBlock + lane * 16;
  int total = a.total ? *a.total : a.max_samples;
  if (total > a.max_samples) total = a.max_samples;
  const int ntiles = (total + TILE - 1) / TILE;
  if (static_cast<int>(blockIdx.x) >= ntiles) return;
  {
    float* lds_bias = reinterpret_cast<float*>(lds + kRingBytes);
    for (int i = threadIdx.x; i < kShadeBiasFloats; i += blockDim.x) lds_bias[i] = a.net.bias[i];
  }
  __syncthreads();
  WS st;
  ws_start(st, a.net.w, kShadeFrags16 * 1024, lds, wave, lane);
  const uint32_t bias0 = static_cast<uint32_t>(reinterpret_cast<uintptr_t>(lds)) + kRingBytes + h * 64;
  const uint32_t* bo = a.net.b_off;
  for (int tile = blockIdx.x; tile < ntiles; tile += gridDim.x) {
    const int s0 = tile * TILE + wave * 64 + j, s1 = s0 + 32;
    uint32_t hA0[64], hB0[64], hA1[64], hB1[64];
    PendingTile2 pend;
    uint64_t outside0, outside1;
    {
      float x[3], dpe[3];
      uint32_t pts0[QP / 2], pts1[QP / 2], dirs[QD / 2];
      outside0 = load_sample(a, s0, total, x, dpe);
      pe_pack<ET, FP>(x, h, pts0);
      pe_pack<ET, FD>(dpe, h, dirs);
      lds_stash_write<QP / 8>(stash, pts0);
      lds_stash_write<QD / 8>(stash + (QP / 8) * 1024, dirs);
      outside1 = load_sample(a, s1, total, x, dpe);
      pe_pack<ET, FP>(x, h, pts1);
      pe_pack<ET, FD>(dpe, h, dirs);
      lds_stash_write<QP / 8>(stash + kStashPerBlock, pts1);
      lds_stash_write<QD / 8>(stash + kStashPerBlock + (QP / 8) * 1024, dirs);
      layer_16x2<ET, WS, QP / 8, 0, 8, true, 0, -1, -1, true, true>(st, bias0 + bo[0] * 4, pts0, pts0, pts1, pts1, hA0, hA1, pend);
    }
#pragma unroll 1
    for (int l = 1; l <= 3; l += 2) {
      layer_16x2<ET, WS, 16, 0, 8, true, 0, -1, 7, true, true>(st, bias0 + bo[l] * 4, hA0, hA0, hA1, hA1, hB0, hB1, pend, hA0, hA1);
      layer_16x2<ET, WS, 16, 0, 8, true, 0, -1, 7, true, true>(st, bias0 + bo[l + 1] * 4, hB0, hB0, hB1, hB1, hA0, hA1, pend, hB0, hB1);
    }
    {
      uint32_t pts0[QP / 2], pts1[QP / 2];
      lds_stash_read<QP / 8>(stash, pts0);
      lds_stash_read<QP / 8>(stash + kStashPerBlock, pts1);
      layer_16x2<ET, WS, QP / 8, 16, 8, true, 0, -1, 7, true, true>(st, bias0 + bo[5] * 4, pts0, hA0, pts1, hA1, hB0, hB1, pend, hA0, hA1);
    }
    layer_16x2<ET, WS, 16, 0, 8, true, 0, -1, 7, true, true>(st, bias0 + bo[6] * 4, hB0, hB0, hB1, hB1, hA0, hA1, pend, hB0, hB1);
    layer_16x2<ET, WS, 16, 0, 8, true, 0, -1, 7, true, true>(st, bias0 + bo[7] * 4, hA0, hA0, hA1, hA1, hB0, hB1, pend, hA0, hA1);
    f32x16 alpha0, alpha1;
    layer_16x2<ET, WS, 16, 0, 9, false, 0, 8, 7, true, false>(st, bias0 + bo[8] * 4, hB0, hB0, hB1, hB1, hA0, hA1, pend, hB0, hB1, &alpha0, &alpha1);
    {
      uint32_t d0[QD / 2], d1[QD / 2];
      lds_stash_read<QD / 8>(stash + (QP / 8) * 1024, d0);
      lds_stash_read<QD / 8>(stash + kStashPerBlock + (QP / 8) * 1024, d1);
      layer_16x2<ET, WS, 16, QD / 8, 4, true, (32 + 4 * 128 + 160 + 2 * 128 + 144) % CF>(st, bias0 + bo[9] * 4, hA0, d0, hA1, d1, hB0, hB1, pend);
    }
    f32x16 rgb0, rgb1;
    layer_16x2<ET, WS, 8, 0, 1, false, (32 + 4 * 128 + 160 + 2 * 128 + 144 + 72) % CF, 0>(st, bias0 + bo[10] * 4, hB0, hB0, hB1, hB1, hA0, hA1, pend, nullptr, nullptr, &rgb0, &rgb1);
    if (h == 0 && s0 < total)
      store_raw(a, s0, rgb0[0], rgb0[1], rgb0[2], alpha0[0], outside_lane(outside0));
    if (h == 0 && s1 < total)
      store_raw(a, s1, rgb1[0], rgb1[1], rgb1[2], alpha1[0], outside_lane(outside1));
  }
  asm volatile("s_waitcnt vmcnt(0)" ::: "memory");
}

template <int FP, int FD>
__global__ __launch_bounds__(256) void shade_mlp32_kernel(ShadeArgs a) {
  constexpr int QP = pe_slots(FP), QD = pe_slots(FD);
  constexpr int TILE = 4 * 32;
  const int lane = lane_id();
  const int wave = __builtin_amdgcn_readfirstlane(static_cast<int>(threadIdx.x) >> 6);
  const int j = lane & 31, h = lane >> 5;
  int total = a.total ? *a.total : a.max_samples;
  if (total > a.max_samples) total = a.max_samples;
  const u32x4* w = a.net.w;
  const float* b = a.net.bias;

  for (int tile = blockIdx.x; tile * TILE < total; tile += gridDim.x) {
    const int s = tile * TILE + wave * 32 + j;
    if (tile * TILE + wave * 32 >= total) continue;
    asm volatile("" : "+v"(w), "+v"(b));
    float x[3], dpe[3];
    const uint64_t outside = load_sample(a, s, total, x, dpe);
    float pts[QP], dirs[QD], hA[144], hB[128];
    pe_eval<FP, true>(x, h, pts);
    pe_eval<FD, true>(dpe, h, dirs);
    layer_f32<QP, 0, 8, true>(w + a.net.w_off[0], b + a.net.b_off[0], lane, pts, pts, hA);
#pragma unroll 1
    for (int l = 1; l <= 3; l += 2) {
      layer_f32<128, 0, 8, true>(w + a.net.w_off[l], b + a.net.b_off[l], lane, hA, hA, hB);
      layer_f32<128, 0, 8, true>(w + a.net.w_off[l + 1], b + a.net.b_off[l + 1], lane, hB, hB, hA);
    }
    layer_f32<QP, 128, 8, true>(w + a.net.w_off[5], b + a.net.b_off[5], lane, pts, hA, hB);
    layer_f32<128, 0, 8, true>(w + a.net.w_off[6], b + a.net.b_off[6], lane, hB, hB, hA);
    layer_f32<128, 0, 8, true>(w + a.net.w_off[7], b + a.net.b_off[7], lane, hA, hA, hB);
    layer_f32<128, 0, 9, false>(w + a.net.w_off[8], b + a.net.b_off[8], lane, hB, hB, hA);
    const float alpha = hA[128];
    layer_f32<128, QD, 4, true>(w + a.net.w_off[9], b + a.net.b_off[9], lane, hA, dirs, hB);
    float rgb[16];
    layer_f32<64, 0, 1, false>(w + a.net.w_off[10], b + a.net.b_off[10], lane, hB, hB, rgb);
    if (h == 0 && s < total) store_raw_f32(a, s, rgb[0], rgb[1], rgb[2], alpha, outside_lane(outside));
  }
}

static __global__ __launch_bounds__(256) void shade_features_kernel(ShadeArgs a, float* feat, int FP, int FD) {
  const int s = blockIdx.x * blockDim.x + threadIdx.x;
  if (s >= a.max_samples) return;
  float x[3], dpe[3];
  load_sample(a, s, a.max_samples, x, dpe);
  const int NP = 3 + 6 * FP, ND = 3 + 6 * FD;
  float* f = feat + static_cast<size_t>(s) * (NP + ND);
  for (int c = 0; c < 3; ++c) {
    f[c] = x[c];
    f[NP + c] = dpe[c];
  }
  for (int b = 0; b < FP; ++b)
    for (int c = 0; c < 3; ++c) {
      float sn, co;
      sincosf(x[c] * static_cast<float>(1 << b), &sn, &co);
      f[3 + 6 * b + c] = sn;
      f[3 + 6 * b + 3 + c] = co;
    }
  for (int b = 0; b < FD; ++b)
    for (int c = 0; c < 3; ++c) {
      float sn, co;
      sincosf(dpe[c] * static_cast<float>(1 << b), &sn, &co);
      f[NP + 3 + 6 * b + c] = sn;
      f[NP + 3 + 6 * b + 3 + c] = co;
    }
}

}
```

Baseline: 209.7.

## Split large batches into two ray ranges overlapped across two streams

Large plain batches are now split into two ray halves, with sampling, compaction, shading and compositing of one half running on a second stream so it overlaps with the other half's stages. Expand and shade kernels gain a first-ray/first-sample offset so each range works on its own slice of the shared buffers. The goal is to fill idle compute during the serial pipeline tail and during the scan and compact phases. The cost is extra events, cross-stream synchronisation, and twice as many kernel launches, each over a smaller range.

```diff
diff --git a/adanerf_amd/csrc/adanerf_hip.hip b/adanerf_amd/csrc/adanerf_hip.hip
--- a/adanerf_amd/csrc/adanerf_hip.hip
+++ b/adanerf_amd/csrc/adanerf_hip.hip
@@ -43,7 +43,11 @@
 
 namespace {
 
-enum { kTotalSamples = 0, kTotalRefined = 4, kTotalGuardSeen = 8, kTotalSlots = 16 };
+enum { kTotalSamples = 0, kTotalEndA = 1, kTotalFirstB = 2, kTotalRefined = 4, kTotalGuardSeen = 8, kTotalSlots = 16 };
+
+enum { kEvHead = 0, kEvSampled = 1, kEvCompacted = 2, kEvShaded = 3, kEvEnd = 4, kEvB = 4, kEvCompositedA = 9, kEventsPerBatch = 10 };
+
+constexpr int kTwoRangeMinRays = 262144;
 enum { kSeenMax = 0, kSeenViolations = 1, kSeenPair = 2, kSeenAuditMismatch = 3, kSeenAudited = 4, kGuardSeenSlots = 5 };
 
 constexpr const char* kOccupancyQuery = "hipOccupancyMaxActiveBlocksPerMultiprocessor";
@@ -153,7 +157,7 @@
   const int32_t* count;
 };
 
-int launch_sample_mlp(adanerf_ctx* c, int first_ray, int n_rays, float* d_oracle, float* d_rays, const SelectOut* sel = nullptr,
+int launch_sample_mlp(adanerf_ctx* c, hipStream_t stream, int first_ray, int n_rays, float* d_oracle, float* d_rays, const SelectOut* sel = nullptr,
                       const RayList* list = nullptr) {
   if (n_rays <= 0) return ADANERF_OK;
   if (list && (c->generic0 || !sel || (c->sampling_mode != ADANERF_SAMPLING_SPLIT_FP16 && c->sampling_mode != ADANERF_SAMPLING_GUARDED)))
@@ -179,13 +183,13 @@
         return fail(c, ADANERF_EUNSUPPORTED, "sampling network: bias table exceeds the kernel's LDS capacity");
       return hip_rc(c, dispatch<kEnc10_4, kEnc2_2, kEncMax>(c->enc0, [&](auto e) {
         return dispatch<64, 128, 256>(W0, [&](auto w) {
-          hipLaunchKernelGGL((sample_mlp16x3_gen_kernel<enc_fp(e()), enc_fd(e()), w()>), grid, block, 0, c->stream, a, c->gen0);
+          hipLaunchKernelGGL((sample_mlp16x3_gen_kernel<enc_fp(e()), enc_fd(e()), w()>), grid, block, 0, stream, a, c->gen0);
           return hipGetLastError();
         }, hipErrorInvalidValue);
       }, hipErrorInvalidValue), "hipGetLastError()");
     }
     if (sel) return fail(c, ADANERF_EINVAL, "fused selection is not available on the fp32 run-time-shaped sampling kernel");
-    HIP_RETURN(c, launch_sample_mlp_gen(a, c->gen0, c->enc0, c->topo0.width, grid.x, c->stream));
+    HIP_RETURN(c, launch_sample_mlp_gen(a, c->gen0, c->enc0, c->topo0.width, grid.x, stream));
   }
   const bool guarded = c->sampling_mode == ADANERF_SAMPLING_GUARDED && sel != nullptr && !has_budget_map(c) && !(c->sample_cap > 0.f) && !list;
   if (list) {
@@ -204,7 +208,7 @@
     if (c->debug_guard & 1) a.sel.guard_rows = nullptr;
     a.sel.guard_seen = reinterpret_cast<uint32_t*>(c->total.p) + kTotalGuardSeen;
   }
-  if (c->sampling_mode == ADANERF_SAMPLING_FP32) HIP_RETURN(c, launch_sample_mlp_f32(a, c->enc0, grid.x, c->stream));
+  if (c->sampling_mode == ADANERF_SAMPLING_FP32) HIP_RETURN(c, launch_sample_mlp_f32(a, c->enc0, grid.x, stream));
   auto for_enc = [&](auto&& f) {
     return dispatch<kEnc10_4, kEnc2_2>(c->enc0, [&](auto e) { return f(std::integral_constant<int, enc_fp(e())>{}, std::integral_constant<int, enc_fd(e())>{}); },
                                        hipErrorInvalidValue);
@@ -220,8 +224,8 @@
     a.net16 = c->net0_f16.params;
     const bool two_blocks = sel != nullptr && a.fused_select && !a.oracle_out && !(c->debug_guard & 2) && (n_rays >= kSample16x2MinRays || (c->debug_guard & 4));
     if (int rc = hip_rc(c, for_enc([&](auto fp, auto fd) {
-      return two_blocks ? launch_persistent(c->grids, sample_mlp16x2_kernel<fp(), fd()>, (n_rays + 255) / 256, 256, c->stream, a)
-                        : launch_persistent(c->grids, sample_mlp16_kernel<fp(), fd()>, (n_rays + 255) / 256, 512, c->stream, a);
+      return two_blocks ? launch_persistent(c->grids, sample_mlp16x2_kernel<fp(), fd()>, (n_rays + 255) / 256, 256, stream, a)
+                        : launch_persistent(c->grids, sample_mlp16_kernel<fp(), fd()>, (n_rays + 255) / 256, 512, stream, a);
     }), kOccupancyQuery)) return rc;
     if (guarded) {
       const int n_words = (n_rays + 31) / 32;
@@ -231,7 +235,7 @@
       const int rgrid = std::min(static_cast<int>(grid.x), resident);
       const int cap_round = (c->opt.flags & ADANERF_FLAG_GUARD_AUDIT_FILL) ? rgrid * 128 : 0;
       const int cycle = a.sel.audit_period > 0 ? static_cast<int>((c->guard_frame / static_cast<uint32_t>(a.sel.audit_period)) & 0x7fffffffu) : 0;
-      hipLaunchKernelGGL(refine_list_kernel, dim3((n_words + 255) / 256), dim3(256), 0, c->stream, reinterpret_cast<const uint32_t*>(c->guard_mask.p),
+      hipLaunchKernelGGL(refine_list_kernel, dim3((n_words + 255) / 256), dim3(256), 0, stream, reinterpret_cast<const uint32_t*>(c->guard_mask.p),
                          n_words, n_rays, a.sel.audit_period, a.sel.audit_phase, cap_round, cycle, reinterpret_cast<int32_t*>(c->refine_list.p), n_list);
       SampleArgs r = a;
       r.net16 = c->net0_split.params;
@@ -245,10 +249,10 @@
       r.sel.refine_list = reinterpret_cast<const int32_t*>(c->refine_list.p);
       r.ray_list = r.sel.refine_list;
       r.n_list = n_list;
-      if (int rc = hip_rc(c, for_enc([&](auto fp, auto fd) { return launch_persistent(c->grids, sample_mlp16x3_kernel<fp(), fd()>, rgrid, 256, c->stream, r); }), kOccupancyQuery)) return rc;
+      if (int rc = hip_rc(c, for_enc([&](auto fp, auto fd) { return launch_persistent(c->grids, sample_mlp16x3_kernel<fp(), fd()>, rgrid, 256, stream, r); }), kOccupancyQuery)) return rc;
     }
   } else {
-    if (int rc = hip_rc(c, for_enc([&](auto fp, auto fd) { return launch_persistent(c->grids, sample_mlp16x3_kernel<fp(), fd()>, static_cast<int>(grid.x), 256, c->stream, a); }), kOccupancyQuery)) return rc;
+    if (int rc = hip_rc(c, for_enc([&](auto fp, auto fd) { return launch_persistent(c->grids, sample_mlp16x3_kernel<fp(), fd()>, static_cast<int>(grid.x), 256, stream, a); }), kOccupancyQuery)) return rc;
   }
   HIP_RETURN(c, hipGetLastError());
 }
@@ -267,16 +271,17 @@
   return so;
 }
 
-int launch_expand(adanerf_ctx* c, int n_rays, int n_max, int seg_shift, int32_t* d_off, const int32_t* d_cnt, uint32_t* d_key, float* d_w,
-                  int32_t* d_total) {
+int launch_expand(adanerf_ctx* c, hipStream_t stream, int n_rays, int n_max, int seg_shift, int32_t* d_off, const int32_t* d_cnt, uint32_t* d_key,
+                  float* d_w, int32_t* d_total, int first_ray = 0, int32_t* d_first = nullptr) {
   const int nblk = (n_rays + (1 << seg_shift) - 1) >> seg_shift;
   const int32_t* bt = reinterpret_cast<const int32_t*>(c->block_total.p);
   int32_t* bo = reinterpret_cast<int32_t*>(c->block_offset.p);
-  const dim3 egrid((n_rays + 255) / 256);
+  const dim3 egrid((n_rays - first_ray + 255) / 256);
   const bool inline_scan = nblk <= kInlineScanMaxBlocks;
-  if (!inline_scan) hipLaunchKernelGGL(scan_blocks_kernel, dim3(1), dim3(1024), 0, c->stream, bt, nblk, bo, d_total);
-  hipLaunchKernelGGL(inline_scan ? expand_kernel<true> : expand_kernel<false>, egrid, dim3(256), 0, c->stream, d_cnt, reinterpret_cast<const uint8_t*>(c->selbin.p),
-                     reinterpret_cast<const float*>(c->selw.p), bo, bt, nblk, n_rays, n_max, seg_shift, d_off, d_key, d_w, d_total);
+  if (first_ray && (!inline_scan || first_ray % 256)) return fail(c, ADANERF_EINVAL, "launch_expand: a ray range needs the inline scan and a first ray on a workgroup boundary");
+  if (!inline_scan) hipLaunchKernelGGL(scan_blocks_kernel, dim3(1), dim3(1024), 0, stream, bt, nblk, bo, d_total);
+  hipLaunchKernelGGL(inline_scan ? expand_kernel<true> : expand_kernel<false>, egrid, dim3(256), 0, stream, d_cnt, reinterpret_cast<const uint8_t*>(c->selbin.p),
+                     reinterpret_cast<const float*>(c->selw.p), bo, bt, nblk, n_rays, n_max, seg_shift, d_off, d_key, d_w, d_total, first_ray / 256, d_first);
   HIP_RETURN(c, hipGetLastError());
 }
 
@@ -379,7 +384,7 @@
       if (int rc = launch_depth_limit(c, *dl, n_rays, n_max, kPairSegShift, d_cnt)) return rc;
     if (cap_total)
       if (int rc = launch_cap(c, n_rays, n_max, thr, kPairSegShift, d_cnt, *cap_total)) return rc;
-    return launch_expand(c, n_rays, n_max, kPairSegShift, d_off, d_cnt, d_key, d_w, d_total);
+    return launch_expand(c, c->stream, n_rays, n_max, kPairSegShift, d_off, d_cnt, d_key, d_w, d_total);
   }
   const int nblk = (n_rays + kSelRaysPerBlock - 1) / kSelRaysPerBlock;
   hipLaunchKernelGGL(select_kernel, dim3(nblk), dim3(256), 0, c->stream, d_oracle, n_rays, n_max, thr, c->ms.transform, d_cnt,
@@ -391,7 +396,7 @@
     if (int rc = launch_depth_limit(c, *dl, n_rays, n_max, kSelSegShift, d_cnt)) return rc;
   if (cap_total)
     if (int rc = launch_cap(c, n_rays, n_max, thr, kSelSegShift, d_cnt, *cap_total)) return rc;
-  return launch_expand(c, n_rays, n_max, kSelSegShift, d_off, d_cnt, d_key, d_w, d_total);
+  return launch_expand(c, c->stream, n_rays, n_max, kSelSegShift, d_off, d_cnt, d_key, d_w, d_total);
 }
 
 GuardKey guard_key(adanerf_ctx* c) {
@@ -482,9 +487,9 @@
       }
       c->ms.rg = g;
       c->sampling_mode = ADANERF_SAMPLING_SPLIT_FP16;
-      if ((rc = launch_sample_mlp(c, 0, CR, reinterpret_cast<float*>(a_buf.p), nullptr))) return done(rc);
+      if ((rc = launch_sample_mlp(c, c->stream, 0, CR, reinterpret_cast<float*>(a_buf.p), nullptr))) return done(rc);
       c->sampling_mode = ADANERF_SAMPLING_FP16;
-      if ((rc = launch_sample_mlp(c, 0, CR, reinterpret_cast<float*>(b_buf.p), nullptr))) return done(rc);
+      if ((rc = launch_sample_mlp(c, c->stream, 0, CR, reinterpret_cast<float*>(b_buf.p), nullptr))) return done(rc);
       hipLaunchKernelGGL(guard_stats_kernel, dim3((CR + 3) / 4), dim3(256), 0, c->stream, reinterpret_cast<const float*>(b_buf.p),
                          reinterpret_cast<const float*>(a_buf.p), CR, c->ms.info.num_samples, c->ms.info.threshold, two_eps, reinterpret_cast<uint32_t*>(acc.p));
     }
@@ -564,8 +569,8 @@
   return ADANERF_OK;
 }
 
-int launch_shade_mlp(adanerf_ctx* c, const float* d_rays, const uint32_t* d_key, const int32_t* d_total, int max_samples, int prec,
-                     float* d_raw, const float* d_z = nullptr, bool coarse = false) {
+int launch_shade_mlp(adanerf_ctx* c, hipStream_t stream, const float* d_rays, const uint32_t* d_key, const int32_t* d_total, int max_samples, int prec,
+                     float* d_raw, const float* d_z = nullptr, bool coarse = false, const int32_t* d_first = nullptr) {
   if (max_samples <= 0) return ADANERF_OK;
   const bool generic = coarse ? c->genericc : c->generic1;
   const NetTopology& topo = coarse ? c->topoc : c->topo1;
@@ -581,6 +586,8 @@
   a.total = d_total;
   a.max_samples = max_samples;
   a.raw_out = d_raw;
+  a.first = d_first;
+  if (d_first && (generic || prec == ADANERF_PREC_FP32)) return fail(c, ADANERF_EINVAL, "launch_shade_mlp: a sample range needs the 8 x 256 network on a 16-bit engine");
   a.pos_limit = prec == ADANERF_PREC_BF16 ? static_cast<float>(kPosIdentityBound) : std::numeric_limits<float>::max();
   const int enc = coarse ? enc_layout(c->ms.fp0, c->ms.fd0, false) : c->enc1;
   auto for_elem = [&](auto&& f) { return prec == ADANERF_PREC_BF16 ? f(Bf16{}) : f(Fp16{}); };
@@ -593,20 +600,20 @@
           using ET = decltype(et);
           constexpr int FP = enc_fp(e()), FD = enc_fd(e()), W = w(), NB = gen_blocks<W, FP>();
           const int tiles = (max_samples + 128 * NB - 1) / (128 * NB);
-          return launch_persistent(c->grids, shade_mlp16_gen_staged_kernel<ET, FP, FD, W, NB, gen_occupancy<W, FP>()>, tiles, 256, c->stream, a, gen);
+          return launch_persistent(c->grids, shade_mlp16_gen_staged_kernel<ET, FP, FD, W, NB, gen_occupancy<W, FP>()>, tiles, 256, stream, a, gen);
         }, hipErrorInvalidValue);
       }, hipErrorInvalidValue);
     }), kOccupancyQuery))) return rc;
   } else if (generic) {
     const int per_wg = topo.width == kWideWidth ? 64 : 128;
-    HIP_TRY(c, launch_shade_mlp_gen(c->grids, a, gen, enc, topo.width, (max_samples + per_wg - 1) / per_wg, c->stream));
+    HIP_TRY(c, launch_shade_mlp_gen(c->grids, a, gen, enc, topo.width, (max_samples + per_wg - 1) / per_wg, stream));
   } else if (prec == ADANERF_PREC_FP32) {
-    HIP_TRY(c, launch_shade_mlp_f32(c->grids, a, (max_samples + 127) / 128, c->stream));
+    HIP_TRY(c, launch_shade_mlp_f32(c->grids, a, (max_samples + 127) / 128, stream));
   } else {
     const int tiles = (max_samples + 255) / 256;
     if ((rc = hip_rc(c, for_elem([&](auto et) {
       using ET = decltype(et);
-      hipLaunchKernelGGL((shade_mlp16x2_kernel<ET, 10, 4>), dim3(std::min(tiles, c->ms.info.compute_units)), dim3(256), 0, c->stream, a);
+      hipLaunchKernelGGL((shade_mlp16x2_kernel<ET, 10, 4>), dim3(std::min(tiles, c->ms.info.compute_units)), dim3(256), 0, stream, a);
       return hipSuccess;
     }), kOccupancyQuery))) return rc;
   }
@@ -652,7 +659,7 @@
   HIP_RETURN(c, hipGetLastError());
 }
 
-int launch_composite(adanerf_ctx* c, const float* d_raw, const float* d_w, const int32_t* d_off, const int32_t* d_cnt, int n_rays,
+int launch_composite(adanerf_ctx* c, hipStream_t stream, const float* d_raw, const float* d_w, const int32_t* d_off, const int32_t* d_cnt, int n_rays,
                      float* d_rgb, void* d_rgba8, const uint32_t* d_key = nullptr, float* d_depth = nullptr, float* d_acc = nullptr) {
   if (n_rays <= 0) return ADANERF_OK;
   AuxOut aux{};
@@ -663,14 +670,14 @@
     aux.ztab = c->ms.sp.ztab;
   }
   if (c->ms.info.num_samples > 32)
-    hipLaunchKernelGGL(composite_wave_kernel, dim3((n_rays + 3) / 4), dim3(256), 0, c->stream, reinterpret_cast<const float4*>(d_raw), d_w,
+    hipLaunchKernelGGL(composite_wave_kernel, dim3((n_rays + 3) / 4), dim3(256), 0, stream, reinterpret_cast<const float4*>(d_raw), d_w,
                        d_off, d_cnt, n_rays, c->ms.mult_mode, d_rgb, reinterpret_cast<uchar4*>(d_rgba8), aux);
   else {
     const int N = c->ms.info.num_samples;
     auto run = [&](auto rb_tag) {
       constexpr int RB = decltype(rb_tag)::value;
       const int cap = RB * N;
-      hipLaunchKernelGGL(composite_kernel<RB>, dim3((n_rays + RB - 1) / RB), dim3(RB), static_cast<size_t>(cap) * 20, c->stream,
+      hipLaunchKernelGGL(composite_kernel<RB>, dim3((n_rays + RB - 1) / RB), dim3(RB), static_cast<size_t>(cap) * 20, stream,
                          reinterpret_cast<const float4*>(d_raw), d_w, d_off, d_cnt, n_rays, c->ms.mult_mode, cap, d_rgb,
                          reinterpret_cast<uchar4*>(d_rgba8), aux);
     };
@@ -742,6 +749,9 @@
   c->sampling_mode = opt->sampling_mode;
   c->model_dir = model_dir;
   if (const char* dbg = std::getenv("ADANERF_DEBUG_GUARD")) c->debug_guard = std::atoi(dbg);
+  c->two_range_min = kTwoRangeMinRays;
+  if (const char* tr = std::getenv("ADANERF_TWO_RANGES"))
+    if (*tr) c->two_range_min = std::max(std::atoi(tr), 0);
   c->guard_audit_period = opt->guard_audit_period == 0 ? ADANERF_GUARD_AUDIT_PERIOD : std::max(opt->guard_audit_period, 0);
   c->ms.info.guard_audit_period = c->sampling_mode == ADANERF_SAMPLING_GUARDED ? c->guard_audit_period : 0;
   if (c->sampling_mode == ADANERF_SAMPLING_GUARDED) c->model0_hash = fnv1a64_file(join_path(model_dir, "model0.onnx"));
@@ -812,6 +822,12 @@
   (void)hipSetDevice(c->device);
   if (c->peer_event) (void)hipEventDestroy(c->peer_event);
   if (c->stream) (void)hipStreamSynchronize(c->stream);
+  if (c->range_stream) {
+    (void)hipStreamSynchronize(c->range_stream);
+    (void)hipStreamDestroy(c->range_stream);
+  }
+  for (hipEvent_t e : {c->range_fork, c->range_sampled, c->range_join})
+    if (e) (void)hipEventDestroy(e);
   for (hipEvent_t e : c->events) (void)hipEventDestroy(e);
   for (int32_t* p : c->pinned_totals) (void)hipHostFree(p);
   if (c->guard_host) (void)hipHostFree(c->guard_host);
@@ -934,7 +950,7 @@
   BIND(c);
   if (c->ms.coarse_fine) return fail(c, ADANERF_EUNSUPPORTED, "coarse/fine models have no sampling network (adanerf_sample_uniform / adanerf_shade_mlp_coarse)");
   if (first_ray < 0 || n_rays < 0 || first_ray + n_rays > c->ms.info.rays_local) return fail(c, ADANERF_EINVAL, "ray range outside this context's rays");
-  return launch_sample_mlp(c, first_ray, n_rays, d_oracle, d_rays);
+  return launch_sample_mlp(c, c->stream, first_ray, n_rays, d_oracle, d_rays);
 }
 
 int adanerf_compact(adanerf_ctx* c, const float* d_oracle, int32_t n_rays, int32_t n_max, float thr, int32_t* d_off, int32_t* d_cnt,
@@ -990,7 +1006,7 @@
   so.guard_rows = d_monitor ? const_cast<float*>(d_approx) : nullptr;
   so.guard_seen = d_monitor;
   hipLaunchKernelGGL(select_rows_kernel, grid, block, 0, c->stream, d_exact, n_rays, so, static_cast<const int32_t*>(d_refined));
-  return launch_expand(c, n_rays, n_max, kPairSegShift, d_off, d_cnt, d_key, d_w, d_total);
+  return launch_expand(c, c->stream, n_rays, n_max, kPairSegShift, d_off, d_cnt, d_key, d_w, d_total);
 }
 
 int adanerf_calibrate_guard(adanerf_ctx* c, int32_t n_poses, uint32_t seed, int32_t set, float* max_diff, float* max_pair_diff) {
@@ -1041,7 +1057,7 @@
                         int32_t max_samples, int32_t precision, float* d_raw) {
   BIND(c);
   if (!d_rays || !d_key || !d_raw || max_samples < 0) return fail(c, ADANERF_EINVAL, "bad argument");
-  return launch_shade_mlp(c, d_rays, d_key, d_total, max_samples, precision < 0 ? c->ms.info.precision : precision, d_raw, d_z);
+  return launch_shade_mlp(c, c->stream, d_rays, d_key, d_total, max_samples, precision < 0 ? c->ms.info.precision : precision, d_raw, d_z);
 }
 
 int adanerf_sample_uniform(adanerf_ctx* c, int32_t first_ray, int32_t n_rays, float* d_rays, int32_t* d_off, int32_t* d_cnt, uint32_t* d_key,
@@ -1059,7 +1075,7 @@
   BIND(c);
   if (!c->ms.coarse_fine) return fail(c, ADANERF_EUNSUPPORTED, "adanerf_shade_mlp_coarse: not a coarse/fine model");
   if (!d_rays || !d_key || !d_raw || max_samples < 0) return fail(c, ADANERF_EINVAL, "bad argument");
-  return launch_shade_mlp(c, d_rays, d_key, d_total, max_samples, precision < 0 ? c->ms.info.precision : precision, d_raw, nullptr, true);
+  return launch_shade_mlp(c, c->stream, d_rays, d_key, d_total, max_samples, precision < 0 ? c->ms.info.precision : precision, d_raw, nullptr, true);
 }
 
 int adanerf_sample_from_coarse(adanerf_ctx* c, const float* d_raw_coarse, const float* d_rays, int32_t n_rays, int32_t* d_off, int32_t* d_cnt,
@@ -1092,7 +1108,7 @@
                       float* d_rgb, void* d_rgba8) {
   BIND(c);
   if (!d_raw || !d_w || !d_off || !d_cnt || n_rays < 0) return fail(c, ADANERF_EINVAL, "bad argument");
-  return launch_composite(c, d_raw, d_w, d_off, d_cnt, n_rays, d_rgb, d_rgba8);
+  return launch_composite(c, c->stream, d_raw, d_w, d_off, d_cnt, n_rays, d_rgb, d_rgba8);
 }
 
 int adanerf_composite_aux(adanerf_ctx* c, const float* d_raw, const float* d_w, const int32_t* d_off, const int32_t* d_cnt, const uint32_t* d_key,
@@ -1101,7 +1117,7 @@
   if (!d_raw || !d_w || !d_off || !d_cnt || n_rays < 0) return fail(c, ADANERF_EINVAL, "bad argument");
   if (!d_key && !c->ms.info.dense && (d_depth || d_acc))
     return fail(c, ADANERF_EINVAL, "adanerf_composite_aux: a depth or acc map needs d_sample_key unless the context is dense (threshold 0)");
-  return launch_composite(c, d_raw, d_w, d_off, d_cnt, n_rays, d_rgb, d_rgba8, d_key, d_depth, d_acc);
+  return launch_composite(c, c->stream, d_raw, d_w, d_off, d_cnt, n_rays, d_rgb, d_rgba8, d_key, d_depth, d_acc);
 }
 
 int adanerf_composite_classic_aux(adanerf_ctx* c, const float* d_raw, const float* d_z, const float* d_rays, int32_t n_rays, int32_t n,
@@ -1131,20 +1147,34 @@
 
 int sum_stats(adanerf_ctx* c, adanerf_stats* stats) {
   std::memset(stats, 0, sizeof(*stats));
-  const size_t nb = c->events_used / 5;
+  const size_t nb = c->events_used / kEventsPerBatch;
+  int two = 0;
   for (size_t b = 0; b < nb; ++b) {
-    hipEvent_t* ev = &c->events[b * 5];
+    hipEvent_t* ev = &c->events[b * kEventsPerBatch];
     float t;
-    HIP_TRY(c, hipEventElapsedTime(&t, ev[0], ev[1]));
-    stats->ms_sample_mlp += t;
-    HIP_TRY(c, hipEventElapsedTime(&t, ev[1], ev[2]));
-    stats->ms_compact += t;
-    HIP_TRY(c, hipEventElapsedTime(&t, ev[2], ev[3]));
-    stats->ms_shade_mlp += t;
-    HIP_TRY(c, hipEventElapsedTime(&t, ev[3], ev[4]));
-    stats->ms_composite += t;
-    HIP_TRY(c, hipEventElapsedTime(&t, ev[0], ev[4]));
-    stats->ms_total += t;
+    if (c->batch_two_ranges[b]) {
+      ++two;
+      float ta[5] = {0.f, 0.f, 0.f, 0.f, 0.f}, tb[5] = {0.f, 0.f, 0.f, 0.f, 0.f};
+      for (int k = kEvSampled; k <= kEvEnd; ++k) {
+        HIP_TRY(c, hipEventElapsedTime(&ta[k], ev[kEvHead], ev[k == kEvEnd ? kEvCompositedA : k]));
+        HIP_TRY(c, hipEventElapsedTime(&tb[k], ev[kEvHead], ev[kEvB + k]));
+      }
+      float* const span[5] = {nullptr, &stats->ms_sample_mlp, &stats->ms_compact, &stats->ms_shade_mlp, &stats->ms_composite};
+      for (int k = kEvSampled; k <= kEvEnd; ++k) *span[k] += std::max(ta[k], tb[k]) - std::min(ta[k - 1], tb[k - 1]);
+      HIP_TRY(c, hipEventElapsedTime(&t, ev[kEvHead], ev[kEvEnd]));
+      stats->ms_total += t;
+    } else {
+      HIP_TRY(c, hipEventElapsedTime(&t, ev[0], ev[1]));
+      stats->ms_sample_mlp += t;
+      HIP_TRY(c, hipEventElapsedTime(&t, ev[1], ev[2]));
+      stats->ms_compact += t;
+      HIP_TRY(c, hipEventElapsedTime(&t, ev[2], ev[3]));
+      stats->ms_shade_mlp += t;
+      HIP_TRY(c, hipEventElapsedTime(&t, ev[3], ev[4]));
+      stats->ms_composite += t;
+      HIP_TRY(c, hipEventElapsedTime(&t, ev[0], ev[4]));
+      stats->ms_total += t;
+    }
     const int32_t* tot = c->pinned_totals[b];
     stats->total_samples += tot[kTotalSamples];
     if (c->sampling_mode == ADANERF_SAMPLING_GUARDED) {
@@ -1164,8 +1194,8 @@
   HIP_TRY(c, hipMemcpy(&ovf, c->overflow.p, sizeof(int32_t), hipMemcpyDeviceToHost));
   stats->sampling_overflow = ovf;
   stats->batches = static_cast<int32_t>(nb);
-  stats->shade_launches = static_cast<int32_t>(nb);
-  stats->sample_launches = static_cast<int32_t>(nb);
+  stats->shade_launches = static_cast<int32_t>(nb) + two;
+  stats->sample_launches = static_cast<int32_t>(nb) + two;
   const adanerf_stats& f = c->folded;
   stats->total_samples += f.total_samples;
   stats->rays_refined += f.rays_refined;
@@ -1208,7 +1238,7 @@
   float* oracle = reinterpret_cast<float*>(c->oracle.p);
   for (int first = 0; first < R; first += B) {
     const int n = std::min(B, R - first);
-    if ((rc = launch_sample_mlp(c, first, n, oracle, rays))) return rc;
+    if ((rc = launch_sample_mlp(c, c->stream, first, n, oracle, rays))) return rc;
     if ((rc = adanerf_copy_result_sampling_network(c, oracle, n, static_cast<char*>(d_rgba8) + static_cast<size_t>(first) * 4))) return rc;
   }
   return ADANERF_OK;
@@ -1269,7 +1299,7 @@
     reset_record(c);
   }
   const bool record = (stats || c->profiling) && static_cast<size_t>(n_batches) <= kMaxProfiledBatches;
-  if (record && c->events_used && c->events_used / 5 + n_batches > kMaxProfiledBatches) {
+  if (record && c->events_used && c->events_used / kEventsPerBatch + n_batches > kMaxProfiledBatches) {
     HIP_TRY(c, hipStreamSynchronize(c->stream));
     adanerf_stats part;
     if ((rc = sum_stats(c, &part))) return rc;
@@ -1277,18 +1307,19 @@
     c->events_used = 0;
   }
   if (record) {
-    const size_t need = c->events_used + static_cast<size_t>(n_batches) * 5;
+    const size_t need = c->events_used + static_cast<size_t>(n_batches) * kEventsPerBatch;
     while (c->events.size() < need) {
       hipEvent_t e;
       HIP_TRY(c, hipEventCreate(&e));
       c->events.push_back(e);
     }
-    while (c->pinned_totals.size() < need / 5) {
+    while (c->pinned_totals.size() < need / kEventsPerBatch) {
       int32_t* p = nullptr;
       HIP_TRY(c, hipHostMalloc(reinterpret_cast<void**>(&p), kTotalSlots * sizeof(int32_t), hipHostMallocDefault));
       std::memset(p, 0, kTotalSlots * sizeof(int32_t));
       c->pinned_totals.push_back(p);
     }
+    if (c->batch_two_ranges.size() < need / kEventsPerBatch) c->batch_two_ranges.resize(need / kEventsPerBatch, 0);
   }
   *record_out = record;
   return ADANERF_OK;
@@ -1301,6 +1332,64 @@
   float* acc;
   float* disp;
 };
+
+int ensure_range_stream(adanerf_ctx* c) {
+  if (!c->range_stream) HIP_TRY(c, hipStreamCreateWithFlags(&c->range_stream, hipStreamNonBlocking));
+  for (hipEvent_t* e : {&c->range_fork, &c->range_sampled, &c->range_join})
+    if (!*e) HIP_TRY(c, hipEventCreateWithFlags(e, hipEventDisableTiming));
+  return ADANERF_OK;
+}
+
+int render_two_ranges(adanerf_ctx* c, int first, int n, int nA, const SelectOut& so, const BatchOut& out, hipEvent_t* ev) {
+  const int N = c->ms.info.num_samples, nB = n - nA, prec = c->ms.info.precision;
+  float* rays = reinterpret_cast<float*>(c->rays.p);
+  int32_t* off = reinterpret_cast<int32_t*>(c->ray_offsets.p);
+  int32_t* cnt = reinterpret_cast<int32_t*>(c->ray_counts.p);
+  uint32_t* key = reinterpret_cast<uint32_t*>(c->sample_key.p);
+  float* sw = reinterpret_cast<float*>(c->sample_w.p);
+  float* raw = reinterpret_cast<float*>(c->raw.p);
+  int32_t* total = reinterpret_cast<int32_t*>(c->total.p);
+  if (int rc = ensure_range_stream(c)) return rc;
+  if (int rc = ensure_shading_net(c, prec, false)) return rc;
+  const hipStream_t sa = c->stream, sb = c->range_stream;
+  const size_t a_rays = static_cast<size_t>(nA);
+  SelectOut so_b = so;
+  so_b.counts += a_rays;
+  so_b.selbin += a_rays * N;
+  so_b.selw += a_rays * N;
+  so_b.seg_total += a_rays >> kPairSegShift;
+  HIP_TRY(c, hipEventRecord(c->range_fork, sa));
+  HIP_TRY(c, hipStreamWaitEvent(sb, c->range_fork, 0));
+  auto both = [&]() -> int {
+    int rc;
+    if ((rc = launch_sample_mlp(c, sa, first, nA, nullptr, rays, &so))) return rc;
+    HIP_TRY(c, hipEventRecord(c->range_sampled, sa));
+    if (ev) HIP_TRY(c, hipEventRecord(ev[kEvSampled], sa));
+    if ((rc = launch_sample_mlp(c, sb, first + nA, nB, nullptr, rays + a_rays * 8, &so_b))) return rc;
+    if (ev) HIP_TRY(c, hipEventRecord(ev[kEvB + kEvSampled], sb));
+    if ((rc = launch_expand(c, sa, nA, N, kPairSegShift, off, cnt, key, sw, total + kTotalEndA))) return rc;
+    if (ev) HIP_TRY(c, hipEventRecord(ev[kEvCompacted], sa));
+    HIP_TRY(c, hipStreamWaitEvent(sb, c->range_sampled, 0));
+    if ((rc = launch_expand(c, sb, n, N, kPairSegShift, off, cnt, key, sw, total + kTotalSamples, nA, total + kTotalFirstB))) return rc;
+    if (ev) HIP_TRY(c, hipEventRecord(ev[kEvB + kEvCompacted], sb));
+    if ((rc = launch_shade_mlp(c, sa, rays, key, total + kTotalEndA, nA * N, prec, raw))) return rc;
+    if (ev) HIP_TRY(c, hipEventRecord(ev[kEvShaded], sa));
+    if ((rc = launch_shade_mlp(c, sb, rays, key, total + kTotalSamples, nB * N, prec, raw, nullptr, false, total + kTotalFirstB))) return rc;
+    if (ev) HIP_TRY(c, hipEventRecord(ev[kEvB + kEvShaded], sb));
+    if ((rc = launch_composite(c, sa, raw, sw, off, cnt, nA, out.rgb, out.rgba8, key))) return rc;
+    if (ev) HIP_TRY(c, hipEventRecord(ev[kEvCompositedA], sa));
+    if ((rc = launch_composite(c, sb, raw, sw, off + a_rays, cnt + a_rays, nB, out.rgb ? out.rgb + a_rays * 3 : nullptr,
+                               out.rgba8 ? static_cast<char*>(out.rgba8) + a_rays * 4 : nullptr, key))) return rc;
+    if (ev) HIP_TRY(c, hipEventRecord(ev[kEvB + kEvEnd], sb));
+    return ADANERF_OK;
+  };
+  const int rc = both();
+  const hipError_t e1 = hipEventRecord(c->range_join, sb);
+  const hipError_t e2 = e1 == hipSuccess ? hipStreamWaitEvent(sa, c->range_join, 0) : e1;
+  if (e2 != hipSuccess) (void)hipStreamSynchronize(sb);
+  if (rc) return rc;
+  return hip_rc(c, e2, "two ray ranges: join");
+}
 
 int render_batch(adanerf_ctx* c, int first, int n, const RayList* list, const BatchOut& out, bool record) {
   const int B = c->ms.info.batch_rays, N = c->ms.info.num_samples;
@@ -1324,7 +1413,7 @@
     float* rawc = reinterpret_cast<float*>(c->raw_coarse.p);
     if ((rc = launch_camera_rays(c, first, n, rays))) return rc;
     if ((rc = launch_sample_uniform(c, n, c->ms.n_coarse, off, cnt, keyc, total))) return rc;
-    if ((rc = launch_shade_mlp(c, rays, keyc, total, n * c->ms.n_coarse, c->ms.info.precision, rawc, nullptr, true))) return rc;
+    if ((rc = launch_shade_mlp(c, c->stream, rays, keyc, total, n * c->ms.n_coarse, c->ms.info.precision, rawc, nullptr, true))) return rc;
     if (ev) HIP_TRY(c, hipEventRecord(ev[1], c->stream));
     if ((rc = launch_sample_fine(c, rawc, rays, n, off, cnt, key, reinterpret_cast<float*>(c->sample_z.p), total))) return rc;
   }
@@ -1336,7 +1425,23 @@
   const bool capped = cap_trims(c) && !pdf && thr > 0.f;
   const int64_t cap_total = capped ? cap_total_of(c, n) : 0;
   const DepthLimit dl{c->depth_limit, first, list ? list->ids : nullptr, rays, c->ms.sp.ztab, depth_pose(c->ms.rg.pos, c->ms.rg.rot)};
-  if (!cfm && (rc = launch_sample_mlp(c, first, n, fused ? nullptr : oracle, rays, fused ? &so : nullptr, list))) return rc;
+  if (ev) c->batch_two_ranges[c->events_used / kEventsPerBatch] = 0;
+  const bool plain_fast = !list && fused && !c->generic0 && !c->generic1 &&
+                          (c->sampling_mode == ADANERF_SAMPLING_SPLIT_FP16 || c->sampling_mode == ADANERF_SAMPLING_FP16) &&
+                          c->ms.info.precision != ADANERF_PREC_FP32 && !budget && !limited && !has_sample_cap(c) && !out.depth && !out.acc && !out.disp &&
+                          N <= 32 && ((n + 31) >> kPairSegShift) <= kInlineScanMaxBlocks;
+  const int nA = (plain_fast && c->two_range_min > 0 && n >= c->two_range_min) ? (n / 2) & ~255 : 0;
+  if (nA > 0) {
+    if ((rc = render_two_ranges(c, first, n, nA, so, out, ev))) return rc;
+    if (ev) {
+      c->batch_two_ranges[c->events_used / kEventsPerBatch] = 1;
+      HIP_TRY(c, hipEventRecord(ev[kEvEnd], c->stream));
+      HIP_TRY(c, hipMemcpyAsync(c->pinned_totals[c->events_used / kEventsPerBatch], total, kTotalSlots * sizeof(int32_t), hipMemcpyDeviceToHost, c->stream));
+      c->events_used += kEventsPerBatch;
+    }
+    return ADANERF_OK;
+  }
+  if (!cfm && (rc = launch_sample_mlp(c, c->stream, first, n, fused ? nullptr : oracle, rays, fused ? &so : nullptr, list))) return rc;
   if (ev && !cfm) HIP_TRY(c, hipEventRecord(ev[1], c->stream));
   float* sz = reinterpret_cast<float*>(c->sample_z.p);
   if (cfm) rc = ADANERF_OK;
@@ -1345,7 +1450,7 @@
     rc = budget ? launch_trim(c, bm, n, N, thr, kPairSegShift, cnt) : ADANERF_OK;
     if (!rc && limited) rc = launch_depth_limit(c, dl, n, N, kPairSegShift, cnt);
     if (!rc && capped) rc = launch_cap(c, n, N, thr, kPairSegShift, cnt, cap_total);
-    if (!rc) rc = launch_expand(c, n, N, kPairSegShift, off, cnt, key, sw, total);
+    if (!rc) rc = launch_expand(c, c->stream, n, N, kPairSegShift, off, cnt, key, sw, total);
   }
   else if (thr == 0.f) {
     hipLaunchKernelGGL(dense_offsets_kernel, dim3((n + 255) / 256), dim3(256), 0, c->stream, n, off, cnt, total);
@@ -1357,7 +1462,7 @@
   const float* sw_s = dense_implicit ? oracle : sw;
   if (ev) HIP_TRY(c, hipEventRecord(ev[2], c->stream));
   const int64_t max_s = static_cast<int64_t>(n) * N;
-  if ((rc = launch_shade_mlp(c, rays, key_s, total, static_cast<int>(max_s), c->ms.info.precision, raw, pdf ? sz : nullptr))) return rc;
+  if ((rc = launch_shade_mlp(c, c->stream, rays, key_s, total, static_cast<int>(max_s), c->ms.info.precision, raw, pdf ? sz : nullptr))) return rc;
   if (ev) HIP_TRY(c, hipEventRecord(ev[3], c->stream));
   float* depth_b = out.depth;
   float* acc_b = out.acc;
@@ -1367,7 +1472,7 @@
     if (!acc_b) acc_b = reinterpret_cast<float*>(c->disp_scratch.p) + B;
   }
   if (pdf) rc = launch_composite_classic(c, raw, sz, rays, n, N, out.rgb, out.rgba8, depth_b, acc_b);
-  else rc = launch_composite(c, raw, sw_s, off, cnt, n, out.rgb, out.rgba8, key_s, depth_b, acc_b);
+  else rc = launch_composite(c, c->stream, raw, sw_s, off, cnt, n, out.rgb, out.rgba8, key_s, depth_b, acc_b);
   if (rc) return rc;
   if (out.disp && n > 0) {
     hipLaunchKernelGGL(disp_map_kernel, dim3((n + 255) / 256), dim3(256), 0, c->stream, depth_b, acc_b, n, out.disp);
@@ -1375,8 +1480,8 @@
   }
   if (ev) {
     HIP_TRY(c, hipEventRecord(ev[4], c->stream));
-    HIP_TRY(c, hipMemcpyAsync(c->pinned_totals[c->events_used / 5], total, kTotalSlots * sizeof(int32_t), hipMemcpyDeviceToHost, c->stream));
-    c->events_used += 5;
+    HIP_TRY(c, hipMemcpyAsync(c->pinned_totals[c->events_used / kEventsPerBatch], total, kTotalSlots * sizeof(int32_t), hipMemcpyDeviceToHost, c->stream));
+    c->events_used += kEventsPerBatch;
   }
   return ADANERF_OK;
 }
@@ -1389,8 +1494,8 @@
     if (int rc = sum_stats(c, stats)) return rc;
     stats->rays = rays;
     if (n_batches > 0 && record) {
-      const size_t e0 = c->events_used - static_cast<size_t>(n_batches) * 5;
-      HIP_TRY(c, hipEventElapsedTime(&stats->ms_total, c->events[e0], c->events[c->events_used - 1]));
+      const size_t e0 = c->events_used - static_cast<size_t>(n_batches) * kEventsPerBatch;
+      HIP_TRY(c, hipEventElapsedTime(&stats->ms_total, c->events[e0 + kEvHead], c->events[c->events_used - kEventsPerBatch + kEvEnd]));
     }
     reset_record(c);
   }
diff --git a/adanerf_amd/csrc/context.hpp b/adanerf_amd/csrc/context.hpp
--- a/adanerf_amd/csrc/context.hpp
+++ b/adanerf_amd/csrc/context.hpp
@@ -55,6 +55,10 @@
   adanerf::GridCache grids;
   std::vector<hipEvent_t> events;
   size_t events_used = 0;
+  std::vector<uint8_t> batch_two_ranges;
+  hipStream_t range_stream = nullptr;
+  hipEvent_t range_fork = nullptr, range_sampled = nullptr, range_join = nullptr;
+  int two_range_min = 0;
   bool profiling = false;
   int prof_frames = 0;
   std::vector<int32_t*> pinned_totals;
diff --git a/adanerf_amd/csrc/k_compact.hip.hpp b/adanerf_amd/csrc/k_compact.hip.hpp
--- a/adanerf_amd/csrc/k_compact.hip.hpp
+++ b/adanerf_amd/csrc/k_compact.hip.hpp
@@ -288,17 +288,19 @@
                                                      const float* __restrict__ selw, const int32_t* __restrict__ block_offset,
                                                      const int32_t* __restrict__ block_total, int n_blocks, int n_rays, int n_max,
                                                      int seg_shift, int32_t* __restrict__ ray_offsets, uint32_t* __restrict__ sample_key,
-                                                     float* __restrict__ sample_w, int32_t* __restrict__ total) {
+                                                     float* __restrict__ sample_w, int32_t* __restrict__ total, int first_wg,
+                                                     int32_t* __restrict__ first_out) {
   const int segs = 256 >> seg_shift;
   const int t = static_cast<int>(threadIdx.x);
-  const int r = blockIdx.x * 256 + t;
+  const int wg = static_cast<int>(blockIdx.x) + first_wg;
+  const int r = wg * 256 + t;
   const int c = (r < n_rays) ? counts[r] : 0;
   const int x = seg_shift == 5 ? wave_incl_sum_dpp_i32<32>(c) : wave_incl_sum_dpp_i32<64>(c);
   const int seg = r >> seg_shift;
   int seg_base;
   if (INLINE_SCAN) {
     __shared__ int part[4];
-    const int b0 = blockIdx.x * segs;
+    const int b0 = wg * segs;
     int s = 0;
     for (int i = t; i < b0; i += 256) s += block_total[i];
     s = wave_sum_dpp_i32(s);
@@ -311,6 +313,7 @@
       for (int i = b0; i < n_blocks; ++i) tot += block_total[i];
       *total = tot;
     }
+    if (first_out && blockIdx.x == 0 && t == 0) *first_out = part[0] + part[1] + part[2] + part[3];
   } else {
     seg_base = (seg < n_blocks) ? block_offset[seg] : 0;
   }
diff --git a/adanerf_amd/csrc/k_mlp16.hip.hpp b/adanerf_amd/csrc/k_mlp16.hip.hpp
--- a/adanerf_amd/csrc/k_mlp16.hip.hpp
+++ b/adanerf_amd/csrc/k_mlp16.hip.hpp
@@ -17,6 +17,7 @@
   int32_t max_samples;
   float* raw_out;
   float pos_limit;
+  const int32_t* first;
 };
 
 __device__ __forceinline__ uint64_t position_outside(const ShadeArgs& a, const float x[3]) {
@@ -510,9 +511,10 @@
   const int j = lane & 31, h = lane >> 5;
   const uint32_t stash = static_cast<uint32_t>(reinterpret_cast<uintptr_t>(lds)) + kRingBytes + kShadeBiasFloats * 4 +
                          wave * 2 * kStashPerBlock + lane * 16;
-  int total = a.total ? *a.total : a.max_samples;
-  if (total > a.max_samples) total = a.max_samples;
-  const int ntiles = (total + TILE - 1) / TILE;
+  const int first = a.first ? max(*a.first, 0) : 0;
+  int total = a.total ? *a.total : first + a.max_samples;
+  if (total - first > a.max_samples) total = first + a.max_samples;
+  const int ntiles = (total - first + TILE - 1) / TILE;
   if (static_cast<int>(blockIdx.x) >= ntiles) return;
   {
     float* lds_bias = reinterpret_cast<float*>(lds + kRingBytes);
@@ -524,7 +526,7 @@
   const uint32_t bias0 = static_cast<uint32_t>(reinterpret_cast<uintptr_t>(lds)) + kRingBytes + h * 64;
   const uint32_t* bo = a.net.b_off;
   for (int tile = blockIdx.x; tile < ntiles; tile += gridDim.x) {
-    const int s0 = tile * TILE + wave * 64 + j, s1 = s0 + 32;
+    const int s0 = first + tile * TILE + wave * 64 + j, s1 = s0 + 32;
     uint32_t hA0[64], hB0[64], hA1[64], hB1[64];
     PendingTile2 pend;
     uint64_t outside0, outside1;
```

New measurement: 211.6, median of 6. No clear change (+0.9%).
